# avik-pal/RegNeuralDE.jl

Measured on AMD Instinct MI355X. Metric: training-step samples/sec + mean NFE, MNIST Neural ODE bs=512, higher is better.
Workload: dtype f32; 1 GPU; MNIST NODE regularized (error_est), Tsit5 reltol=abstol=1.4e-8, batch 512 per GPU, 1xMI355X per rank; step = loss fwd + reverse pass through the solver + InvDecay/Momentum update; the weights train during the timed steps (mean_nfe drifts with --steps: value_fixed_weights of --full is the stationary companion); global_batch=512, parallelism=single

## Files before the change

### include/rnde.h

```cpp
#ifndef RNDE_H
#define RNDE_H
#include <stddef.h>
#include <stdint.h>

#ifdef __cplusplus
extern "C" {
#endif

#define RNDE_MAX_LAYERS 8

typedef enum {
    RNDE_OK = 0,
    RNDE_ERR_BAD_ARG = 1,
    RNDE_ERR_MAX_ATTEMPTS = 2,
    RNDE_ERR_DT_UNDERFLOW = 3,
    RNDE_ERR_NONFINITE = 4,
    RNDE_ERR_HIP = 5,
    RNDE_ERR_NO_TAPE = 6,
    RNDE_ERR_NO_DEVICE = 7
} rnde_status;

typedef enum { RNDE_ACT_IDENTITY = 0, RNDE_ACT_TANH = 1, RNDE_ACT_RELU = 2, RNDE_ACT_SIGMOID = 3, RNDE_ACT_SOFTPLUS = 4, RNDE_ACT_ELU = 5 } rnde_act;
typedef enum { RNDE_PRE_NONE = 0, RNDE_PRE_TANH = 1, RNDE_PRE_CUBE = 2 } rnde_pre_act;
typedef enum { RNDE_SOLVER_TSIT5 = 0, RNDE_SOLVER_DP5 = 1, RNDE_SOLVER_DOP853 = 2 } rnde_solver;
typedef enum { RNDE_REG_NONE = 0, RNDE_REG_ERR = 1, RNDE_REG_STIFF = 2, RNDE_REG_ERR_STIFF = 3,
               RNDE_REG_STIFF_DT = 4
} rnde_reg;

typedef struct {
    int32_t n_layers;
    int32_t dims[RNDE_MAX_LAYERS + 1];
    int32_t act[RNDE_MAX_LAYERS];
    int32_t time_dep;
    int32_t pre_act;
    int32_t max_batch;
    int32_t solver;
    float   reltol, abstol;
    int32_t regularize;
    int32_t cb_save_start;
    int32_t track_ctrl;
    int32_t track_initdt;
    int32_t max_attempts;
    int32_t device;
    int32_t col_tile;
    int32_t persist;
    int32_t wgrad_side_pct;
    int32_t stage_generic;
} rnde_node_config;

typedef struct rnde_node rnde_node;
typedef struct rnde_comm rnde_comm;

const char* rnde_version(void);
const char* rnde_last_error(const rnde_node* h);
int32_t     rnde_param_count(const rnde_node_config* cfg);

rnde_status rnde_node_create(const rnde_node_config* cfg, rnde_node** out);
void        rnde_node_destroy(rnde_node* h);

rnde_status rnde_node_create_tiled(const rnde_node_config* cfg, rnde_node** out);
int64_t     rnde_node_tiled_lds_bytes(const rnde_node_config* cfg);

rnde_status rnde_node_forward(rnde_node* h, const float* x_dev, const float* p_dev, int32_t B,
                              float t0, float t1, float* u_out_dev, int64_t* nfe_out,
                              float* saveval_host, int32_t* n_saveval_out, int32_t keep_tape,
                              void* stream);

rnde_status rnde_node_forward_saveat(rnde_node* h, const float* x_dev, const float* p_dev, int32_t B,
                                     float t0, float t1, const float* saveat_host, int32_t n_saveat,
                                     float* u_saved_dev, int64_t* nfe_out, float* saveval_host,
                                     int32_t* n_saveval_out, int32_t keep_tape, void* stream);

rnde_status rnde_node_forward_everystep(rnde_node* h, const float* x_dev, const float* p_dev, int32_t B, float t0, float t1,
                                        int32_t save_start, float* sol_out_dev, int32_t capacity, float* t_host_out, int32_t* n_out,
                                        int64_t* nfe_out, float* saveval_host, int32_t* n_saveval_out, int32_t keep_tape, void* stream);

rnde_status rnde_node_forward_replay(rnde_node* h, const float* x_dev, const float* p_dev, int32_t B,
                                     float t0, float t1, const float* steps_host, int32_t n_steps,
                                     float* u_out_dev, int64_t* nfe_out, float* saveval_host,
                                     int32_t* n_saveval_out, int32_t keep_tape, void* stream);

rnde_status rnde_node_backward(rnde_node* h, const float* u_bar_dev, const float* saveval_bar_host,
                               float* x_bar_dev, float* p_bar_dev, float* tspan_bar_host,
                               void* stream);

rnde_status rnde_node_backward_async(rnde_node* h, const float* u_bar_dev, const float* saveval_bar_host,
                                     float* x_bar_dev, float* p_bar_dev, float* tspan_bar_dev, void* stream);

rnde_status rnde_node_release_tape(rnde_node* h);

rnde_status rnde_node_forward_host(rnde_node* h, const float* x, const float* p, int32_t B, float t0,
                                   float t1, float* u_out, int64_t* nfe_out, float* saveval,
                                   int32_t* n_saveval_out, int32_t keep_tape);
rnde_status rnde_node_backward_host(rnde_node* h, const float* u_bar, const float* saveval_bar,
                                    float* x_bar, float* p_bar, float* tspan_bar);

rnde_status rnde_node_steps(rnde_node* h, float* steps_host, int32_t capacity, int32_t* n_attempts_out);

rnde_status rnde_debug_feval(rnde_node* h, const float* u_dev, const float* p_dev, int32_t B, float t,
                             float* out_dev, void* stream);
rnde_status rnde_debug_attempt(rnde_node* h, const float* uprev_dev, const float* k1_dev,
                               const float* p_dev, int32_t B, float t, float dt, float* k_out_dev,
                               float* unew_out_dev, float* eest_out, void* stream);
rnde_status rnde_bench_attempt(rnde_node* h, const float* x_dev, const float* p_dev, int32_t B,
                               int32_t iters, float* mean_us_out, void* stream);
rnde_status rnde_bench_attempt_taped(rnde_node* h, const float* x_dev, const float* p_dev, int32_t B,
                                     int32_t iters, float* mean_us_out, void* stream);
rnde_status rnde_bench_attempt_cold_tape(rnde_node* h, const float* x_dev, const float* p_dev, int32_t B, int32_t iters,
                                         int32_t records, float* mean_us_out, void* stream);
rnde_status rnde_node_set_timing(rnde_node* h, int32_t on);
rnde_status rnde_node_timing(rnde_node* h, float* fwd_attempts_ms, float* rev_sweep_ms, float* rev_rest_ms);
int32_t     rnde_node_last_attempts(const rnde_node* h);
int32_t     rnde_node_fallback_count(const rnde_node* h);
int32_t     rnde_node_launches_per_attempt(const rnde_node* h);
int32_t     rnde_node_one_launch_solves(const rnde_node* h);
#define RNDE_MATRIX_F32 0
#define RNDE_MATRIX_BF16X3 1
rnde_status rnde_node_set_matrix_mode(rnde_node* h, int32_t mode);
int32_t     rnde_node_matrix_mode(const rnde_node* h);

typedef struct rnde_tapes rnde_tapes;
rnde_status rnde_tapes_create(const rnde_node_config* cfg, int32_t max_tapes, rnde_tapes** out);
void        rnde_tapes_destroy(rnde_tapes* t);
const char* rnde_tapes_last_error(const rnde_tapes* t);
int32_t     rnde_tapes_in_use(const rnde_tapes* t);
rnde_node*  rnde_tapes_node(rnde_tapes* t, int32_t tape_id);
rnde_status rnde_tapes_forward(rnde_tapes* t, const float* x_dev, const float* p_dev, int32_t B, float t0, float t1, float* u_out_dev,
                               int64_t* nfe_out, float* saveval_host, int32_t* n_saveval_out, int32_t keep_tape, void* stream,
                               int32_t* tape_id_out);
rnde_status rnde_tapes_backward(rnde_tapes* t, int32_t tape_id, const float* u_bar_dev, const float* saveval_bar_host, float* x_bar_dev,
                                float* p_bar_dev, float* tspan_bar_host, void* stream);
rnde_status rnde_tapes_release(rnde_tapes* t, int32_t tape_id);

rnde_status rnde_classifier_head(rnde_node* h, const float* u_dev, const float* p3_dev, const float* y_dev,
                                 int32_t B, int32_t n_classes, float* logits_out_dev, float* u_bar_dev,
                                 float* p3_bar_dev, float* ce_out_dev, void* stream);

rnde_status rnde_node_classifier_grad(rnde_node* h, const float* x_dev, const float* p2_dev, const float* p3_dev,
                                      const float* y_dev, int32_t B, int32_t n_classes, float t0, float t1, float lambda,
                                      float* p2_bar_dev, float* p3_bar_dev, float* x_bar_dev, float* ce_out_dev,
                                      float* reg_out_host, int64_t* nfe_out, rnde_comm* comm, void* stream);

rnde_status rnde_momentum_step(float* p_dev, const float* g_dev, float* v_dev, int64_t len, int64_t n, float gamma,
                               float eta, float rho, void* stream);

rnde_status rnde_momentum_step_scaled(float* p_dev, const float* g_dev, float* v_dev, int64_t len, int64_t n, float gamma,
                                      float eta, float rho, float gscale, void* stream);
rnde_status rnde_adam_step(float* p_dev, const float* g_dev, float* m_dev, float* v_dev, int64_t len, int64_t t, float eta, float beta1,
                           float beta2, float eps, float gscale, void* stream);
rnde_status rnde_adabelief_step(float* p_dev, const float* g_dev, float* m_dev, float* s_dev, int64_t len, float eta, float beta1, float beta2,
                                float eps, float gscale, void* stream);

#define RNDE_COMM_ID_BYTES 128
rnde_status rnde_comm_unique_id(uint8_t id_out[RNDE_COMM_ID_BYTES]);
rnde_status rnde_comm_create(const uint8_t id[RNDE_COMM_ID_BYTES], int32_t rank, int32_t world, int32_t device, rnde_comm** out);
void        rnde_comm_destroy(rnde_comm* c);
int32_t     rnde_comm_world(const rnde_comm* c);
const char* rnde_comm_last_error(const rnde_comm* c);
const char* rnde_comm_library(void);
rnde_status rnde_comm_allreduce(rnde_comm* c, float* buf_dev, int64_t n, int32_t mean, void* stream);
rnde_status rnde_comm_create_local_group(int32_t world, int32_t device, rnde_comm** out);
rnde_status rnde_comm_health(rnde_comm* c);
#define RNDE_COMM_WINDOW_BYTES 64
typedef struct rnde_comm_window rnde_comm_window;
rnde_status rnde_comm_window_create(int32_t device, rnde_comm_window** win_out, uint8_t handle_out[RNDE_COMM_WINDOW_BYTES]);
void        rnde_comm_window_destroy(rnde_comm_window* w);
rnde_status rnde_comm_create_peers(rnde_comm_window* win, const uint8_t* handles, int32_t rank, int32_t world, rnde_comm** out);
const char* rnde_comm_path(const rnde_comm* c);

rnde_status rnde_node_set_coupling(rnde_node* h, rnde_comm* c, int32_t global_batch);

typedef enum { RNDE_SDE_SOSRI = 0, RNDE_SDE_SRIW1 = 1, RNDE_SDE_SOSRI2 = 2 } rnde_sde_solver;

typedef struct {
    int32_t drift_layers;
    int32_t drift_dims[RNDE_MAX_LAYERS + 1];
    int32_t drift_act[RNDE_MAX_LAYERS];
    int32_t diff_layers;
    int32_t diff_dims[RNDE_MAX_LAYERS + 1];
    int32_t diff_act[RNDE_MAX_LAYERS];
    int32_t max_batch;
    int32_t solver;
    float   reltol, abstol;
    int32_t regularize;
    int32_t cb_save_start;
    int32_t max_attempts;
    int32_t device;
    float   beta1, beta2, gamma, qmin, qmax, qoldinit, delta;
    int32_t generic;
    float   stability_size;
} rnde_nsde_config;

typedef struct rnde_nsde rnde_nsde;

int32_t     rnde_nsde_param_count(const rnde_nsde_config* cfg, int32_t* len_drift_out);
rnde_status rnde_nsde_create(const rnde_nsde_config* cfg, rnde_nsde** out);
void        rnde_nsde_destroy(rnde_nsde* h);
const char* rnde_nsde_last_error(const rnde_nsde* h);

rnde_status rnde_nsde_forward(rnde_nsde* h, const float* x_dev, const float* p_dev, int32_t B, float t0, float t1,
                              const float* noise_dev, int32_t n_pool, uint64_t seed, float* u_out_dev,
                              int64_t* nfe1_out, int64_t* nfe2_out, float* saveval_host, int32_t* n_saveval_out,
                              int32_t keep_tape, void* stream);
rnde_status rnde_nsde_forward_saveat(rnde_nsde* h, const float* x_dev, const float* p_dev, int32_t B, float t0, float t1,
                                     const float* noise_dev, int32_t n_pool, uint64_t seed, const float* saveat_host,
                                     int32_t n_saveat, float* u_saved_dev, int64_t* nfe1_out, int64_t* nfe2_out,
                                     float* saveval_host, int32_t* n_saveval_out, int32_t keep_tape, void* stream);

rnde_status rnde_nsde_forward_everystep(rnde_nsde* h, const float* x_dev, const float* p_dev, int32_t B, float t0, float t1,
                                        const float* noise_dev, int32_t n_pool, uint64_t seed, int32_t save_start, float* sol_out_dev,
                                        int32_t capacity, float* t_host_out, int32_t* n_out, int64_t* nfe1_out, int64_t* nfe2_out,
                                        float* saveval_host, int32_t* n_saveval_out, int32_t keep_tape, void* stream);
rnde_status rnde_nsde_forward_replay(rnde_nsde* h, const float* x_dev, const float* p_dev, int32_t B, float t0, float t1,
                                     const float* noise_dev, int32_t n_pool, const float* steps_host, int32_t n_steps,
                                     float* u_out_dev, int64_t* nfe1_out, int64_t* nfe2_out, float* saveval_host,
                                     int32_t* n_saveval_out, int32_t keep_tape, void* stream);
rnde_status rnde_nsde_backward(rnde_nsde* h, const float* u_bar_dev, const float* saveval_bar_host, float* x_bar_dev,
                               float* p_bar_dev, void* stream);
rnde_status rnde_nsde_backward_async(rnde_nsde* h, const float* u_bar_dev, const float* saveval_bar_host, float* x_bar_dev,
                               float* p_bar_dev, void* stream);
rnde_status rnde_nsde_classifier_head(rnde_nsde* h, const float* u_dev, const float* p3_dev, const float* y_dev, int32_t B, int32_t n_classes,
                                      float* logits_out_dev, float* u_bar_dev, float* p3_bar_dev, float* ce_out_dev, void* stream);

rnde_status rnde_nsde_classifier_grad(rnde_nsde* h, const float* x_dev, const float* p2_dev, const float* p3_dev, const float* y_dev,
                                      int32_t B, int32_t n_classes, float t0, float t1, const float* noise_dev, int32_t n_pool,
                                      uint64_t seed, float lambda, float* p2_bar_dev, float* p3_bar_dev, float* x_bar_dev,
                                      float* ce_out_dev, float* reg_out_host, int64_t* nfe1_out, int64_t* nfe2_out, void* stream);
rnde_status rnde_moment_loss(const float* u_saved_dev, const float* data_mean_dev, const float* data_var_dev, int32_t D, int32_t T, int32_t B,
                             float* loss_out_dev, float* u_bar_dev, void* stream);
rnde_status rnde_nsde_moment_grad(rnde_nsde* h, const float* x_dev, const float* p_dev, int32_t B, float t0, float t1, const float* noise_dev,
                                  int32_t n_pool, uint64_t seed, const float* saveat_host, int32_t n_saveat, const float* data_mean_dev,
                                  const float* data_var_dev, float c, float* p_bar_dev, float* x_bar_dev, float* loss_out_dev, float* reg_out_host,
                                  int64_t* nfe1_out, int64_t* nfe2_out, void* stream);
rnde_status rnde_nsde_set_pre_act(rnde_nsde* h, int32_t drift_pre, int32_t diff_pre);
rnde_status rnde_nsde_steps(rnde_nsde* h, float* steps_host, int32_t capacity, int32_t* n_attempts_out, int32_t* draws_out);
rnde_status rnde_nsde_debug_attempt(rnde_nsde* h, const float* uprev_dev, const float* p_dev, int32_t B, float dt,
                                    const float* dW_dev, const float* dZ_dev, float* kg_out_dev, float* unew_out_dev,
                                    float* eest_out, void* stream);
rnde_status rnde_nsde_timing(rnde_nsde* h, float* solve_ms, float* rev_sweep_ms, int32_t* attempts, int32_t* accepted);
rnde_status rnde_normal_fill(float* out_dev, int64_t n, uint64_t seed, uint64_t stream_id, void* stream);

typedef struct { int32_t max_batch, max_T, device; } rnde_latent_config;
typedef struct rnde_latent rnde_latent;
rnde_status rnde_latent_create(const rnde_latent_config* cfg, rnde_latent** out);
void        rnde_latent_destroy(rnde_latent* h);
const char* rnde_latent_last_error(const rnde_latent* h);
void        rnde_latent_param_counts(int32_t* n_p1, int32_t* n_p2, int32_t* n_p4);
rnde_status rnde_latent_encode(rnde_latent* h, const float* x_dev, const float* p1_dev, const float* p2_dev, const float* eps_dev, int32_t B,
                               int32_t T, float* z0_out_dev, float* mu0_out_dev, float* logvar_out_dev, void* stream);
rnde_status rnde_latent_decode_loss(rnde_latent* h, const float* res_dev, const float* p4_dev, const float* x_dev, int32_t B, int32_t T,
                                    float* loss2_out_dev, float* res_bar_out_dev, float* p4_bar_out_dev, void* stream);
rnde_status rnde_adamax_step(float* p_dev, const float* g_dev, float* m_dev, float* u_dev, int64_t len, int64_t n, float gamma, float eta, float beta1,
                             float beta2, float eps, float beta1_pow, void* stream);
rnde_status rnde_latent_encode_backward(rnde_latent* h, const float* z0_bar_dev, float lambda_k, const float* p1_dev, const float* p2_dev,
                                        const float* x_dev, float* p1_bar_out_dev, float* p2_bar_out_dev, void* stream);

typedef enum { RNDE_FFJORD_CONCAT_SQUASH = 0, RNDE_FFJORD_TRACKER_FORWARD = 1 } rnde_ffjord_dynamics;
typedef struct {
    int32_t in_dims, hidden;
    int32_t dynamics;
    int32_t time_dep;
    int32_t regularize;
    int32_t kinetic_reg;
    int32_t max_batch, solver;
    float reltol, abstol;
    int32_t cb_save_start;
    int32_t max_attempts, device;
} rnde_ffjord_config;
// ... 59 lines not shown
```

### regneuralde.jl_amd/_lib.py

```python
import ctypes as C
import os

from . import build as _build

MAX_LAYERS = 8
OK, BAD_ARG, MAX_ATTEMPTS, DT_UNDERFLOW, NONFINITE, HIP_ERR, NO_TAPE, NO_DEVICE = range(8)
REG = {"none": 0, False: 0, None: 0, "error_est": 1, True: 1, "stiff_est": 2, "error_stiff_est": 3}


class NodeConfig(C.Structure):
    _fields_ = [("n_layers", C.c_int32), ("dims", C.c_int32 * (MAX_LAYERS + 1)), ("act", C.c_int32 * MAX_LAYERS),
                ("time_dep", C.c_int32), ("pre_act", C.c_int32), ("max_batch", C.c_int32), ("solver", C.c_int32),
                ("reltol", C.c_float), ("abstol", C.c_float), ("regularize", C.c_int32),
                ("cb_save_start", C.c_int32), ("track_ctrl", C.c_int32), ("track_initdt", C.c_int32),
                ("max_attempts", C.c_int32), ("device", C.c_int32), ("col_tile", C.c_int32),
                ("persist", C.c_int32), ("wgrad_side_pct", C.c_int32), ("stage_generic", C.c_int32)]


class NsdeConfig(C.Structure):
    _fields_ = [("drift_layers", C.c_int32), ("drift_dims", C.c_int32 * (MAX_LAYERS + 1)), ("drift_act", C.c_int32 * MAX_LAYERS),
                ("diff_layers", C.c_int32), ("diff_dims", C.c_int32 * (MAX_LAYERS + 1)), ("diff_act", C.c_int32 * MAX_LAYERS),
                ("max_batch", C.c_int32), ("solver", C.c_int32), ("reltol", C.c_float), ("abstol", C.c_float),
                ("regularize", C.c_int32), ("cb_save_start", C.c_int32), ("max_attempts", C.c_int32), ("device", C.c_int32),
                ("beta1", C.c_float), ("beta2", C.c_float), ("gamma", C.c_float), ("qmin", C.c_float), ("qmax", C.c_float),
                ("qoldinit", C.c_float), ("delta", C.c_float), ("generic", C.c_int32), ("stability_size", C.c_float)]


class FfjordConfig(C.Structure):
    _fields_ = [("in_dims", C.c_int32), ("hidden", C.c_int32), ("dynamics", C.c_int32), ("time_dep", C.c_int32), ("regularize", C.c_int32),
                ("kinetic_reg", C.c_int32), ("max_batch", C.c_int32), ("solver", C.c_int32), ("reltol", C.c_float), ("abstol", C.c_float),
                ("cb_save_start", C.c_int32), ("max_attempts", C.c_int32), ("device", C.c_int32)]


class FfjordChainConfig(C.Structure):
    _fields_ = [("n_layers", C.c_int32), ("dims", C.c_int32 * (MAX_LAYERS + 1)), ("act", C.c_int32 * MAX_LAYERS), ("time_dep", C.c_int32),
                ("regularize", C.c_int32), ("max_batch", C.c_int32), ("solver", C.c_int32), ("reltol", C.c_float), ("abstol", C.c_float),
                ("cb_save_start", C.c_int32), ("max_attempts", C.c_int32), ("device", C.c_int32)]


class LatentConfig(C.Structure):
    _fields_ = [("max_batch", C.c_int32), ("max_T", C.c_int32), ("device", C.c_int32)]


ODE_SOLVER = {"Tsit5": 0, "AutoTsit5": 0, "DP5": 1, "DOP853": 2}
SDE_SOLVER = {"SOSRI": 0, "SRIW1": 1, "SOSRI2": 2, "AutoSOSRI2": 2}


class RndeError(RuntimeError):
    def __init__(self, status, msg):
        super().__init__(f"rnde status {status}: {msg}")
        self.status = status


_lib = None


def lib():
    global _lib
    if _lib is not None:
        return _lib
    path = _build.LIB
    if not os.path.exists(path):
        raise ImportError(f"{path} is missing: build it with `python -c 'import __graft_entry__ as g; g.build()'` "
                          "(hipcc --offload-arch=gfx950). There is no CPU fallback for the integration path.")
    L = C.CDLL(path)
    vp, f, i32, i64p, fp, i32p = C.c_void_p, C.c_float, C.c_int32, C.POINTER(C.c_int64), C.POINTER(C.c_float), C.POINTER(C.c_int32)
    L.rnde_version.restype = C.c_char_p
    L.rnde_last_error.restype = C.c_char_p
    L.rnde_last_error.argtypes = [vp]
    L.rnde_param_count.restype = i32
    L.rnde_param_count.argtypes = [C.POINTER(NodeConfig)]
    L.rnde_node_create.argtypes = [C.POINTER(NodeConfig), C.POINTER(vp)]
    L.rnde_node_destroy.argtypes = [vp]
    L.rnde_node_destroy.restype = None
    L.rnde_node_create_tiled.argtypes = [C.POINTER(NodeConfig), C.POINTER(vp)]
    L.rnde_node_tiled_lds_bytes.argtypes = [C.POINTER(NodeConfig)]
    L.rnde_node_tiled_lds_bytes.restype = C.c_int64
    L.rnde_node_forward.argtypes = [vp, vp, vp, i32, f, f, vp, i64p, fp, i32p, i32, vp]
    L.rnde_node_forward_saveat.argtypes = [vp, vp, vp, i32, f, f, fp, i32, vp, i64p, fp, i32p, i32, vp]
    L.rnde_node_forward_everystep.argtypes = [vp, vp, vp, i32, f, f, i32, vp, i32, fp, i32p, i64p, fp, i32p, i32, vp]
    L.rnde_node_forward_replay.argtypes = [vp, vp, vp, i32, f, f, fp, i32, vp, i64p, fp, i32p, i32, vp]
    L.rnde_node_backward.argtypes = [vp, vp, fp, vp, vp, fp, vp]
    L.rnde_node_backward_async.restype = C.c_int32
    L.rnde_node_backward_async.argtypes = [vp, vp, fp, vp, vp, vp, vp]
    L.rnde_node_release_tape.argtypes = [vp]
    L.rnde_node_forward_host.argtypes = [vp, fp, fp, i32, f, f, fp, i64p, fp, i32p, i32]
    L.rnde_node_backward_host.argtypes = [vp, fp, fp, fp, fp, fp]
    L.rnde_node_steps.argtypes = [vp, fp, i32, i32p]
    L.rnde_debug_feval.argtypes = [vp, vp, vp, i32, f, vp, vp]
    L.rnde_debug_attempt.argtypes = [vp, vp, vp, vp, i32, f, f, vp, vp, fp, vp]
    L.rnde_bench_attempt.argtypes = [vp, vp, vp, i32, i32, fp, vp]
    L.rnde_bench_attempt_taped.argtypes = [vp, vp, vp, i32, i32, fp, vp]
    L.rnde_bench_attempt_cold_tape.argtypes = [vp, vp, vp, i32, i32, i32, fp, vp]
    L.rnde_node_set_timing.argtypes = [vp, i32]
    L.rnde_node_timing.argtypes = [vp, fp, fp, fp]
    L.rnde_node_fallback_count.restype = C.c_int32
    L.rnde_node_fallback_count.argtypes = [vp]
    L.rnde_node_last_attempts.restype = C.c_int32
    L.rnde_node_last_attempts.argtypes = [vp]
    L.rnde_node_launches_per_attempt.restype = C.c_int32
    L.rnde_node_launches_per_attempt.argtypes = [vp]
    L.rnde_node_one_launch_solves.restype = C.c_int32
    L.rnde_node_one_launch_solves.argtypes = [vp]
    L.rnde_node_set_matrix_mode.restype = C.c_int32
    L.rnde_node_set_matrix_mode.argtypes = [vp, i32]
    L.rnde_node_matrix_mode.restype = C.c_int32
    L.rnde_node_matrix_mode.argtypes = [vp]
    L.rnde_classifier_head.argtypes = [vp, vp, vp, vp, i32, i32, vp, vp, vp, vp, vp]
    L.rnde_node_classifier_grad.argtypes = [vp, vp, vp, vp, vp, i32, i32, f, f, f, vp, vp, vp, vp, fp, C.POINTER(C.c_int64), vp, vp]
    L.rnde_momentum_step.argtypes = [vp, vp, vp, C.c_int64, C.c_int64, f, f, f, vp]
    u64 = C.c_uint64
    L.rnde_momentum_step_scaled.argtypes = [vp, vp, vp, C.c_int64, C.c_int64, f, f, f, f, vp]
    L.rnde_adam_step.argtypes = [vp, vp, vp, vp, C.c_int64, C.c_int64, C.c_float, C.c_float, C.c_float, C.c_float, C.c_float, vp]
    L.rnde_adabelief_step.argtypes = [vp, vp, vp, vp, C.c_int64, f, f, f, f, f, vp]
    L.rnde_moment_loss.argtypes = [vp, vp, vp, i32, i32, i32, vp, vp, vp]
    L.rnde_comm_unique_id.argtypes = [C.c_char_p]
    L.rnde_comm_create.argtypes = [C.c_char_p, i32, i32, i32, C.POINTER(vp)]
    L.rnde_comm_destroy.argtypes = [vp]
    L.rnde_comm_destroy.restype = None
    L.rnde_comm_world.argtypes = [vp]
    L.rnde_comm_world.restype = i32
    L.rnde_comm_last_error.argtypes = [vp]
    L.rnde_comm_last_error.restype = C.c_char_p
    L.rnde_comm_library.argtypes = []
    L.rnde_comm_library.restype = C.c_char_p
    L.rnde_comm_allreduce.argtypes = [vp, vp, C.c_int64, i32, vp]
    L.rnde_comm_create_local_group.argtypes = [i32, i32, C.POINTER(vp)]
    L.rnde_node_set_coupling.argtypes = [vp, vp, i32]
    L.rnde_comm_health.argtypes = [vp]
    L.rnde_comm_window_create.argtypes = [i32, C.POINTER(vp), C.c_char_p]
    L.rnde_comm_window_destroy.argtypes = [vp]
    L.rnde_comm_window_destroy.restype = None
    L.rnde_comm_create_peers.argtypes = [vp, C.c_char_p, i32, i32, C.POINTER(vp)]
    L.rnde_comm_path.argtypes = [vp]
    L.rnde_comm_path.restype = C.c_char_p
    L.rnde_tapes_create.argtypes = [C.POINTER(NodeConfig), i32, C.POINTER(vp)]
    L.rnde_tapes_destroy.argtypes = [vp]
    L.rnde_tapes_destroy.restype = None
    L.rnde_tapes_last_error.argtypes = [vp]
    L.rnde_tapes_last_error.restype = C.c_char_p
    L.rnde_tapes_in_use.argtypes = [vp]
    L.rnde_tapes_node.argtypes = [vp, i32]
    L.rnde_tapes_node.restype = vp
    L.rnde_tapes_forward.argtypes = [vp, vp, vp, i32, C.c_float, C.c_float, vp, C.POINTER(C.c_int64), fp, C.POINTER(i32), i32, vp, C.POINTER(i32)]
    L.rnde_tapes_backward.argtypes = [vp, i32, vp, fp, vp, vp, fp, vp]
    L.rnde_tapes_release.argtypes = [vp, i32]
    L.rnde_nsde_param_count.restype = i32
    L.rnde_nsde_param_count.argtypes = [C.POINTER(NsdeConfig), i32p]
    L.rnde_nsde_create.argtypes = [C.POINTER(NsdeConfig), C.POINTER(vp)]
    L.rnde_nsde_destroy.argtypes = [vp]
    L.rnde_nsde_destroy.restype = None
    L.rnde_nsde_last_error.restype = C.c_char_p
    L.rnde_nsde_last_error.argtypes = [vp]
    L.rnde_nsde_forward.argtypes = [vp, vp, vp, i32, f, f, vp, i32, u64, vp, i64p, i64p, fp, i32p, i32, vp]
    L.rnde_nsde_forward_saveat.argtypes = [vp, vp, vp, i32, f, f, vp, i32, u64, fp, i32, vp, i64p, i64p, fp, i32p, i32, vp]
    L.rnde_nsde_forward_everystep.argtypes = [vp, vp, vp, i32, f, f, vp, i32, u64, i32, vp, i32, fp, i32p, i64p, i64p, fp, i32p, i32, vp]
    L.rnde_nsde_forward_replay.argtypes = [vp, vp, vp, i32, f, f, vp, i32, fp, i32, vp, i64p, i64p, fp, i32p, i32, vp]
    L.rnde_nsde_backward.argtypes = [vp, vp, fp, vp, vp, vp]
    L.rnde_nsde_backward_async.argtypes = [vp, vp, fp, vp, vp, vp]
    L.rnde_nsde_classifier_head.argtypes = [vp, vp, vp, vp, i32, i32, vp, vp, vp, vp, vp]
    L.rnde_nsde_classifier_grad.argtypes = [vp, vp, vp, vp, vp, i32, i32, f, f, vp, i32, C.c_uint64, f, vp, vp, vp, vp, fp, C.POINTER(C.c_int64), C.POINTER(C.c_int64), vp]
    L.rnde_nsde_steps.argtypes = [vp, fp, i32, i32p, i32p]
    L.rnde_nsde_debug_attempt.argtypes = [vp, vp, vp, i32, f, vp, vp, vp, vp, fp, vp]
    L.rnde_nsde_set_pre_act.argtypes = [vp, i32, i32]
    L.rnde_nsde_moment_grad.argtypes = [vp, vp, vp, i32, f, f, vp, i32, u64, fp, i32, vp, vp, f, vp, vp, vp, fp, i64p, i64p, vp]
    L.rnde_nsde_timing.argtypes = [vp, fp, fp, i32p, i32p]
    L.rnde_normal_fill.argtypes = [vp, C.c_int64, u64, u64, vp]
    L.rnde_latent_create.argtypes = [C.POINTER(LatentConfig), C.POINTER(vp)]
    L.rnde_latent_destroy.argtypes = [vp]
    L.rnde_latent_destroy.restype = None
    L.rnde_latent_last_error.argtypes = [vp]
    L.rnde_latent_last_error.restype = C.c_char_p
    L.rnde_latent_param_counts.argtypes = [i32p, i32p, i32p]
    L.rnde_latent_param_counts.restype = None
    L.rnde_latent_encode.argtypes = [vp, vp, vp, vp, vp, i32, i32, vp, vp, vp, vp]
    L.rnde_latent_decode_loss.argtypes = [vp, vp, vp, vp, i32, i32, vp, vp, vp, vp]
    L.rnde_latent_encode_backward.argtypes = [vp, vp, f, vp, vp, vp, vp, vp, vp]
    L.rnde_adamax_step.argtypes = [vp, vp, vp, vp, C.c_int64, C.c_int64, f, f, f, f, f, f, vp]
    L.rnde_ffjord_param_count.restype = i32
    L.rnde_ffjord_param_count.argtypes = [C.POINTER(FfjordConfig)]
    L.rnde_ffjord_create.argtypes = [C.POINTER(FfjordConfig), C.POINTER(vp)]
    L.rnde_ffjord_destroy.argtypes = [vp]
    L.rnde_ffjord_destroy.restype = None
    L.rnde_ffjord_last_error.argtypes = [vp]
    L.rnde_ffjord_last_error.restype = C.c_char_p
    L.rnde_ffjord_forward.argtypes = [vp, vp, vp, vp, i32, f, f, u64, vp, vp, i64p, fp, i32p, i32, vp]
    L.rnde_ffjord_forward_replay.argtypes = [vp, vp, vp, vp, i32, f, f, u64, fp, i32, vp, vp, i64p, fp, i32p, i32, vp]
    L.rnde_ffjord_steps.argtypes = [vp, fp, i32, i32p]
    L.rnde_ffjord_backward.argtypes = [vp, vp, fp, vp, vp, vp]
    L.rnde_ffjord_sample.argtypes = [vp, vp, vp, i32, f, f, u64, vp, vp]
    L.rnde_ffjord_debug_feval.argtypes = [vp, vp, vp, vp, i32, f, i32, vp, vp]
    L.rnde_ffjord_timing.argtypes = [vp, fp, fp, i32p, i32p]
    L.rnde_ffjord_create_tiled.argtypes = [C.POINTER(FfjordConfig), C.POINTER(vp)]
    L.rnde_ffjord_engine.restype = i32
    L.rnde_ffjord_engine.argtypes = [vp]
    L.rnde_ffjord_forward_kinetic.argtypes = [vp, vp, vp, vp, i32, f, f, u64, vp, vp, vp, i64p, i32, vp]
    L.rnde_ffjord_forward_kinetic_replay.argtypes = [vp, vp, vp, vp, i32, f, f, u64, fp, i32, vp, vp, vp, i64p, i32, vp]
    L.rnde_ffjord_backward_kinetic.argtypes = [vp, vp, vp, vp, vp, vp]
    L.rnde_ffjord_debug_feval_kinetic.argtypes = [vp, vp, vp, vp, i32, f, vp, vp]
    L.rnde_ffjord_step_log.argtypes = [vp, fp, i32, i32p]
    L.rnde_ffjord_chain_param_count.restype = i32
    L.rnde_ffjord_chain_param_count.argtypes = [C.POINTER(FfjordChainConfig)]
    L.rnde_ffjord_create_chain.argtypes = [C.POINTER(FfjordChainConfig), C.POINTER(vp)]
    L.rnde_ffjord_forward_exact.argtypes = [vp, vp, vp, i32, f, f, vp, vp, i64p, fp, i32p, i32, vp]
    L.rnde_ffjord_forward_exact_replay.argtypes = [vp, vp, vp, i32, f, f, fp, i32, vp, vp, i64p, fp, i32p, i32, vp]
    L.rnde_ffjord_set_track_ctrl.argtypes = [vp, i32]
    L.rnde_ffjord_track_ctrl.restype = i32
    L.rnde_ffjord_track_ctrl.argtypes = [vp]
    _lib = L
    return L


EXPORTS = ["rnde_version", "rnde_last_error", "rnde_param_count", "rnde_node_create", "rnde_node_destroy",
           "rnde_node_forward", "rnde_node_forward_saveat", "rnde_node_forward_everystep", "rnde_node_forward_replay", "rnde_node_backward", "rnde_node_backward_async", "rnde_node_release_tape", "rnde_node_forward_host",
           "rnde_node_backward_host", "rnde_node_steps", "rnde_debug_feval", "rnde_debug_attempt",
           "rnde_bench_attempt", "rnde_bench_attempt_taped", "rnde_bench_attempt_cold_tape", "rnde_node_set_timing", "rnde_node_timing", "rnde_node_last_attempts", "rnde_node_fallback_count",
           "rnde_node_launches_per_attempt", "rnde_node_one_launch_solves", "rnde_node_set_matrix_mode", "rnde_node_matrix_mode", "rnde_classifier_head", "rnde_node_classifier_grad", "rnde_momentum_step", "rnde_momentum_step_scaled", "rnde_adam_step",
           "rnde_comm_unique_id", "rnde_comm_create", "rnde_comm_destroy", "rnde_comm_world", "rnde_comm_last_error", "rnde_comm_library", "rnde_comm_allreduce", "rnde_comm_create_local_group", "rnde_comm_health", "rnde_comm_window_create", "rnde_comm_window_destroy", "rnde_comm_create_peers", "rnde_comm_path", "rnde_node_set_coupling", "rnde_tapes_create", "rnde_tapes_destroy", "rnde_tapes_last_error", "rnde_tapes_in_use", "rnde_tapes_node", "rnde_tapes_forward", "rnde_tapes_backward", "rnde_tapes_release",
           "rnde_nsde_param_count", "rnde_nsde_create", "rnde_nsde_destroy", "rnde_nsde_last_error", "rnde_nsde_forward",
           "rnde_nsde_forward_saveat", "rnde_nsde_forward_everystep", "rnde_nsde_forward_replay", "rnde_nsde_backward", "rnde_nsde_backward_async", "rnde_nsde_classifier_head", "rnde_nsde_classifier_grad", "rnde_nsde_steps", "rnde_nsde_debug_attempt", "rnde_nsde_set_pre_act", "rnde_nsde_moment_grad", "rnde_moment_loss", "rnde_adabelief_step", "rnde_nsde_timing", "rnde_normal_fill", "rnde_latent_create", "rnde_latent_destroy", "rnde_latent_last_error", "rnde_latent_param_counts", "rnde_latent_encode",
           "rnde_latent_decode_loss", "rnde_latent_encode_backward", "rnde_adamax_step",
           "rnde_ffjord_param_count", "rnde_ffjord_create", "rnde_ffjord_destroy", "rnde_ffjord_last_error", "rnde_ffjord_forward",
           "rnde_ffjord_forward_replay", "rnde_ffjord_steps", "rnde_ffjord_backward", "rnde_ffjord_sample", "rnde_ffjord_debug_feval",
           "rnde_ffjord_timing", "rnde_ffjord_create_tiled", "rnde_ffjord_engine", "rnde_ffjord_forward_kinetic",
           "rnde_ffjord_forward_kinetic_replay", "rnde_ffjord_backward_kinetic", "rnde_ffjord_debug_feval_kinetic", "rnde_ffjord_step_log",
           "rnde_ffjord_chain_param_count", "rnde_ffjord_create_chain", "rnde_ffjord_forward_exact", "rnde_ffjord_forward_exact_replay",
           "rnde_ffjord_set_track_ctrl", "rnde_ffjord_track_ctrl",
           "rnde_node_create_tiled", "rnde_node_tiled_lds_bytes"]


def check(h, status):
    if status != OK:
        msg = lib().rnde_last_error(h).decode() if h else lib().rnde_last_error(None).decode()
        raise RndeError(status, msg)


def check_latent(h, status):
    if status != OK:
        raise RndeError(status, lib().rnde_latent_last_error(h if h else None).decode())


def check_ffjord(h, status):
    if status != OK:
        raise RndeError(status, lib().rnde_ffjord_last_error(h if h else None).decode())


def check_nsde(h, status):
    if status != OK:
        raise RndeError(status, lib().rnde_nsde_last_error(h if h else None).decode())
```

### regneuralde.jl_amd/csrc/rnde.hip

```cpp
#include "rnde_node.h"

static thread_local std::string g_create_err;
void rnde_set_create_error(const std::string& msg) { g_create_err = msg; }
extern "C" const char* rnde_version(void) { return "rnde 0.1.0 (gfx950)"; }
extern "C" const char* rnde_last_error(const rnde_node* h) { return h ? h->err.c_str() : g_create_err.c_str(); }

extern "C" int32_t rnde_param_count(const rnde_node_config* c) {
    int n = 0;
    for (int l = 0; l < c->n_layers; ++l) n += (c->dims[l] + (c->time_dep ? 1 : 0)) * c->dims[l + 1] + c->dims[l + 1];
    return n;
}

StepParams make_params(rnde_node* h, const float* x, int B, float t0, float t1, int tape) {
    StepParams P{};
    P.x = x;
    P.f0 = h->f0; P.h0 = h->h0; P.u1 = h->u1; P.f1 = h->f1; P.h1 = h->h1;
    P.arena = h->arena; P.rec_stride = h->rec_stride;
    P.ctl = h->ctl; P.ctl_final = h->ctl_final; P.meta = h->meta; P.initrec = h->initrec;
    P.errpart = h->errpart; P.initpart = h->initpart; P.dbg_out = nullptr;
    P.D = h->D; P.H = h->H; P.B = B; P.Bn = h->couple ? h->couple_batch : B;
    P.Bpad = ((B + 15) / 16) * 16;
    P.nwg = h->engine == 2 ? h->sR * (P.Bpad / 16) : (h->engine == 3 ? (h->mw ? P.Bpad / 16 : (P.Bpad / 16 + kCW - 1) / kCW) : P.Bpad / h->BT);
    P.reltol = h->cfg.reltol; P.abstol = h->cfg.abstol; P.t0 = t0; P.t1 = t1;
    P.tape = tape; P.max_attempts = h->cfg.max_attempts;
// ... 233 lines not shown
    if (h->mw_lat) return h->rk_tab ? launch_mw_t<2, MODE, 1, 1>(h, Q, n, s) : launch_mw_t<2, MODE, 0, 1>(h, Q, n, s);
    if (h->rk_tab) {
        switch (h->NKD) {
            case 4: return launch_mw_t<1, MODE, 1>(h, Q, n, s);
            case 8: return launch_mw_t<2, MODE, 1>(h, Q, n, s);
            default: return launch_mw_t<4, MODE, 1>(h, Q, n, s);
        }
    }
    switch (h->NKD) {
        case 4: return launch_mw_t<1, MODE, 0>(h, Q, n, s);
        case 8: return launch_mw_t<2, MODE, 0>(h, Q, n, s);
        default: return launch_mw_t<4, MODE, 0>(h, Q, n, s);
    }
}
static rnde_status ensure_mw_slab(rnde_node* h, long long evals, int Bpad, hipStream_t s) {
    const long long per_eval = (long long)(h->Bpad_max / 16) * h->mg.RS * 64;
    (void)Bpad;
    if (h->mw_slab_evals >= evals) return RNDE_OK;
    long long want = std::max(evals, 2 * h->mw_slab_evals);
    {
        const long long full = 2 + (long long)(h->rk_S - 1) * h->cfg.max_attempts;
        long long cap_mb = 8192;
        if (const char* e = getenv("RNDE_EAGER_SLAB_MB")) cap_mb = atoll(e);
        size_t fr = 0, tot = 0;
        const size_t full_bytes = (size_t)full * per_eval * 4;
        if (full > want && cap_mb > 0 && full_bytes <= (size_t)cap_mb << 20 && hipMemGetInfo(&fr, &tot) == hipSuccess && full_bytes <= fr / 8) want = full;
    }
    float* nb = nullptr;
    HIPCHK(h, hipStreamSynchronize(s));
    if (hipMalloc((void**)&nb, (size_t)want * per_eval * 4) != hipSuccess) {
        (void)hipGetLastError();
        nb = nullptr;
        want = evals;
        HIPCHK(h, hipMalloc((void**)&nb, (size_t)want * per_eval * 4));
    }
    if (h->mw_slab) {
        HIPCHK(h, hipMemcpy(nb, h->mw_slab, (size_t)h->mw_slab_evals * per_eval * 4, hipMemcpyDeviceToDevice));
        hipFree(h->mw_slab);
    }
    h->mw_slab = nb; h->mw_slab_evals = want;
    return RNDE_OK;
}

static rnde_status chain_pack(rnde_node* h, const float* p_dev, hipStream_t s) {
    if (h->mw) {
        const long long tm = (long long)mw_tab_floats(h->mg);
        hipLaunchKernelGGL(rnde_chainmw_pack_kernel, dim3((int)std::min<long long>((tm + 255) / 256, 512)), dim3(256), 0, s, p_dev, h->mw_tab, h->mg);
        HIPCHK(h, hipGetLastError());
        return RNDE_OK;
    }
    const long long total = (long long)(h->cg.nfrag_f + h->cg.nfrag_b + h->cg.nfrag_t) * 64;
    hipLaunchKernelGGL(rnde_chain_pack_kernel, dim3((int)std::min<long long>((total + 255) / 256, 512)), dim3(256), 0, s, p_dev, h->cfrags, h->cg);
    HIPCHK(h, hipGetLastError());
    return RNDE_OK;
}
static hipError_t chain_convert(const float* src, float* dst, int D, int B, int ntiles, int nksD, int to_caller, hipStream_t s) {
    const long long total = (long long)ntiles * nksD * 64;
    hipLaunchKernelGGL(rnde_chain_convert_kernel, dim3((int)std::min<long long>((total + 255) / 256, 512)), dim3(256), 0, s, src, dst, D, B, ntiles, nksD, to_caller);
    return hipGetLastError();
}

extern "C" rnde_status rnde_node_create(const rnde_node_config* c, rnde_node** out) {
    *out = nullptr;
    int ndev = 0;
    if (hipGetDeviceCount(&ndev) != hipSuccess || ndev <= c->device) { g_create_err = "no HIP device"; return RNDE_ERR_NO_DEVICE; }
    if ((c->solver != RNDE_SOLVER_TSIT5 && c->solver != RNDE_SOLVER_DP5 && c->solver != RNDE_SOLVER_DOP853) || c->n_layers < 1 || c->n_layers > RNDE_MAX_LAYERS || c->dims[0] != c->dims[c->n_layers]) {
        g_create_err = "unsupported configuration: Tsit5 (or DP5) over a Dense chain with dims[0] == dims[n_layers]"; return RNDE_ERR_BAD_ARG;
    }
    if (c->pre_act != RNDE_PRE_NONE && c->pre_act != RNDE_PRE_TANH && c->pre_act != RNDE_PRE_CUBE) {
        g_create_err = "pre_act: RNDE_PRE_NONE, RNDE_PRE_TANH or RNDE_PRE_CUBE"; return RNDE_ERR_BAD_ARG;
    }
    if (!rnde_check_acts(c->n_layers, c->act, "act", g_create_err)) return RNDE_ERR_BAD_ARG;
    const bool mnist_form = c->n_layers == 2 && c->time_dep && !c->pre_act && c->act[0] == RNDE_ACT_TANH;
    if (mnist_form && c->col_tile != 64 && c->col_tile != 65 && c->act[1] != RNDE_ACT_IDENTITY && c->act[1] != RNDE_ACT_TANH) {
        g_create_err = std::string("act[1] = ") + rnde_act_name(c->act[1]) + ": the stage engine (two time-dependent layers, act[0] = tanh, no pre_act, col_tile 0 / 16) "
                       "serves identity or tanh in its second layer; a chain of width <= 64 runs any served activation on the chain engine (col_tile 64 / 65)";
        return RNDE_ERR_BAD_ARG;
    }
    if ((c->solver == RNDE_SOLVER_DP5 || c->solver == RNDE_SOLVER_DOP853) && ((mnist_form && c->col_tile != 65) || c->col_tile == 64 || c->regularize >= RNDE_REG_STIFF)) {
        g_create_err = "DP5 / DOP853 run on the tableau-as-data kernels of the chain engine (col_tile 0 for Dense chains of width <= 64, or 65), callbacks none / EEst*dt";
        return RNDE_ERR_BAD_ARG;
    }
    if (c->col_tile == 64 || c->col_tile == 65 || !mnist_form) return chain_create(c, out);
    if (c->regularize < RNDE_REG_NONE || c->regularize > RNDE_REG_STIFF_DT) { g_create_err = "regularize: unknown value"; return RNDE_ERR_BAD_ARG; }
    rnde_node* h = new rnde_node();
    h->cfg = *c;
    h->D = c->dims[0]; h->H = c->dims[1]; h->P = rnde_param_count(c); h->act2 = c->act[1];
    h->BT = 8;
    if (c->col_tile != 0 && c->col_tile != 16) {
        g_create_err = "col_tile must be 0 (auto) or 16 (stage engine) for the two-layer TDChain form; 64 / 65 select the chain engine.  (The round-1 column-owner "
                       "engine, col_tile 4 / 8, was retired in round 4: 126 us per attempted step against 24; its sources are kept under tools/experiments/column_owner/.)";
        delete h; return RNDE_ERR_BAD_ARG;
    }
    if (h->H + 2 > 128 || h->D < 1 || h->H < 1 || (h->D + 15) / 16 > 64 || c->max_batch < 1 || c->max_attempts < 1) {
        g_create_err = "shape outside the kernel limits (H <= 126, D <= 1024)"; delete h; return RNDE_ERR_BAD_ARG;
    }
    h->Bpad_max = ((c->max_batch + 15) / 16) * 16;
    h->sMT = (h->D + 15) / 16; h->sHT = (h->H + 1 + 15) / 16; h->sK2b = (h->H + 2 + 15) / 16; h->sKHb = (h->H + 15) / 16;
    { int best = 1, bw = 1 << 30;
      for (int wt = std::min(8, h->sMT); wt >= std::max(1, std::min(4, h->sMT)); --wt) { int R = (h->sMT + wt - 1) / wt; int waste = R * wt - h->sMT; if (waste < bw) { bw = waste; best = wt; } }
      if (const char* e = getenv("RNDE_STAGE_WT")) { const int v = atoi(e); if (v >= 1 && v <= 8) best = std::min(v, h->sMT); }
      h->sWT = best; h->sR = (h->sMT + best - 1) / best; }
    h->engine = 2;
    h->nwg_max = std::max(h->Bpad_max / h->BT, h->sR * (h->Bpad_max / 16));
    h->stage_lds = sizeof(float) * ((size_t)16 * (16 * std::max(h->sK2b, h->sHT) + 4) + (size_t)16 * (16 * std::max(h->sWT, h->sKHb) + 4) + 64);
    if (hipSetDevice(c->device) != hipSuccess) { g_create_err = "hipSetDevice failed"; delete h; return RNDE_ERR_HIP; }
    const size_t A = (size_t)h->D * h->Bpad_max, HB = (size_t)h->H * h->Bpad_max;
    RecLayout L{(long long)A, (long long)HB};
    h->rec_stride = L.total();
    auto dm = [&](void** p, size_t bytes) { return hipMalloc(p, bytes) == hipSuccess; };
    bool ok = true;
    ok &= dm((void**)&h->f0, A * 4) && dm((void**)&h->u1, A * 4) && dm((void**)&h->f1, A * 4) && dm((void**)&h->xcopy, A * 4);
    ok &= dm((void**)&h->h0, HB * 4) && dm((void**)&h->h1, HB * 4);
    ok &= dm((void**)&h->pcopy, (size_t)h->P * 4);
    ok &= dm((void**)&h->spwB, (size_t)h->sMT * h->sK2b * 64 * 16) && dm((void**)&h->spwD, (size_t)h->sHT * h->sMT * 64 * 16);
    ok &= dm((void**)&h->spwBt, (size_t)h->sMT * h->sKHb * 64 * 16) && dm((void**)&h->spwDt, (size_t)h->sHT * h->sMT * 64 * 16);
    ok &= dm((void**)&h->slab2, (size_t)2 * (h->Bpad_max / 16) * h->sR * h->sHT * 64 * 16);
    const size_t tslab_bytes = (size_t)kSlabBufs * (h->Bpad_max / 16) * h->sR * h->sHT * 64 * 16;
    h->tslab_bytes = tslab_bytes;
    ok &= dm((void**)&h->tslab, tslab_bytes);
    static_assert(sizeof(StepState) <= 512 && sizeof(InitRec) <= 504, "mailbox layout");
    h->mbox_meta_off = (1024 + (size_t)h->nwg_max * 4 + 255) / 256 * 256;
    const size_t mbox_bytes = h->mbox_meta_off + (size_t)(c->max_attempts + 1) * sizeof(StepMeta);
    ok &= dm((void**)&h->mbox, mbox_bytes) && hipHostMalloc((void**)&h->h_mbox, mbox_bytes) == hipSuccess;
    if (ok) {
        hipMemset(h->mbox, 0, mbox_bytes);
        h->ctl_final = (StepState*)h->mbox; h->initrec = (InitRec*)(h->mbox + 512);
        h->pabort = (unsigned*)(h->mbox + 1016); h->pxcc = (unsigned*)(h->mbox + 1024); h->meta = (StepMeta*)(h->mbox + h->mbox_meta_off);
        h->h_ctl = (StepState*)h->h_mbox; h->h_init = (InitRec*)(h->h_mbox + 512);
        h->h_pchk = (unsigned*)(h->h_mbox + 1016); h->h_meta = (StepMeta*)(h->h_mbox + h->mbox_meta_off);
    }
    ok &= dm((void**)&h->ctl, 2 * sizeof(StepState));
    ok &= dm((void**)&h->errpart, (size_t)(6 * h->nwg_max + 256 + 16) * 4) && dm((void**)&h->initpart, (size_t)(3 * h->nwg_max + 256) * 4);
    h->arena_recs = 2;
    ok &= dm((void**)&h->arena, (size_t)h->arena_recs * h->rec_stride * 4);
    ok &= hipHostMalloc((void**)&h->h_scal, 64 * sizeof(float)) == hipSuccess;
    if (!ok) { g_create_err = "device allocation failed"; rnde_node_destroy(h); return RNDE_ERR_HIP; }
    hipMemset(h->tslab, 0xFF, tslab_bytes); hipMemset(h->pabort, 0, 8); hipMemset(h->pxcc, 0, (size_t)h->nwg_max * 4);
    {
        const char* e = getenv("RNDE_PERSIST");
        const bool off = c->persist < 0 || (e && e[0] == '0');
        h->persist = (h->engine == 2 && h->sR <= 8 && !off) ? 1 : 0;
        if (const char* e2 = getenv("RNDE_PERSIST_SPINS")) h->persist_spins = atoi(e2);
        if (const char* e3 = getenv("RNDE_PERSIST2")) h->persist2 = atoi(e3);
        h->wgrad_side_pct = c->wgrad_side_pct < 0 ? 0 : (c->wgrad_side_pct == 0 ? 30 : std::min(100, c->wgrad_side_pct));
        if (const char* e3 = getenv("RNDE_WGRAD_SIDE")) h->wgrad_side_pct = atoi(e3);
        h->stage_generic = (c->stage_generic != 0 || getenv("RNDE_STAGE_GENERIC") != nullptr) ? 1 : 0;
        if (const char* e6 = getenv("RNDE_STAGE_SOLVE")) h->stage_solve = atoi(e6);
    }
    if (h->persist == 1 && h->stage_solve && c->max_attempts + kSolveInitRows < (int)kMeetRows) {
        if (h->s_meet.create_granules((size_t)c->max_attempts + kSolveInitRows, 3, 256) != hipSuccess) { g_create_err = "device allocation failed"; rnde_node_destroy(h); return RNDE_ERR_HIP; }
    }
    if (h->persist == 1) {
        h->x3 = 1;
        if (const char* e7 = getenv("RNDE_X3")) h->x3 = atoi(e7) != 0;
        if (h->sMT == 49 && h->sHT == 7 && h->sR == 7 && h->sWT == 7 && h->D == 784 && h->H == 100 && !h->stage_generic) {
            const size_t img = (size_t)49 * 4 * 3 * 64 * 16;
            if (hipMalloc(&h->x3B, img) != hipSuccess || hipMalloc(&h->x3D, img) != hipSuccess || hipMalloc(&h->x3Bt, img) != hipSuccess || hipMalloc(&h->x3Dt, img) != hipSuccess) { g_create_err = "device allocation failed"; rnde_node_destroy(h); return RNDE_ERR_HIP; }
        } else h->x3 = 0;
    }
    h->predicted = 12;
    *out = h;
    return RNDE_OK;
}

extern "C" void rnde_node_destroy(rnde_node* h) {
    if (!h) return;
    node_tiled_destroy(h);
    void* d[] = {h->f0, h->h0, h->u1, h->f1, h->h1, h->arena, h->xcopy, h->pcopy, h->spwB, h->spwD, h->spwBt, h->spwDt, h->slab2,
                 h->ctl, h->ctl_final, h->meta, h->initrec, h->errpart, h->initpart};
    if (h->mbox || h->h_mbox) {
        for (void*& p : d) if (p == h->ctl_final || p == h->meta || p == h->initrec) p = nullptr;
        h->pabort = h->pxcc = nullptr; h->h_pchk = nullptr; h->h_ctl = nullptr; h->h_meta = nullptr; h->h_init = nullptr;
        if (h->mbox) hipFree(h->mbox);
        if (h->h_mbox) hipHostFree(h->h_mbox);
    }
    for (void* p : d) if (p) hipFree(p);
    bwd_free(h->bw);
    if (h->head_ws) hipFree(h->head_ws);
    if (h->cg_ws) hipFree(h->cg_ws);
    if (h->ev_host) hipEventDestroy(h->ev_host);
    if (h->sv_t_dev) hipFree(h->sv_t_dev);
    if (h->replay_dev) hipFree(h->replay_dev);
    if (h->cfrags) hipFree(h->cfrags);
    if (h->mw_tab) hipFree(h->mw_tab);
    h->mw_meet.destroy();
    if (h->h_mw_bchk) hipHostFree(h->h_mw_bchk);
    if (h->h_mw_bargs) hipHostFree(h->h_mw_bargs);
    if (h->mw_bargs) hipFree(h->mw_bargs);
    if (h->mw_slab) hipFree(h->mw_slab);
    if (h->tslab) hipFree(h->tslab);
    h->s_meet.destroy();
    if (h->x3B) hipFree(h->x3B);
    if (h->x3D) hipFree(h->x3D);
    if (h->x3Bt) hipFree(h->x3Bt);
    if (h->x3Dt) hipFree(h->x3Dt);
    if (h->pabort) hipFree(h->pabort);
    if (h->pxcc) hipFree(h->pxcc);
    if (h->h_pchk) hipHostFree(h->h_pchk);
    if (h->cslab) hipFree(h->cslab);
    if (h->ev_t) hipFree(h->ev_t);
    if (h->h_ev_t) hipHostFree(h->h_ev_t);
    for (hipEvent_t e : h->wevents) hipEventDestroy(e);
    for (hipEvent_t e : h->tev) if (e) hipEventDestroy(e);
    if (h->wstream) hipStreamDestroy(h->wstream);
    if (h->h_ctl) hipHostFree(h->h_ctl);
    if (h->h_meta) hipHostFree(h->h_meta);
    if (h->h_init) hipHostFree(h->h_init);
    if (h->h_scal) hipHostFree(h->h_scal);
    delete h;
}

rnde_status couple_sum(rnde_node* h, float* partials, long long count, hipStream_t s) {
    if (!h->couple) return RNDE_OK;
    const rnde_status st = rnde_comm_allreduce(h->couple, partials, count, 0, (void*)s);
    if (st != RNDE_OK) h->err = std::string("coupled controller: ") + rnde_comm_last_error(h->couple);
    return st;
}
extern "C" rnde_status rnde_node_set_coupling(rnde_node* h, rnde_comm* c, int32_t global_batch) {
    if (!h) return RNDE_ERR_BAD_ARG;
    RNDE_TILED_REFUSE(h, "rnde_node_set_coupling is not served (one controller over several shards: the stage engine and the chain engine's multi-wave kernels, rnde_node_create)");
    if (!c) { h->couple = nullptr; h->couple_batch = 0; h->couple_world = 1; return RNDE_OK; }
    const int world = rnde_comm_world(c);
    if (h->engine != 2 && !(h->engine == 3 && h->mw)) { h->err = "coupled controller: the stage engine (MNIST form, col_tile 0 or 16) and the chain engine's multi-wave kernels only"; return RNDE_ERR_BAD_ARG; }
    if (global_batch < world || world < 1) { h->err = "coupled controller: global_batch must cover every rank"; return RNDE_ERR_BAD_ARG; }
    h->couple = c; h->couple_batch = global_batch; h->couple_world = world;
    return RNDE_OK;
}

static rnde_status ensure_arena(rnde_node* h, long long recs) {
    if (h->arena_recs >= recs) return RNDE_OK;
    if (h->arena) hipFree(h->arena);
    h->arena = nullptr; h->arena_recs = 0;
    HIPCHK(h, hipMalloc((void**)&h->arena, (size_t)recs * h->rec_stride * 4));
    h->arena_recs = recs;
    return RNDE_OK;
}

static StageParams make_stage_params(rnde_node* h, const StepParams& P, const float* p_dev) {
    StageParams Q{};
    Q.F = P; Q.p = p_dev; Q.pwB = h->spwB; Q.pwD = h->spwD; Q.slab = h->slab2;
    Q.MT = h->sMT; Q.WT = h->sWT; Q.R = h->sR; Q.C = P.Bpad / 16; Q.HT = h->sHT; Q.K2b = h->sK2b; Q.Bpad16 = P.Bpad;
    return Q;
}
template <int ACT2, int MODE>
static hipError_t launch_stage_t(rnde_node* h, const StageParams& Q, int n, int s, hipStream_t st) {
    hipLaunchKernelGGL((rnde_stage_kernel<ACT2, MODE>), dim3(Q.R * Q.C), dim3(64 * Q.WT), h->stage_lds, st, Q, n, s);
    return hipGetLastError();
}
template <int MODE>
static hipError_t launch_stage(rnde_node* h, const StageParams& Q, int n, int s, hipStream_t st) {
    return h->act2 ? launch_stage_t<1, MODE>(h, Q, n, s, st) : launch_stage_t<0, MODE>(h, Q, n, s, st);
}
hipError_t stage_pack(rnde_node* h, const float* p, f32x4* dst, int which, int MTrows, int Kb, hipStream_t st) {
    const long long total = (long long)MTrows * Kb * 64;
    const int grid = (int)std::min<long long>((total + 255) / 256, 1024);
    hipLaunchKernelGGL(rnde_stage_pack_kernel, dim3(grid), dim3(256), 0, st, p, dst, which, h->D, h->H, MTrows, Kb);
    return hipGetLastError();
}
static rnde_status x3_pack(rnde_node* h, const float* p_dev, bool with_rev, hipStream_t s) {
    h->x3_fwd = false;
    if (!(h->x3 && h->x3B && h->x3D && h->persist == 1 && !h->stage_generic)) return RNDE_OK;
    HIPCHK(h, rnde_launch_x3_pack(p_dev, h->x3B, h->x3D, with_rev ? h->x3Bt : nullptr, with_rev ? h->x3Dt : nullptr, h->D, h->H, h->sMT, h->sWT, h->sR, h->sHT, s));
    h->x3_fwd = true;
    h->x3_packed = with_rev;
    return RNDE_OK;
}
static rnde_status stage_pack_weights(rnde_node* h, const float* p_dev, hipStream_t s) {
    HIPCHK(h, stage_pack(h, p_dev, h->spwB, 0, h->sMT, h->sK2b, s));
    HIPCHK(h, stage_pack(h, p_dev, h->spwD, 1, h->sHT, h->sMT, s));
    return x3_pack(h, p_dev, false, s);
}
rnde_status stage_pack_all(rnde_node* h, const float* p_dev, hipStream_t s, const float* x_src, long long x_floats) {
    PackJobs J{};
    int n = 0;
    auto add = [&](void* dst, long long total, int kind, int which, int kdim, const float* src = nullptr) { J.j[n++] = PackJob{dst, src, total, kind, which, kdim, 0}; };
    add(h->spwB, (long long)h->sMT * h->sK2b * 64, 0, 0, h->sK2b);
    add(h->spwD, (long long)h->sHT * h->sMT * 64, 0, 1, h->sMT);
    add(h->spwBt, (long long)h->sMT * h->sKHb * 64, 0, 2, h->sKHb);
    add(h->spwDt, (long long)h->sHT * h->sMT * 64, 0, 3, h->sMT);
    auto add_copy = [&](float* dst, const float* src, long long floats) {
        const bool v4 = floats % 4 == 0 && ((uintptr_t)dst % 16 == 0) && ((uintptr_t)(src ? src : p_dev) % 16 == 0);
        add(dst, v4 ? floats / 4 : floats, v4 ? 3 : 2, 0, 0, src);
    };
    add_copy(h->pcopy, nullptr, (long long)h->P);
    if (x_src) add_copy(h->xcopy, x_src, x_floats);
    long long most = 0;
    for (int i = 0; i < n; ++i) most = std::max(most, J.j[i].total);
    const int grid = (int)std::min<long long>((most + 255) / 256, 256);
    hipLaunchKernelGGL(rnde_pack_all_kernel, dim3(grid, n), dim3(256), 0, s, p_dev, J, h->D, h->H);
    HIPCHK(h, hipGetLastError());
    h->rev_packed = true;
    return x3_pack(h, p_dev, true, s);
}
hipError_t slab_prepare(rnde_node* h, int Bpad, hipStream_t s) {
    if (h->tslab_Bpad == Bpad) return hipSuccess;
    h->tslab_Bpad = Bpad;
    return hipMemsetAsync(h->tslab, 0xFF, h->tslab_bytes, s);
}
static bool stage_two_tile(const rnde_node* h, const StageParams& Q) {
    const bool fix = Q.WT == 7 && Q.HT == 7 && Q.K2b == 7 && Q.MT == 49 && Q.R == 7 && h->D == 784 && h->H == 100 && !h->stage_generic;
    return h->persist == 1 && fix && Q.C % 2 == 0 && h->persist2 != 0 && (Q.C >= kPersist2MinTiles || h->persist2 >= 1);
}
static bool stage_epart_reduce(const rnde_node* h, const StageParams& Q) {
    return stage_two_tile(h, Q) && Q.F.nwg >= 896 && !getenv("RNDE_NO_EPART_REDUCE");
}
static hipError_t stage_attempt(rnde_node* h, const StageParams& Q, int n, hipStream_t s) {
    if (h->persist == 1) {
        PersistSync Y{h->tslab, h->pabort, h->pxcc, h->persist_spins};
        if (hipError_t e = slab_prepare(h, Q.Bpad16, s); e != hipSuccess) return e;
        const dim3 grid(8 * Q.R * ((Q.C + 7) / 8));
        const bool fix = Q.WT == 7 && Q.HT == 7 && Q.K2b == 7 && Q.MT == 49 && Q.R == 7 && h->D == 784 && h->H == 100 && !h->stage_generic;
        static const bool x3_over_mt = !(getenv("RNDE_X3_MT") && atoi(getenv("RNDE_X3_MT")) == 0);
        if (stage_two_tile(h, Q)) {
            const dim3 grid2(8 * Q.R * ((Q.C / 2 + 7) / 8));
            if (h->x3_fwd && x3_over_mt) {
                const size_t xlds2 = sizeof(float) * ((size_t)2 * 2 * kX3ImageFloats + 32 * 3);
                if (h->act2) hipLaunchKernelGGL((rnde_stage_attempt_mt_kernel<1, 2, 1>), grid2, dim3(64 * 7), xlds2, s, Q, n, Y, (const void*)h->x3B, (const void*)h->x3D);
                else hipLaunchKernelGGL((rnde_stage_attempt_mt_kernel<0, 2, 1>), grid2, dim3(64 * 7), xlds2, s, Q, n, Y, (const void*)h->x3B, (const void*)h->x3D);
                return hipGetLastError();
            }
            const size_t lds2 = sizeof(float) * (2 * 2 * 16 * (16 * 7 + 4) + 32 * 3);
            if (h->act2) hipLaunchKernelGGL((rnde_stage_attempt_mt_kernel<1, 2>), grid2, dim3(64 * 7), lds2, s, Q, n, Y, (const void*)nullptr, (const void*)nullptr);
            else hipLaunchKernelGGL((rnde_stage_attempt_mt_kernel<0, 2>), grid2, dim3(64 * 7), lds2, s, Q, n, Y, (const void*)nullptr, (const void*)nullptr);
            return hipGetLastError();
        }
        if (fix && h->x3_fwd) {
            const size_t xlds = sizeof(float) * ((size_t)2 * kX3ImageFloats + 64);
            if (h->act2) hipLaunchKernelGGL((rnde_stage_attempt_kernel<1, 1, 1>), grid, dim3(64 * 7), xlds, s, Q, n, Y, (const void*)h->x3B, (const void*)h->x3D);
            else hipLaunchKernelGGL((rnde_stage_attempt_kernel<0, 1, 1>), grid, dim3(64 * 7), xlds, s, Q, n, Y, (const void*)h->x3B, (const void*)h->x3D);
        } else if (fix) {
            if (h->act2) hipLaunchKernelGGL((rnde_stage_attempt_kernel<1, 1>), grid, dim3(64 * Q.WT), h->stage_lds, s, Q, n, Y, (const void*)nullptr, (const void*)nullptr);
            else hipLaunchKernelGGL((rnde_stage_attempt_kernel<0, 1>), grid, dim3(64 * Q.WT), h->stage_lds, s, Q, n, Y, (const void*)nullptr, (const void*)nullptr);
        } else if (h->act2) hipLaunchKernelGGL((rnde_stage_attempt_kernel<1, 0>), grid, dim3(64 * Q.WT), h->stage_lds, s, Q, n, Y, (const void*)nullptr, (const void*)nullptr);
        else hipLaunchKernelGGL((rnde_stage_attempt_kernel<0, 0>), grid, dim3(64 * Q.WT), h->stage_lds, s, Q, n, Y, (const void*)nullptr, (const void*)nullptr);
        return hipGetLastError();
    }
    hipError_t e = launch_stage<SM_START>(h, Q, n, 0, s);
    for (int st = 1; st <= 5 && e == hipSuccess; ++st) e = launch_stage<SM_STAGE>(h, Q, n, st, s);
    if (e == hipSuccess) e = launch_stage<SM_LAST>(h, Q, n, 6, s);
    return e;
}

bool bsweep_failed(rnde_node* h, hipStream_t s) {
    if (!h->pending_bsweep) return false;
    h->pending_bsweep = false;
    const MeetVerdict v = meet_verdict(h->h_mw_bchk, h->bsweep_nt, h->bsweep_global);
    if (v == MEET_OK) return false;
    fprintf(stderr, "[rnde] chain engine: one-launch reverse sweep abandoned (%s); one launch per reversed attempt for the next %d solves\n",
            v == MEET_TIMED_OUT ? "a meeting timed out" : "workgroups pinned by block index landed on different XCDs", h->mw_retry_after);
    h->mw_bsweep = -1; h->mw_clean = 0; ++h->persist_fallbacks;
    h->mw_meet.clear_abort(s);
    h->h_mw_bchk[0] = 0;
    return true;
}

static rnde_status forward_core(rnde_node* h, const float* x_dev, const float* p_dev, int32_t B, float t0, float t1,
                                float* u_out_dev, const float* saveat_host, int32_t n_saveat, float* sv_out_dev,
                                int64_t* nfe_out, float* saveval_host, int32_t* n_saveval_out, int32_t keep_tape, void* stream);

void persist_check_enqueue(rnde_node* h, int grid, hipStream_t s) {
    if (h->persist != 1) return;
    h->h_pchk[0] = 1;
    if (hipMemcpyAsync(h->h_pchk, h->pabort, 8, hipMemcpyDeviceToHost, s) != hipSuccess) return;
    (void)hipMemcpyAsync(h->h_pchk + 2, h->pxcc, (size_t)grid * 4, hipMemcpyDeviceToHost, s);
}
bool persist_check_result(rnde_node* h, int C, int R, hipStream_t s) {
    if (h->persist != 1) return false;
    bool bad = h->h_pchk[0] != 0;
    for (int ct = 0; ct < C && !bad; ++ct)
        for (int rb = 1; rb < R; ++rb) if (h->h_pchk[2 + rb * C + ct] != h->h_pchk[2 + ct]) { bad = true; break; }
    if (bad) {
        fprintf(stderr, "[rnde] persistent attempt kernel suspended (%s); using the multi-launch kernels for the next %d solves\n",
                h->h_pchk[0] ? "hand-off timed out" : "column tile spans XCDs", h->persist_retry_after);
        h->persist = -1; h->persist_clean = 0; ++h->persist_fallbacks;
        hipMemsetAsync(h->pabort, 0, 8, s);
    }
    return bad;
}
static bool persist_failed(rnde_node* h, int grid, int C, int R, hipStream_t s) {
    if (h->persist != 1) return false;
    persist_check_enqueue(h, grid, s);
    if (hipStreamSynchronize(s) != hipSuccess) return true;
    return persist_check_result(h, C, R, s);
}

rnde_status forward_impl(rnde_node* h, const float* x_dev, const float* p_dev, int32_t B, float t0, float t1,
                                float* u_out_dev, const float* saveat_host, int32_t n_saveat, float* sv_out_dev,
                                int64_t* nfe_out, float* saveval_host, int32_t* n_saveval_out, int32_t keep_tape, void* stream) {
    if (h && h->engine == 4) return node_tiled_forward(h, x_dev, p_dev, B, t0, t1, u_out_dev, saveat_host, n_saveat, sv_out_dev, nfe_out, saveval_host, n_saveval_out, keep_tape, stream);
    rnde_status st = RNDE_INTERNAL_RETRY;
    for (int tries = 0; tries < 4 && st == RNDE_INTERNAL_RETRY; ++tries)
        st = forward_core(h, x_dev, p_dev, B, t0, t1, u_out_dev, saveat_host, n_saveat, sv_out_dev, nfe_out, saveval_host, n_saveval_out, keep_tape, stream);
    if (st == RNDE_INTERNAL_RETRY) { h->err = "the forward solve asked to be redone four times in a row (one-launch fallbacks and slab growth): giving up"; st = RNDE_ERR_HIP; }
    return st;
}

extern "C" rnde_status rnde_node_forward(rnde_node* h, const float* x_dev, const float* p_dev, int32_t B, float t0,
                                         float t1, float* u_out_dev, int64_t* nfe_out, float* saveval_host,
                                         int32_t* n_saveval_out, int32_t keep_tape, void* stream) {
    return forward_impl(h, x_dev, p_dev, B, t0, t1, u_out_dev, nullptr, 0, nullptr, nfe_out, saveval_host, n_saveval_out, keep_tape, stream);
}

extern "C" rnde_status rnde_node_forward_replay(rnde_node* h, const float* x_dev, const float* p_dev, int32_t B, float t0,
                                                float t1, const float* steps_host, int32_t n_steps, float* u_out_dev,
                                                int64_t* nfe_out, float* saveval_host, int32_t* n_saveval_out,
                                                int32_t keep_tape, void* stream) {
    if (!h || !steps_host || n_steps < 1) return RNDE_ERR_BAD_ARG;
    if (n_steps > h->cfg.max_attempts) { h->err = "replay: more steps than max_attempts"; return RNDE_ERR_BAD_ARG; }
    h->replay_host = steps_host; h->n_replay = n_steps;
    const rnde_status st = forward_impl(h, x_dev, p_dev, B, t0, t1, u_out_dev, nullptr, 0, nullptr, nfe_out, saveval_host, n_saveval_out, keep_tape, stream);
    h->replay_host = nullptr; h->n_replay = 0;
    return st;
}

extern "C" rnde_status rnde_node_forward_saveat(rnde_node* h, const float* x_dev, const float* p_dev, int32_t B, float t0,
                                                float t1, const float* saveat_host, int32_t n_saveat, float* u_saved_dev,
                                                int64_t* nfe_out, float* saveval_host, int32_t* n_saveval_out,
                                                int32_t keep_tape, void* stream) {
    if (!h || !saveat_host || n_saveat < 1 || !u_saved_dev) return RNDE_ERR_BAD_ARG;
    return forward_impl(h, x_dev, p_dev, B, t0, t1, nullptr, saveat_host, n_saveat, u_saved_dev, nfe_out, saveval_host, n_saveval_out, keep_tape, stream);
}

static rnde_status forward_core(rnde_node* h, const float* x_dev, const float* p_dev, int32_t B, float t0, float t1,
                                float* u_out_dev, const float* saveat_host, int32_t n_saveat, float* sv_out_dev,
                                int64_t* nfe_out, float* saveval_host, int32_t* n_saveval_out, int32_t keep_tape, void* stream) {
    if (!h) return RNDE_ERR_BAD_ARG;
    hipStream_t s = (hipStream_t)stream;
    if (n_saveat > 0) {
        if (h->rk_tab == 2) { h->err = "saveat: this Runge-Kutta table carries no dense output (DOP853)"; return RNDE_ERR_BAD_ARG; }
        for (int i = 0; i < n_saveat; ++i)
            if (!(saveat_host[i] >= t0 && saveat_host[i] <= t1) || (i > 0 && !(saveat_host[i] > saveat_host[i - 1]))) {
                h->err = "saveat must be increasing and inside [t0, t1]"; return RNDE_ERR_BAD_ARG;
            }
        if ((size_t)n_saveat > h->sv_cap) {
            if (h->sv_t_dev) hipFree(h->sv_t_dev);
            h->sv_t_dev = nullptr; h->sv_cap = 0;
            HIPCHK(h, hipMalloc((void**)&h->sv_t_dev, (size_t)n_saveat * 4));
            h->sv_cap = n_saveat;
        }
        h->saveat.assign(saveat_host, saveat_host + n_saveat);
        HIPCHK(h, hipMemcpyAsync(h->sv_t_dev, h->saveat.data(), (size_t)n_saveat * 4, hipMemcpyHostToDevice, s));
    } else h->saveat.clear();
    if (B < 1 || B > h->cfg.max_batch || !(t1 > t0)) { h->err = "bad B or tspan"; return RNDE_ERR_BAD_ARG; }
    if (h->couple && (long long)B * h->couple_world != h->couple_batch) {
// ... 211 lines not shown
            HIPCHK(h, hipMemcpyAsync(h->h_mbox, h->mbox, h->mbox_meta_off + (size_t)launched * sizeof(StepMeta), hipMemcpyDeviceToHost, s));
        } else {
            HIPCHK(h, hipMemcpyAsync(h->h_ctl, h->ctl_final, sizeof(StepState), hipMemcpyDeviceToHost, s));
            HIPCHK(h, hipMemcpyAsync(h->h_meta, h->meta, (size_t)launched * sizeof(StepMeta), hipMemcpyDeviceToHost, s));
            HIPCHK(h, hipMemcpyAsync(h->h_init, h->initrec, sizeof(InitRec), hipMemcpyDeviceToHost, s));
        }
        if (h->after_solve) {
            HIPCHK(h, hipEventRecord(h->ev_host, s));
            const rnde_status hs = h->after_solve(s);
            if (hs != RNDE_OK) return hs;
            HIPCHK(h, hipEventSynchronize(h->ev_host));
        } else HIPCHK(h, hipStreamSynchronize(s));
#ifdef RNDE_DIAG
        if (h->engine == 2 && getenv("RNDE_DIAG_FWD") && h->diag_buf) {
            unsigned long long hst[64] = {0};
            hipMemcpy(hst, h->diag_buf, sizeof(hst), hipMemcpyDeviceToHost);
            if (hst[34]) {
                fprintf(stderr, "attempt %s of a real solve (workgroup 0 thread 0, cycles): controller %lld startC %lld startD %lld |", getenv("RNDE_DIAG_FWD"), (long long)(hst[1]-hst[0]), (long long)(hst[2]-hst[1]), (long long)(hst[3]-hst[2]));
                for (int st_ = 0; st_ < 6; ++st_) fprintf(stderr, " poll %lld", (long long)(hst[4 + 5 * st_] - hst[3 + 5 * st_]));
                fprintf(stderr, " | total %lld  (entry -> all loads issued %lld, -> controller state here %lld)\n", (long long)(hst[34]-hst[0]), (long long)(hst[35]-hst[0]), (long long)(hst[36]-hst[35]));
            }
        }
#endif
        if (h->couple && rnde_comm_health(h->couple) != RNDE_OK) { h->err = std::string("coupled controller: ") + rnde_comm_last_error(h->couple); return RNDE_ERR_HIP; }
        if (bsweep_failed(h, s)) { h->err = "the one-launch reverse sweep of the previous asynchronous backward call was abandoned: the gradients of that step are invalid (one launch per reversed attempt now in use)"; return RNDE_ERR_HIP; }
        if (h->engine == 2 && persist_check_result(h, SQ.C, SQ.R, s)) {
            if (h->pending_bwd) {
                h->pending_bwd = false;
                h->err = "a persistent kernel abandoned its hand-off during or after the previous asynchronous reverse pass: the gradients of that step are invalid (multi-launch kernels now in use)";
                return RNDE_ERR_HIP;
            }
            if (h->couple) {
                h->err = "coupled controller: a persistent kernel abandoned its hand-off; the ranks are out of step -- use cfg.persist = -1 (7-launch kernels) with rnde_node_set_coupling where other work shares the GPU";
                return RNDE_ERR_HIP;
            }
            return RNDE_INTERNAL_RETRY;
        }
        h->pending_bwd = false;
        if (h->h_ctl->done) break;
        if (launched >= cap) { h->err = "max_attempts reached"; h->n_att = h->h_ctl->n_att; return RNDE_ERR_MAX_ATTEMPTS; }
        chunk = h->couple ? 16 : 4;
    }
    h->n_att = h->h_ctl->n_att;
    h->predicted = h->n_att + 1;
    if (h->engine == 3 && (h->mw_solve == -1 || h->mw_bsweep == -1) && ++h->mw_clean >= h->mw_retry_after) {
        if (h->mw_solve == -1) h->mw_solve = 1;
        if (h->mw_bsweep == -1) h->mw_bsweep = 1;
        h->mw_retry_after = std::min(1024, 2 * h->mw_retry_after);
        h->mw_meet.slot = (h->mw_meet.slot + 1) & 7;
    }
    if (h->persist == -1 && h->engine == 2 && h->cfg.persist >= 0 && ++h->persist_clean >= h->persist_retry_after) {
        h->persist = 1; h->persist_retry_after = std::min(1024, 2 * h->persist_retry_after);
        h->tslab_Bpad = -1;
    }
    if (nfe_out) *nfe_out = 3 + (int64_t)(h->rk_S - 1) * h->n_att;
    int nsv = 0;
    h->sv_index.assign(h->n_att, -1);
    const float stab = 1.0f / 3.5068f;
    auto cbval = [&](float eest, float dt, float eig) -> float {
        const bool eg_ok = !(eig == 0.f || eig != eig);
        switch (h->cfg.regularize) {
            case RNDE_REG_ERR: return eest * dt;
            case RNDE_REG_STIFF: return eg_ok ? stab * fabsf(eig) : 0.f;
            case RNDE_REG_ERR_STIFF: { const float e = eest * dt; return ((e == 0.f || e != e) ? 0.f : e) + 0.1f * (eg_ok ? stab * eig : 0.f); }
            case RNDE_REG_STIFF_DT: return fabsf(eig * dt);
            default: return 0.f;
        }
    };
    if (h->cfg.regularize != RNDE_REG_NONE) {
        if (h->cfg.cb_save_start) { if (saveval_host) saveval_host[nsv] = cbval(1.f, 0.f, 1.f); ++nsv; }
        for (int i = 0; i < h->n_att; ++i)
            if (h->h_meta[i].flags & F_ACCEPT) {
                if (saveval_host) saveval_host[nsv] = cbval(h->h_meta[i].eest, h->h_meta[i].dt, h->h_meta[i].eigen);
                h->sv_index[i] = nsv++;
            }
    }
    h->n_saveval = nsv;
    if (n_saveval_out) *n_saveval_out = nsv;
    switch (h->h_ctl->status) {
        case 0: break;
        case 2: h->err = "max_attempts reached"; return RNDE_ERR_MAX_ATTEMPTS;
        case 3: h->err = "dt underflow"; return RNDE_ERR_DT_UNDERFLOW;
        default: h->err = "non-finite error estimate or dt"; return RNDE_ERR_NONFINITE;
    }
    h->have_tape = keep_tape != 0;
    return RNDE_OK;
}

extern "C" rnde_status rnde_node_forward_everystep(rnde_node* h, const float* x_dev, const float* p_dev, int32_t B, float t0, float t1, int32_t save_start,
                                                   float* sol_out_dev, int32_t capacity, float* t_host_out, int32_t* n_out, int64_t* nfe_out,
                                                   float* saveval_host, int32_t* n_saveval_out, int32_t keep_tape, void* stream) {
    if (!h || !n_out || !sol_out_dev || capacity < 1) return RNDE_ERR_BAD_ARG;
    RNDE_TILED_REFUSE(h, "rnde_node_forward_everystep is not served (the end state only; save_everystep runs on the engines of rnde_node_create)");
    rnde_status st = forward_impl(h, x_dev, p_dev, B, t0, t1, nullptr, nullptr, 0, nullptr, nullptr, nullptr, nullptr, 0, stream);
    if (st != RNDE_OK) return st;
    std::vector<float> times;
    if (save_start) times.push_back(t0);
    for (int i = 0; i < h->n_att; ++i) {
        const StepMeta& m = h->h_meta[i];
        if (m.flags & F_ACCEPT) { float tn = m.t + m.dt; if (tn > t1) tn = t1; times.push_back(tn); }
    }
    *n_out = (int32_t)times.size();
    if ((int)times.size() > capacity) { h->err = "rnde_node_forward_everystep: more accepted steps than the output has room for"; return RNDE_ERR_BAD_ARG; }
    if (t_host_out) memcpy(t_host_out, times.data(), times.size() * sizeof(float));
    st = forward_impl(h, x_dev, p_dev, B, t0, t1, nullptr, times.data(), (int32_t)times.size(), sol_out_dev, nfe_out, saveval_host, n_saveval_out, keep_tape, stream);
    if (st != RNDE_OK) return st;
    size_t k = save_start ? 1 : 0;
    for (int i = 0; i < h->n_att; ++i) {
        const StepMeta& m = h->h_meta[i];
        if (!(m.flags & F_ACCEPT)) continue;
        float tn = m.t + m.dt; if (tn > t1) tn = t1;
        if (k >= times.size() || times[k] != tn) { h->err = "rnde_node_forward_everystep: the saving solve did not retrace the steps of the first one"; return RNDE_ERR_HIP; }
        ++k;
    }
    if (k != times.size()) { h->err = "rnde_node_forward_everystep: the saving solve took fewer accepted steps than the first one"; return RNDE_ERR_HIP; }
    return RNDE_OK;
}

extern "C" rnde_status rnde_node_steps(rnde_node* h, float* steps_host, int32_t capacity, int32_t* n_out) {
    if (!h) return RNDE_ERR_BAD_ARG;
    const int n = std::min(capacity, h->n_att);
    for (int i = 0; i < n; ++i) {
        steps_host[4 * i + 0] = h->h_meta[i].t; steps_host[4 * i + 1] = h->h_meta[i].dt;
        steps_host[4 * i + 2] = h->h_meta[i].eest; steps_host[4 * i + 3] = (h->h_meta[i].flags & F_ACCEPT) ? 1.f : 0.f;
    }
    if (n_out) *n_out = h->n_att;
    return RNDE_OK;
}

extern "C" rnde_status rnde_node_set_timing(rnde_node* h, int32_t on) {
    if (!h) return RNDE_ERR_BAD_ARG;
    if (on && !h->tev[0]) for (auto& e : h->tev) HIPCHK(h, hipEventCreate(&e));
    h->timing = on ? 1 : 0; h->tev_fwd = h->tev_bwd = false;
    return RNDE_OK;
}
extern "C" rnde_status rnde_node_timing(rnde_node* h, float* fwd_attempts_ms, float* rev_sweep_ms, float* rev_rest_ms) {
    if (h && h->engine == 4) return node_tiled_timing(h, fwd_attempts_ms, rev_sweep_ms, rev_rest_ms);
    if (!h || !h->timing) return RNDE_ERR_BAD_ARG;
    float a = -1.f, b = -1.f, c = -1.f;
    if (h->tev_fwd) { HIPCHK(h, hipEventSynchronize(h->tev[1])); HIPCHK(h, hipEventElapsedTime(&a, h->tev[0], h->tev[1])); }
    if (h->tev_bwd) {
        HIPCHK(h, hipEventSynchronize(h->tev[4]));
        HIPCHK(h, hipEventElapsedTime(&b, h->tev[2], h->tev[3])); HIPCHK(h, hipEventElapsedTime(&c, h->tev[3], h->tev[4]));
    }
    if (fwd_attempts_ms) *fwd_attempts_ms = a;
    if (rev_sweep_ms) *rev_sweep_ms = b;
    if (rev_rest_ms) *rev_rest_ms = c;
    return RNDE_OK;
}
extern "C" int32_t rnde_node_last_attempts(const rnde_node* h) { return h ? h->n_att : 0; }
extern "C" int32_t rnde_node_fallback_count(const rnde_node* h) { return h ? h->persist_fallbacks : 0; }

extern "C" int32_t rnde_node_one_launch_solves(const rnde_node* h) { return h ? h->one_launch_solves : 0; }
extern "C" rnde_status rnde_node_set_matrix_mode(rnde_node* h, int32_t mode) {
    if (!h) return RNDE_ERR_BAD_ARG;
    if (mode != RNDE_MATRIX_F32 && mode != RNDE_MATRIX_BF16X3) { h->err = "matrix mode: 0 (fp32-input MFMA) or 1 (bf16x3 on the matrix cores)"; return RNDE_ERR_BAD_ARG; }
    if (mode == RNDE_MATRIX_BF16X3) RNDE_TILED_REFUSE(h, "rnde_node_set_matrix_mode(h, 1) is not served (its layer products are the fp32-input MFMA, mode 0; bf16x3 serves the MNIST form on the stage engine)");
    h->x3 = (mode == RNDE_MATRIX_BF16X3 && h->x3B && h->x3D) ? 1 : 0;
    return RNDE_OK;
}
extern "C" int32_t rnde_node_matrix_mode(const rnde_node* h) { return (h && h->x3 && h->x3B && h->x3D) ? RNDE_MATRIX_BF16X3 : RNDE_MATRIX_F32; }
extern "C" int32_t rnde_node_launches_per_attempt(const rnde_node* h) {
    if (!h) return 0;
    return (h->engine == 2 && h->persist != 1) ? 7 : 1;
}

extern "C" rnde_status rnde_node_release_tape(rnde_node* h) {
    if (!h) return RNDE_ERR_BAD_ARG;
    h->have_tape = false;
    return RNDE_OK;
}

extern "C" rnde_status rnde_node_forward_host(rnde_node* h, const float* x, const float* p, int32_t B, float t0, float t1,
                                              float* u_out, int64_t* nfe_out, float* saveval, int32_t* n_saveval_out,
                                              int32_t keep_tape) {
    if (!h) return RNDE_ERR_BAD_ARG;
    float *xd = nullptr, *pd = nullptr, *ud = nullptr;
    const size_t nb = (size_t)h->D * B * 4;
    HIPCHK(h, hipMalloc((void**)&xd, nb)); HIPCHK(h, hipMalloc((void**)&ud, nb)); HIPCHK(h, hipMalloc((void**)&pd, (size_t)h->P * 4));
    HIPCHK(h, hipMemcpy(xd, x, nb, hipMemcpyHostToDevice)); HIPCHK(h, hipMemcpy(pd, p, (size_t)h->P * 4, hipMemcpyHostToDevice));
    rnde_status st = rnde_node_forward(h, xd, pd, B, t0, t1, ud, nfe_out, saveval, n_saveval_out, keep_tape, nullptr);
    if (st == RNDE_OK || st == RNDE_ERR_MAX_ATTEMPTS) hipMemcpy(u_out, ud, nb, hipMemcpyDeviceToHost);
    hipFree(xd); hipFree(pd); hipFree(ud);
    return st;
}

extern "C" rnde_status rnde_debug_feval(rnde_node* h, const float* u_dev, const float* p_dev, int32_t B, float t,
                                        float* out_dev, void* stream) {
    if (!h || B < 1 || B > h->cfg.max_batch) return RNDE_ERR_BAD_ARG;
    if (h->engine == 4) return node_tiled_feval(h, u_dev, p_dev, B, t, out_dev, stream);
    hipStream_t s = (hipStream_t)stream;
    StepParams P = make_params(h, u_dev, B, 0.f, 1.f, 0);
    P.forced = 1; P.forced_t = t; P.dbg_out = out_dev;
    if (h->engine == 3) {
        rnde_status st3 = chain_pack(h, p_dev, s);
        if (st3 != RNDE_OK) return st3;
        if (h->mw) HIPCHK(h, launch_mw<MW_FEVAL>(h, make_mw_params(h, P), 0, s));
        else HIPCHK(h, launch_chain<CM_FEVAL>(h, make_chain_params(h, P), 0, nullptr, s));
        HIPCHK(h, hipStreamSynchronize(s));
        return RNDE_OK;
    }
    if (h->engine == 2) {
        rnde_status st2 = stage_pack_weights(h, p_dev, s);
        if (st2 != RNDE_OK) return st2;
        StageParams SQ = make_stage_params(h, P, p_dev);
        HIPCHK(h, launch_stage<SM_FEVAL1>(h, SQ, 0, 0, s));
        HIPCHK(h, launch_stage<SM_FEVAL2>(h, SQ, 0, 0, s));
        HIPCHK(h, hipStreamSynchronize(s));
        return RNDE_OK;
    }
    h->err = "rnde_debug_feval: unknown engine";
    return RNDE_ERR_BAD_ARG;
}

extern "C" rnde_status rnde_debug_attempt(rnde_node* h, const float* uprev_dev, const float* k1_dev, const float* p_dev,
                                          int32_t B, float t, float dt, float* k_out_dev, float* unew_out_dev,
                                          float* eest_out, void* stream) {
    if (!h || B < 1 || B > h->cfg.max_batch) return RNDE_ERR_BAD_ARG;
    RNDE_TILED_REFUSE(h, "rnde_debug_attempt is not served (its solve is one launch with no single-attempt entry; rnde_node_forward_replay runs a given attempt sequence)");
    hipStream_t s = (hipStream_t)stream;
    h->have_tape = false;
    StepParams P = make_params(h, uprev_dev, B, 0.f, 1.f, 0);
    P.forced = 1; P.forced_t = t; P.forced_dt = dt;
    if (h->engine == 3) {
        rnde_status st3 = chain_pack(h, p_dev, s);
        if (st3 != RNDE_OK) return st3;
        const ChainParams CQ = make_chain_params(h, P);
        const int nks = h->NKD;
        HIPCHK(h, chain_convert(k1_dev, h->f0, h->D, B, CQ.ntiles, nks, 0, s));
        if (h->mw) { HIPCHK(h, launch_mw<MW_STEP>(h, make_mw_params(h, P), 0, s)); HIPCHK(h, launch_mw<MW_FINISH>(h, make_mw_params(h, P), 1, s)); }
        else { HIPCHK(h, launch_chain<CM_STEP>(h, CQ, 0, nullptr, s)); HIPCHK(h, launch_chain<CM_FINISH>(h, CQ, 1, nullptr, s)); }
        HIPCHK(h, hipMemcpyAsync(h->h_ctl, h->ctl_final, sizeof(StepState), hipMemcpyDeviceToHost, s));
        const ChainRec CL{(long long)CQ.ntiles * nks * 64, h->rk_S};
        for (int sidx = 2; sidx <= h->rk_S; ++sidx)
            HIPCHK(h, chain_convert(h->arena + CL.k(sidx), k_out_dev + (size_t)(sidx - 2) * h->D * B, h->D, B, CQ.ntiles, nks, 1, s));
        HIPCHK(h, chain_convert(h->arena + CL.unew(), unew_out_dev, h->D, B, CQ.ntiles, nks, 1, s));
        HIPCHK(h, hipStreamSynchronize(s));
        if (eest_out) *eest_out = h->h_ctl->last_eest;
        return RNDE_OK;
    }
    HIPCHK(h, hipMemsetAsync(h->f0, 0, (size_t)h->D * P.Bpad * 4, s));
    HIPCHK(h, hipMemcpyAsync(h->f0, k1_dev, (size_t)h->D * B * 4, hipMemcpyDeviceToDevice, s));
    {
        rnde_status st2 = stage_pack_weights(h, p_dev, s);
        if (st2 != RNDE_OK) return st2;
        StageParams SQ = make_stage_params(h, P, p_dev);
        HIPCHK(h, stage_attempt(h, SQ, 0, s));
        hipLaunchKernelGGL(rnde_stage_finish_kernel, dim3(256), dim3(256), 0, s, SQ, 1, (float*)nullptr);
        HIPCHK(h, hipGetLastError());
    }
    HIPCHK(h, hipMemcpyAsync(h->h_ctl, h->ctl_final, sizeof(StepState), hipMemcpyDeviceToHost, s));
    RecLayout L{(long long)h->D * P.Bpad, (long long)h->H * P.Bpad};
    const float* R = h->arena;
    for (int sidx = 2; sidx <= 7; ++sidx)
        HIPCHK(h, hipMemcpyAsync(k_out_dev + (size_t)(sidx - 2) * h->D * B, R + L.k(sidx), (size_t)h->D * B * 4, hipMemcpyDeviceToDevice, s));
    HIPCHK(h, hipMemcpyAsync(unew_out_dev, R + L.unew(), (size_t)h->D * B * 4, hipMemcpyDeviceToDevice, s));
    HIPCHK(h, hipStreamSynchronize(s));
    if (h->engine == 2 && persist_failed(h, h->sR * (P.Bpad / 16), P.Bpad / 16, h->sR, s)) { h->err = "persistent attempt kernel abandoned its hand-off; call again (multi-launch kernels now in use)"; return RNDE_ERR_HIP; }
    if (eest_out) *eest_out = h->h_ctl->last_eest;
    return RNDE_OK;
}

static rnde_status bench_attempt_impl(rnde_node* h, const float* x_dev, const float* p_dev, int32_t B, int32_t iters, int32_t taped,
                                      float* mean_us_out, void* stream);
extern "C" rnde_status rnde_bench_attempt(rnde_node* h, const float* x_dev, const float* p_dev, int32_t B, int32_t iters,
                                          float* mean_us_out, void* stream) {
    return bench_attempt_impl(h, x_dev, p_dev, B, iters, 0, mean_us_out, stream);
}
extern "C" rnde_status rnde_bench_attempt_taped(rnde_node* h, const float* x_dev, const float* p_dev, int32_t B, int32_t iters,
                                                float* mean_us_out, void* stream) {
    return bench_attempt_impl(h, x_dev, p_dev, B, iters, 1, mean_us_out, stream);
}
extern "C" rnde_status rnde_bench_attempt_cold_tape(rnde_node* h, const float* x_dev, const float* p_dev, int32_t B, int32_t iters,
                                                    int32_t records, float* mean_us_out, void* stream) {
    if (records < 2) return RNDE_ERR_BAD_ARG;
    return bench_attempt_impl(h, x_dev, p_dev, B, iters, records, mean_us_out, stream);
}
static rnde_status bench_attempt_impl(rnde_node* h, const float* x_dev, const float* p_dev, int32_t B, int32_t iters, int32_t taped,
                                      float* mean_us_out, void* stream) {
    if (!h || B < 1 || B > h->cfg.max_batch || iters < 1) return RNDE_ERR_BAD_ARG;
    RNDE_TILED_REFUSE(h, "rnde_bench_attempt* are not served (there is no per-attempt launch to time; rnde_node_timing reports the one-launch solve and the reverse sweep)");
    hipStream_t s = (hipStream_t)stream;
    h->have_tape = false;
    if (taped > 1) { const rnde_status sa = ensure_arena(h, std::min<long long>(taped, h->cfg.max_attempts)); if (sa != RNDE_OK) return sa; }
    StepParams P = make_params(h, x_dev, B, 0.f, 1.f, taped ? 1 : 0);
    P.forced = 1; P.forced_t = 0.f; P.forced_dt = 0.05f;
    rnde_status st = h->engine == 3 ? chain_pack(h, p_dev, s) : RNDE_OK;
    if (st != RNDE_OK) return st;
    StageParams SQ{};
    ChainParams CQ{};
    MwParams MQ{};
    if (h->engine == 3 && h->mw) {
        if (taped) { st = ensure_mw_slab(h, 8, P.Bpad, s); if (st != RNDE_OK) return st; }
        MQ = make_mw_params(h, P);
        HIPCHK(h, launch_mw<MW_INIT_A>(h, MQ, 0, s));
        for (int i = 0; i < 3; ++i) HIPCHK(h, launch_mw<MW_STEP>(h, MQ, 0, s));
    } else if (h->engine == 3) {
        CQ = make_chain_params(h, P);
        HIPCHK(h, launch_chain<CM_INIT_A>(h, CQ, 0, nullptr, s));
        for (int i = 0; i < 3; ++i) HIPCHK(h, launch_chain<CM_STEP>(h, CQ, 0, nullptr, s));
    } else {
        st = stage_pack_weights(h, p_dev, s);
        if (st != RNDE_OK) return st;
        SQ = make_stage_params(h, P, p_dev);
        HIPCHK(h, launch_stage<SM_I1>(h, SQ, 0, 0, s));
        HIPCHK(h, launch_stage<SM_I2>(h, SQ, 0, 0, s));
// ... 61 lines not shown
```

### regneuralde.jl_amd/csrc/rnde_binit_stage.h

```cpp
#pragma once
#include "rnde_bstage.h"

namespace rnde {

template <int ACT2, int STEP>
__global__ __launch_bounds__(64 * kSMaxW) void rnde_binit_stage_kernel(const BStageParams Q) {
#pragma clang fp contract(off)
    const BwdParams& Bq = Q.B;
    const StepParams& P = Bq.F;
    extern __shared__ __attribute__((aligned(16))) float smem[];
    const int KZ = 16 * Q.KHb + 4, KG = 16 * Q.WT + 4;
    float* ZL = smem;
    float* GL = ZL + kSCB * KZ;
    float* RED = GL + kSCB * KG;
    const int tid = threadIdx.x, lane = tid & 63;
    const int w = __builtin_amdgcn_readfirstlane(tid >> 6);
    const int rb = blockIdx.x / Q.C, ct = blockIdx.x - rb * Q.C;
    const int wg = blockIdx.x;
    const int col = lane & 15, gcol = ct * kSCB + col;
    const bool colok = gcol < P.B;
    const bool vec = (P.D & 3) == 0;
    const bool writer = (blockIdx.x == 0 && tid == 0);
    const int T = rb * Q.WT + w;
    const int r0 = 16 * T + 4 * (lane >> 4);
    const bool tile_ok = T < Q.MT;
    const long long A = (long long)P.D * P.Bpad, HB = (long long)P.H * P.Bpad;
    const size_t co = (size_t)gcol * P.D;
    const double N = (double)P.D * (double)P.Bn;
    const InitRec ir = *P.initrec;
    const float dt0 = ir.dt0;
    constexpr bool kD = (STEP == 0 || STEP == 2);
    constexpr int kPhase = STEP < 2 ? 1 : 2;
    constexpr int par = STEP < 2 ? 0 : 1;

    float dot = 0.f, tau = 0.f;
    if constexpr (kD) {
        f32x4 wD[kSMaxW];
#pragma unroll
        for (int kb = 0; kb < kSMaxW; ++kb)
            if (kb < Q.WT && w < Q.HT && rb * Q.WT + kb < Q.MT) wD[kb] = Q.pwDt[((size_t)w * Q.MT + rb * Q.WT + kb) * 64 + lane];
        f32x4 xv = {0.f, 0.f, 0.f, 0.f}, f0v = xv, f1v = xv, ub1 = xv, Uv = xv, K1v = xv;
        if (tile_ok) {
            xv = ld4(P.x + co, r0, P.D, colok, P.xvec != 0);
            f0v = ld4(P.f0 + co, r0, P.D, true, vec);
            f1v = ld4(P.f1 + co, r0, P.D, true, vec);
            if constexpr (kPhase == 2) {
                ub1 = ld4(Bq.UB1 + co, r0, P.D, true, vec);
                Uv = ld4(Bq.U + co, r0, P.D, true, vec);
                K1v = ld4(Bq.K1 + co, r0, P.D, true, vec);
            }
        }
        f32x4 v = {0.f, 0.f, 0.f, 0.f};
        if constexpr (kPhase == 1) {
            double tb, dtpb, qoldb, t1b, t0b;
            finish_attempt_scalars(Bq, 0, lane, tb, dtpb, qoldb, t1b, t0b);
            const double dtb = Bq.track_initdt ? dtpb : 0.0;
            double dt0b = 0, d1b = 0, d2b = 0;
            if (ir.sel == 2) { t1b += dtb; t0b -= dtb; }
            else if (ir.sel == 0) dt0b += 100.0 * dtb;
            else if (!ir.dt1_const) {
                const double mm = ir.max_is_d2 ? (double)ir.d2 : (double)ir.d1;
                const double mb = dtb * (-0.2) * (double)ir.dt1 / mm;
                if (ir.max_is_d2) d2b += mb; else d1b += mb;
            } else if (dt0 * 1e-3f > 1e-6f) dt0b += 1e-3 * dtb;
            const double n2 = (double)ir.d2 * (double)dt0, n2b = d2b / (double)dt0;
            dt0b += -d2b * (double)ir.d2 / (double)dt0;
            const double coef_w = n2 > 0 ? n2b / (N * n2) : 0.0;
            if (writer) { IBState b; b.tb = tb; b.t1b = t1b; b.t0b = t0b; b.dt0b = dt0b; b.d1b = d1b; b.d2b = d2b; b.coef_w = coef_w; b.pad = 0; Bq.ibstate[0] = b; }
            const float cw = (float)coef_w;
            if (tile_ok) {
#pragma unroll
                for (int i = 0; i < 4; ++i) {
                    const float sk = P.abstol + fabsf(xv[i]) * P.reltol;
                    const float wv = (f1v[i] - f0v[i]) / sk;
                    const float f1b = (colok && r0 + i < P.D ? cw * wv : 0.f) / sk;
                    v[i] = ACT2 ? f1b * (1.f - f1v[i] * f1v[i]) : f1b;
                }
                st4(Bq.zi2 + A + co, r0, P.D, true, vec, v);
            }
        } else {
            const IBState ib = Bq.ibstate[0];
            double dot1 = 0, tau1 = 0;
            for (int i = lane; i < P.nwg; i += 64) { dot1 += (double)Bq.ipart[4 * i]; tau1 += (double)Bq.ipart[4 * i + 1]; }
            dot1 = wave_sum_d(dot1); tau1 = wave_sum_d(tau1);
            double dt0b = ib.dt0b + tau1 + dot1, t0b = ib.t0b + tau1, t1b = ib.t1b, d1b = ib.d1b, d0b = 0;
            if (ir.dt0_clamped) { t1b += dt0b; t0b -= dt0b; }
            else if (!ir.dt0_const) { d0b = dt0b / (100.0 * (double)ir.d1); d1b += -dt0b * (double)dt0 / (double)ir.d1; }
            const float cv = ir.d1 > 0.f ? (float)(d1b / (N * (double)ir.d1)) : 0.f;
            const float cz = ir.d0 > 0.f ? (float)(d0b / (N * (double)ir.d0)) : 0.f;
            const float cw = (float)ib.coef_w;
            if (writer) { IBState b = ib; b.t1b = t1b; b.t0b = t0b; Bq.ibstate[1] = b; }
            if (tile_ok) {
                f32x4 u0b = {0.f, 0.f, 0.f, 0.f};
#pragma unroll
                for (int i = 0; i < 4; ++i) {
                    const bool ok = colok && r0 + i < P.D;
                    const float sk = P.abstol + fabsf(xv[i]) * P.reltol;
                    const float wv = (f1v[i] - f0v[i]) / sk, vv = f0v[i] / sk, z = xv[i] / sk;
                    const float wb = ok ? cw * wv : 0.f, vb = ok ? cv * vv : 0.f, zb = ok ? cz * z : 0.f;
                    const float skb = -(wb * wv + vb * vv + zb * z) / sk;
                    const float f0b = K1v[i] + dt0 * ub1[i] + (vb - wb) / sk;
                    u0b[i] = Uv[i] + ub1[i] + zb / sk + skb * P.reltol * sgnf(xv[i]);
                    if (Bq.sv_ubar0 && ok) u0b[i] += Bq.sv_ubar0[((size_t)gcol * Bq.sv_T) * P.D + r0 + i];
                    v[i] = ACT2 ? f0b * (1.f - f0v[i] * f0v[i]) : f0b;
                }
                st4(Bq.zi2 + co, r0, P.D, true, vec, v);
                st_tile(Bq.xbar + co, r0, P.D, colok, false, u0b);
            }
        }
#pragma unroll
        for (int i = 0; i < 4; ++i) GL[col * KG + kperm(16 * w + 4 * (lane >> 4) + i)] = tile_ok ? v[i] : 0.f;
        __syncthreads();
        f32x4* sl = (f32x4*)Q.slab + ((((size_t)par * Q.C + ct) * Q.R + rb) * Q.HT) * 64;
        const float* gbp = GL + col * KG + 4 * (lane >> 4);
        f32x4 bg[kSMaxW];
#pragma unroll
        for (int kb = 0; kb < kSMaxW; ++kb) if (kb < Q.WT) bg[kb] = *(const f32x4*)(gbp + 16 * kb);
        if (w < Q.HT) {
            f32x4 acc0 = {0.f, 0.f, 0.f, 0.f}, acc1 = {0.f, 0.f, 0.f, 0.f};
#pragma unroll
            for (int kb = 0; kb < kSMaxW; ++kb) {
                if (kb < Q.WT && rb * Q.WT + kb < Q.MT) {
                    acc0 = mfma16(wD[kb][0], bg[kb][0], acc0);
                    acc1 = mfma16(wD[kb][1], bg[kb][1], acc1);
                    acc0 = mfma16(wD[kb][2], bg[kb][2], acc0);
                    acc1 = mfma16(wD[kb][3], bg[kb][3], acc1);
                }
            }
            sl[(size_t)w * 64 + lane] = acc0 + acc1;
        }
        for (int ht = w + Q.WT; ht < Q.HT; ht += Q.WT) {
            f32x4 acc0 = {0.f, 0.f, 0.f, 0.f}, acc1 = {0.f, 0.f, 0.f, 0.f};
#pragma unroll
            for (int kb = 0; kb < kSMaxW; ++kb) {
                if (kb < Q.WT && rb * Q.WT + kb < Q.MT) {
                    const f32x4 a = Q.pwDt[((size_t)ht * Q.MT + rb * Q.WT + kb) * 64 + lane];
                    acc0 = mfma16(a[0], bg[kb][0], acc0);
                    acc1 = mfma16(a[1], bg[kb][1], acc1);
                    acc0 = mfma16(a[2], bg[kb][2], acc0);
                    acc1 = mfma16(a[3], bg[kb][3], acc1);
                }
            }
            sl[(size_t)ht * 64 + lane] = acc0 + acc1;
        }
        return;
    } else {
        f32x4 wB[kSMaxHT];
#pragma unroll
        for (int kb = 0; kb < kSMaxHT; ++kb)
            if (kb < Q.KHb && tile_ok) wB[kb] = Q.pwBt[((size_t)T * Q.KHb + kb) * 64 + lane];
        const float* hsrc = kPhase == 1 ? P.h1 : P.h0;
        float* z1dst = kPhase == 1 ? Bq.zi1 + HB : Bq.zi1;
        const float* W1t = Q.p + (size_t)P.H * P.D;
        const f32x4* sl = (const f32x4*)Q.slab + (((size_t)par * Q.C + ct) * Q.R) * Q.HT * 64;
        f32x4 f0v = {0.f, 0.f, 0.f, 0.f};
        if (kPhase == 1 && tile_ok) f0v = ld4(P.f0 + co, r0, P.D, true, vec);
        for (int ht = w; ht < Q.HT; ht += Q.WT) {
            f32x4 z = {0.f, 0.f, 0.f, 0.f};
            for (int r = 0; r < Q.R; ++r) z += sl[((size_t)r * Q.HT + ht) * 64 + lane];
            const int h0 = 16 * ht + 4 * (lane >> 4);
#pragma unroll
            for (int i = 0; i < 4; ++i) {
                const int hr = h0 + i;
                float zv = 0.f;
                if (hr < P.H) {
                    const float hv = hsrc[(size_t)gcol * P.H + hr];
                    zv = z[i] * (1.f - hv * hv);
                    if (rb == 0) { z1dst[(size_t)gcol * P.H + hr] = zv; tau += W1t[hr] * zv; }
                } else if (hr == P.H) {
                    if (rb == 0) tau += z[i];
                }
                if (hr < 16 * Q.KHb) ZL[col * KZ + kperm(hr)] = zv;
            }
        }
        if (Q.KHb > Q.HT) {
            for (int i = tid; i < kSCB * 16 * Q.KHb; i += blockDim.x) {
                const int c = i / (16 * Q.KHb), k = i - c * 16 * Q.KHb;
                if (k >= 16 * Q.HT) ZL[c * KZ + kperm(k)] = 0.f;
            }
        }
        __syncthreads();
        f32x4 gb = {0.f, 0.f, 0.f, 0.f};
        if (tile_ok) {
            f32x4 acc0 = {0.f, 0.f, 0.f, 0.f}, acc1 = {0.f, 0.f, 0.f, 0.f};
            const float* zb = ZL + col * KZ + 4 * (lane >> 4);
            f32x4 bf[kSMaxHT];
#pragma unroll
            for (int kb = 0; kb < kSMaxHT; ++kb) if (kb < Q.KHb) bf[kb] = *(const f32x4*)(zb + 16 * kb);
#pragma unroll
            for (int kb = 0; kb < kSMaxHT; ++kb) {
                if (kb < Q.KHb) {
                    acc0 = mfma16(wB[kb][0], bf[kb][0], acc0);
                    acc1 = mfma16(wB[kb][1], bf[kb][1], acc1);
                    acc0 = mfma16(wB[kb][2], bf[kb][2], acc0);
                    acc1 = mfma16(wB[kb][3], bf[kb][3], acc1);
                }
            }
            gb = acc0 + acc1;
#pragma unroll
            for (int i = 0; i < 4; ++i) if (r0 + i >= P.D) gb[i] = 0.f;
            if constexpr (kPhase == 1) {
                st4(Bq.UB1 + co, r0, P.D, true, vec, gb);
#pragma unroll
                for (int i = 0; i < 4; ++i) dot += gb[i] * f0v[i];
            } else {
                const f32x4 u0b = ld_tile(Bq.xbar + co, r0, P.D, colok, false);
                st_tile(Bq.xbar + co, r0, P.D, colok, false, u0b + gb);
            }
        }
        if (!colok) tau = 0.f;
        dot = wave_sum_f(dot); tau = wave_sum_f(tau);
        __syncthreads();
        if (lane == 0) { RED[w] = dot; RED[8 + w] = tau; }
        __syncthreads();
        if (tid == 0) {
            float sa = 0.f, ta = 0.f;
            for (int i = 0; i < Q.WT; ++i) { sa += RED[i]; ta += RED[8 + i]; }
            if constexpr (kPhase == 1) { float* o = Bq.ipart + (size_t)wg * 4; o[0] = sa; o[1] = ta; o[2] = 0.f; o[3] = 0.f; }
            else { float* o = Bq.ipart + ((size_t)P.nwg + wg) * 4; o[0] = ta; o[1] = 0.f; o[2] = 0.f; o[3] = 0.f; }
        }
    }
}

}
```

### regneuralde.jl_amd/csrc/rnde_node.h

```cpp
#pragma once
#include "../../include/rnde.h"
#include "rnde_fwd.h"
#include "rnde_bwd.h"
#include "rnde_stage.h"
#include "rnde_bstage.h"
#include "rnde_stage_persist2.h"
#include "rnde_bstage_persist.h"
#include "rnde_solve_sync.h"
#include "rnde_meet.h"
#include "rnde_binit_stage.h"
#include "rnde_head.h"
#include "rnde_chain.h"
#include "rk_tables.h"
#include "rnde_bchain.h"
#include "rnde_chainmw.h"
#include "rnde_bchainmw.h"

#include <chrono>
#include <algorithm>
#include <atomic>
#include <cmath>
#include <cstdlib>
#include <cstdio>
#include <cstring>
#include <functional>
#include <string>
#include <vector>

static hipError_t rnde_malloc(void** p, size_t bytes) {
    const hipError_t e = (hipMalloc)(p, bytes);
    const bool poison = getenv("RNDE_POISON") != nullptr;
    if (e == hipSuccess && poison && bytes) (void)hipMemset(*p, 0xFF, bytes);
    return e;
}
#define hipMalloc(p, n) rnde_malloc((void**)(p), (n))

extern "C" hipError_t rnde_launch_stage_solve(const void* stage_params, const void* persist_sync, const void* solve_sync, int act2, int x3, hipStream_t s);
extern "C" hipError_t rnde_launch_x3_pack(const float* p, void* x3B, void* x3D, void* x3Bt, void* x3Dt, int D, int H, int MT, int WT, int R, int HT, hipStream_t s);
using namespace rnde;

struct rnde_node {
    rnde_node_config cfg{};
    int D = 0, H = 0, P = 0, BT = 8, act2 = 1;
    int Bpad_max = 0, nwg_max = 0;
    int engine = 1;
    struct rnde_node_tiled* tiled = nullptr;
    ChainGeo cg{}; float* cfrags = nullptr; int NKD = 0, chain_alt = 0;
    int chain_ga = 0;
    size_t chain_lds_f = 0, chain_lds_b = 0;
    rnde_comm* couple = nullptr; int couple_batch = 0, couple_world = 1;
    int rk_tab = 0; RkTab rk{};
    int mw_clean = 0, mw_retry_after = 8;
    int mw_solve = 1; MeetRes mw_meet;
    int mw_bsweep = 1; int* mw_bargs = nullptr; int* h_mw_bargs = nullptr; unsigned* h_mw_bchk = nullptr; bool pending_bsweep = false; int bsweep_nt = 0; bool bsweep_global = false;
    int rk_S = 7, rk_order = 5;
    int mw_lat = 0;
    int mw = 0; MwGeo mg{}; float* mw_tab = nullptr; float* mw_slab = nullptr; long long mw_slab_evals = 0; size_t mw_lds_f = 0, mw_lds_b = 0;
    float* cslab = nullptr; size_t cslab_floats = 0; float* ev_t = nullptr; float* h_ev_t = nullptr;
    int sMT = 0, sWT = 0, sR = 0, sHT = 0, sK2b = 0, sKHb = 0;
    f32x4 *spwB = nullptr, *spwD = nullptr, *spwBt = nullptr, *spwDt = nullptr;
    float* slab2 = nullptr;
    size_t stage_lds = 0;
    float* head_ws = nullptr; size_t head_ws_floats = 0;
    std::function<rnde_status(hipStream_t)> after_solve; hipEvent_t ev_host = nullptr; bool rev_packed = false;
    float* cg_ws = nullptr; size_t cg_ws_floats = 0; std::vector<float> cg_sv;
    float* sv_t_dev = nullptr; size_t sv_cap = 0; std::vector<float> saveat;
    float* replay_dev = nullptr; size_t replay_cap = 0; const float* replay_host = nullptr; int n_replay = 0;
    int wgrad_side_pct = 30, stage_generic = 0;
    int persist_clean = 0, persist_retry_after = 8, persist_fallbacks = 0;
    int persist2 = -1;
    int persist = 0, persist_spins = kPersistMaxSpins; int tslab_Bpad = -1; size_t tslab_bytes = 0; float* tslab = nullptr; unsigned *pabort = nullptr, *pxcc = nullptr; unsigned* h_pchk = nullptr;
    int stage_solve = 1; MeetRes s_meet; int one_launch_solves = 0;
    int x3 = 0; void *x3B = nullptr, *x3D = nullptr, *x3Bt = nullptr, *x3Dt = nullptr; bool x3_packed = false, x3_fwd = false;
    hipStream_t wstream = nullptr;
    std::vector<hipEvent_t> wevents;
    float *f0 = nullptr, *h0 = nullptr, *u1 = nullptr, *f1 = nullptr, *h1 = nullptr, *arena = nullptr;
    float* xcopy = nullptr;
    long long arena_recs = 0, rec_stride = 0;
    float* pcopy = nullptr;
    StepState *ctl = nullptr, *ctl_final = nullptr;
    unsigned char *mbox = nullptr, *h_mbox = nullptr; size_t mbox_meta_off = 0;
    StepMeta* meta = nullptr;
    InitRec* initrec = nullptr;
    float *errpart = nullptr, *initpart = nullptr;
    BwdBuffers bw{};
    StepState* h_ctl = nullptr;
    StepMeta* h_meta = nullptr;
    InitRec* h_init = nullptr;
    float* h_scal = nullptr;
    int B = 0, Bpad = 0, nwg = 0, n_att = 0, predicted = 0;
    float t0 = 0, t1 = 0;
    bool have_tape = false;
    bool pending_bwd = false;
    float* diag_buf = nullptr;
    std::vector<int> sv_index;
    int n_saveval = 0;
    int timing = 0; hipEvent_t tev[5] = {nullptr, nullptr, nullptr, nullptr, nullptr}; bool tev_fwd = false, tev_bwd = false;
    std::string err;
};

#define HIPCHK(h, call)                                                                              \
    do {                                                                                             \
        hipError_t e__ = (call);                                                                     \
        if (e__ != hipSuccess) {                                                                     \
            (h)->err = std::string(#call) + ": " + hipGetErrorString(e__);                           \
            return RNDE_ERR_HIP;                                                                     \
        }                                                                                            \
    } while (0)

void rnde_set_create_error(const std::string& msg);
void node_tiled_destroy(rnde_node* h);
rnde_status node_tiled_forward(rnde_node* h, const float* x_dev, const float* p_dev, int32_t B, float t0, float t1, float* u_out_dev,
                               const float* saveat_host, int32_t n_saveat, float* sv_out_dev, int64_t* nfe_out, float* saveval_host,
                               int32_t* n_saveval_out, int32_t keep_tape, void* stream);
rnde_status node_tiled_backward(rnde_node* h, const float* u_bar_dev, const float* saveval_bar_host, float* x_bar_dev, float* p_bar_dev,
                                float* tspan_bar_host, void* stream);
rnde_status node_tiled_feval(rnde_node* h, const float* u_dev, const float* p_dev, int32_t B, float t, float* out_dev, void* stream);
rnde_status node_tiled_timing(rnde_node* h, float* fwd_ms, float* rev_sweep_ms, float* rev_rest_ms);
#define RNDE_TILED_REFUSE(h, what)                                                                                                       \
    do {                                                                                                                                 \
        if ((h) && (h)->engine == 4) {                                                                                                   \
            (h)->err = std::string("TrackedNeuralODE tiled engine: ") + what;                                                            \
            return RNDE_ERR_BAD_ARG;                                                                                                     \
        }                                                                                                                                \
    } while (0)

static const rnde_status RNDE_INTERNAL_RETRY = static_cast<rnde_status>(100);
StepParams make_params(rnde_node* h, const float* x, int B, float t0, float t1, int tape);
MwParams make_mw_params(rnde_node* h, const StepParams& P);
ChainParams make_chain_params(rnde_node* h, const StepParams& P);
rnde_status couple_sum(rnde_node* h, float* partials, long long count, hipStream_t s);
hipError_t stage_pack(rnde_node* h, const float* p, f32x4* dst, int which, int MTrows, int Kb, hipStream_t st);
rnde_status stage_pack_all(rnde_node* h, const float* p_dev, hipStream_t s, const float* x_src = nullptr, long long x_floats = 0);
hipError_t slab_prepare(rnde_node* h, int Bpad, hipStream_t s);
void persist_check_enqueue(rnde_node* h, int grid, hipStream_t s);
bool persist_check_result(rnde_node* h, int C, int R, hipStream_t s);
bool bsweep_failed(rnde_node* h, hipStream_t s);
rnde_status forward_impl(rnde_node* h, const float* x_dev, const float* p_dev, int32_t B, float t0, float t1,
                         float* u_out_dev, const float* saveat_host, int32_t n_saveat, float* sv_out_dev,
                         int64_t* nfe_out, float* saveval_host, int32_t* n_saveval_out, int32_t keep_tape, void* stream);
```

### regneuralde.jl_amd/csrc/rnde_reverse.hip

```cpp
#include "rnde_node.h"
#include "rnde_wgradx.h"

static rnde_status chain_bwd_run(rnde_node* h, const float* u_bar_dev, const float* saveval_bar_host, float* x_bar_dev,
                                 float* p_bar_dev, float* tspan_bar_host, hipStream_t s, bool sync = true, float* tspan_bar_dev = nullptr);
static rnde_status bwd_run(rnde_node* h, const float* u_bar_dev, const float* saveval_bar_host, float* x_bar_dev,
                           float* p_bar_dev, float* tspan_bar_host, hipStream_t s, bool sync = true, float* tspan_bar_dev = nullptr);


extern "C" rnde_status rnde_node_backward_async(rnde_node* h, const float* u_bar_dev, const float* saveval_bar_host, float* x_bar_dev,
                                                float* p_bar_dev, float* tspan_bar_dev, void* stream) {
    if (!h) return RNDE_ERR_BAD_ARG;
    RNDE_TILED_REFUSE(h, "rnde_node_backward_async is not served (rnde_node_backward runs its reverse sweep and waits for it)");
    if (!h->have_tape) { h->err = "no recorded forward"; return RNDE_ERR_NO_TAPE; }
    if (h->engine == 3) return chain_bwd_run(h, u_bar_dev, saveval_bar_host, x_bar_dev, p_bar_dev, nullptr, (hipStream_t)stream, false, tspan_bar_dev);
    return bwd_run(h, u_bar_dev, saveval_bar_host, x_bar_dev, p_bar_dev, nullptr, (hipStream_t)stream, false, tspan_bar_dev);
}

extern "C" rnde_status rnde_node_backward(rnde_node* h, const float* u_bar_dev, const float* saveval_bar_host,
                                          float* x_bar_dev, float* p_bar_dev, float* tspan_bar_host, void* stream) {
    if (!h) return RNDE_ERR_BAD_ARG;
    if (!h->have_tape) { h->err = "no recorded forward"; return RNDE_ERR_NO_TAPE; }
    if (h->engine == 4) return node_tiled_backward(h, u_bar_dev, saveval_bar_host, x_bar_dev, p_bar_dev, tspan_bar_host, stream);
    if (h->engine == 3) return chain_bwd_run(h, u_bar_dev, saveval_bar_host, x_bar_dev, p_bar_dev, tspan_bar_host, (hipStream_t)stream);
    return bwd_run(h, u_bar_dev, saveval_bar_host, x_bar_dev, p_bar_dev, tspan_bar_host, (hipStream_t)stream);
// ... 183 lines not shown
    BwdParams Q{};
    Q.F = make_params(h, h->xcopy, h->B, h->t0, h->t1, 1);
    Q.U = b.U; Q.K1 = b.K1; Q.UB1 = b.UB1; Q.zi2 = b.zi2; Q.zi1 = b.zi1; Q.svb_att = d_svb;
    Q.bstate = b.bstate; Q.ibstate = b.ibstate; Q.bpart = b.bpart; Q.ipart = b.ipart;
    Q.ubar = u_bar_dev; Q.xbar = x_bar_dev; Q.tspan_out = b.tspan_out;
    Q.n_att = n_att; Q.track_ctrl = h->cfg.track_ctrl; Q.track_initdt = h->cfg.track_initdt; Q.reg_kind = h->cfg.regularize;
    Q.bpart_n = Q.F.nwg;
    Q.tspan_scale = h->couple ? 1.f / (float)h->couple_world : 1.f;
#ifdef RNDE_DIAG
    if (getenv("RNDE_DIAG_BWD")) { if (!h->diag_buf) hipMalloc((void**)&h->diag_buf, 8192); hipMemset(h->diag_buf, 0, 512); Q.F.dbg_out = h->diag_buf; }
#endif
    Q.sv_T = (int)h->saveat.size();
    Q.sv_ubar0 = (!h->saveat.empty() && h->saveat[0] == h->t0) ? u_bar_dev : nullptr;
    if (!h->saveat.empty() && h->engine != 2) { h->err = "saveat reverse pass runs on the stage engine only"; return RNDE_ERR_BAD_ARG; }
    const long long A = (long long)h->D * Q.F.Bpad, HB = (long long)h->H * Q.F.Bpad;
    RecLayout L{A, HB};
    int ne = 2;
    h_ev2[0] = EvalDesc{b.zi2, h->h0, h->t0, 0};           h_ev1[0] = EvalDesc{b.zi1, h->xcopy, h->t0, 0};
    h_ev2[1] = EvalDesc{b.zi2 + A, h->h1, h->t0 + h->h_init->dt0, 0}; h_ev1[1] = EvalDesc{b.zi1 + HB, h->u1, h->t0 + h->h_init->dt0, 0};
    for (int n = 0; n < n_att; ++n) {
        const StepMeta& m = h->h_meta[n];
        const float* R = h->arena + (long long)m.rec * h->rec_stride;
        for (int sidx = 2; sidx <= 7; ++sidx) {
            const float ts = m.t + tsC(sidx - 1) * m.dt;
            h_ev2[ne] = EvalDesc{R + L.k(sidx), R + L.h(sidx), ts, 0};
            h_ev1[ne] = EvalDesc{R + L.z1(sidx), sidx < 7 ? R + L.g(sidx) : R + L.unew(), ts, 0};
            ++ne;
        }
    }
    HIPCHK(h, hipMemcpyAsync(b.ev1, b.h_ev1, 2 * (size_t)ne * sizeof(EvalDesc) + (size_t)n_att * 4, hipMemcpyHostToDevice, s));
    float* slab1 = b.slab;
    float* slab2w = b.slab + b.slab_floats;
    int cur1 = 0, cur2 = 0, evi = 0;
    const int per_chunk = std::max(1, (ne + 239) / 240);
    const int side_pct = h->wgrad_side_pct;
    const int sweep_cus = 8 * h->sR * ((Q.F.Bpad / 16 + 7) / 8);
    const bool side = h->engine == 2 && h->persist == 1 && side_pct > 0 && n_att >= 8 && sweep_cus <= 224 &&
                      wgrad3_ok(h->H, h->D) && wgrad3_ok(h->D, h->H);
    const int side_att = side ? std::min(n_att, n_att * side_pct / 100) : 0;
    const int group = std::max(4, (side_att + 5) / 6);
    bool used_side = false;
    auto wgrad_group = [&](int lo, int hi, bool on_side) -> rnde_status {
        if (hi <= lo) return RNDE_OK;
        hipStream_t ws = s;
        if (on_side) {
            hipEvent_t ev = h->wevents[evi++ % 64];
            HIPCHK(h, hipEventRecord(ev, s));
            HIPCHK(h, hipStreamWaitEvent(h->wstream, ev, 0));
            ws = h->wstream; used_side = true;
        }
        rnde_status r = launch_wgrad_part(h, d_ev1 + lo, hi - lo, per_chunk, h->H, h->D, h->B, slab1, &cur1, ws, on_side ? 16 : 0);
        if (r != RNDE_OK) return r;
        return launch_wgrad_part(h, d_ev2 + lo, hi - lo, per_chunk, h->D, h->H, h->B, slab2w, &cur2, ws, on_side ? 16 : 0);
    };
    int hi_att = n_att;
    hipError_t e;
    h->tev_bwd = false;
    if (h->timing) HIPCHK(h, hipEventRecord(h->tev[2], s));
    if (h->engine == 2) {
        if (!h->rev_packed) {
            HIPCHK(h, stage_pack(h, h->pcopy, h->spwBt, 2, h->sMT, h->sKHb, s));
            HIPCHK(h, stage_pack(h, h->pcopy, h->spwDt, 3, h->sHT, h->sMT, s));
        }
        h->rev_packed = false;
        BStageParams BQ{};
        BQ.B = Q; BQ.p = h->pcopy; BQ.pwBt = h->spwBt; BQ.pwDt = h->spwDt; BQ.slab = h->slab2; BQ.x3Bt = h->x3Bt; BQ.x3Dt = h->x3Dt;
        BQ.UTB = b.UTB; BQ.UNB = b.UNB; BQ.UPB0 = b.UPB0; BQ.GB = b.GB;
        BQ.EXK = b.GB + 6 * A; BQ.EXG = b.GB + 7 * A; BQ.SVW = b.GB + 8 * A;
        BQ.sv_t = h->saveat.empty() ? nullptr : h->sv_t_dev; BQ.sv_ubar = u_bar_dev; BQ.nsave = (int)h->saveat.size();
        BQ.MT = h->sMT; BQ.WT = h->sWT; BQ.R = h->sR; BQ.C = Q.F.Bpad / 16; BQ.HT = h->sHT; BQ.KHb = h->sKHb;
        double* const bsum = (double*)(b.bstate + 2);
        const bool pre_reduce = h->persist == 1 && Q.bpart_n >= 896 && !getenv("RNDE_NO_BPART_REDUCE");
        if (pre_reduce) BQ.B.bsum = bsum;
        const dim3 grid(BQ.R * BQ.C), blk(64 * BQ.WT);
        std::vector<int> sv_lo(n_att, 0), sv_hi(n_att, 0);
        if (!h->saveat.empty()) {
            int ns = (h->saveat[0] == h->t0) ? 1 : 0;
            for (int n = 0; n < n_att; ++n) {
                sv_lo[n] = ns;
                if (h->h_meta[n].flags & F_ACCEPT) {
                    const float tnew = h->h_meta[n].t + h->h_meta[n].dt;
                    while (ns < (int)h->saveat.size() && h->saveat[ns] <= tnew) ++ns;
                }
                sv_hi[n] = ns;
            }
        }
        auto eig_coefs = [&](int n, float& c1, float& c2) {
            c1 = 0.f; c2 = 0.f;
            const StepMeta& mm = h->h_meta[n];
            const bool eg_ok = !(mm.eigen == 0.f || mm.eigen != mm.eigen);
            double eigb = 0.0;
            if (h->cfg.regularize == RNDE_REG_STIFF && eg_ok) eigb = (double)b.h_svb[n] * (mm.eigen > 0 ? 1.0 : -1.0) / 3.5068;
            if (h->cfg.regularize == RNDE_REG_ERR_STIFF && eg_ok) eigb = 0.1 * (double)b.h_svb[n] / 3.5068;
            if (h->cfg.regularize == RNDE_REG_STIFF_DT && eg_ok) eigb = (double)b.h_svb[n] * ((double)mm.eigen * (double)mm.dt > 0 ? 1.0 : -1.0) * (double)mm.dt;
            if (eigb != 0.0 && mm.n1 > 0.f && mm.n2 > 0.f) {
                c1 = (float)(eigb / ((double)mm.n2 * (double)mm.n1));
                c2 = (float)(-eigb * ((double)mm.n1 / (double)mm.n2) / ((double)mm.n2 * (double)mm.n2));
            }
        };
        for (int n = n_att - 1; n >= 0; --n) {
            float c1 = 0.f, c2 = 0.f;
            eig_coefs(n, c1, c2);
            const double qo = pow((double)h->h_meta[n].qold_in, (double)kBeta2);
            if (h->persist == 1) {
                PersistSync Y{h->tslab, h->pabort, h->pxcc, h->persist_spins};
                HIPCHK(h, slab_prepare(h, Q.F.Bpad, s));
                const dim3 pgrid(8 * BQ.R * ((BQ.C + 7) / 8));
                const bool fix = BQ.WT == 7 && BQ.HT == 7 && BQ.KHb == 7 && BQ.MT == 49 && BQ.R == 7 && h->D == 784 && h->H == 100 && !h->stage_generic;
                if (fix) {
                    const size_t flds = h->stage_lds + (size_t)(RNDE_BSTAGE_HDMA ? 1 : 0) * 6 * 7 * 2 * 1024;
                    static DeviceOnce attr;
                    if (attr.need()) {
                        HIPCHK(h, hipFuncSetAttribute((const void*)rnde_bstage_attempt_kernel<1, 1>, hipFuncAttributeMaxDynamicSharedMemorySize, 160 * 1024));
                        HIPCHK(h, hipFuncSetAttribute((const void*)rnde_bstage_attempt_kernel<0, 1>, hipFuncAttributeMaxDynamicSharedMemorySize, 160 * 1024));
                        attr.done();
                    }
                    const bool x3 = h->x3_packed && h->x3Bt && h->x3Dt && !getenv("RNDE_X3_REV_OFF");
                    if (x3) {
                        const size_t xlds = sizeof(float) * ((size_t)2 * kX3ImageFloats + 64) + (size_t)(RNDE_BSTAGE_HDMA ? 1 : 0) * 6 * 7 * 2 * 1024;
                        static DeviceOnce attr3;
                        if (attr3.need()) {
#define RNDE_X3_ATTR(A, E) HIPCHK(h, hipFuncSetAttribute((const void*)rnde_bstage_attempt_kernel<A, 1, 1, E>, hipFuncAttributeMaxDynamicSharedMemorySize, 160 * 1024));
                            RNDE_X3_ATTR(1, 0) RNDE_X3_ATTR(1, 1) RNDE_X3_ATTR(1, 2) RNDE_X3_ATTR(1, 3) RNDE_X3_ATTR(0, 0) RNDE_X3_ATTR(0, 1) RNDE_X3_ATTR(0, 2) RNDE_X3_ATTR(0, 3)
#undef RNDE_X3_ATTR
                            attr3.done();
                        }
                        const int ex = (h->saveat.empty() ? 0 : 1) | (h->cfg.regularize >= RNDE_REG_STIFF ? 2 : 0);
#define RNDE_X3_LAUNCH(A, E) hipLaunchKernelGGL((rnde_bstage_attempt_kernel<A, 1, 1, E>), pgrid, blk, xlds, s, BQ, n, h->h_meta[n], c1, c2, sv_lo[n], sv_hi[n], Y, qo, b.h_svb[n])
                        if (h->act2) { if (ex == 0) RNDE_X3_LAUNCH(1, 0); else if (ex == 1) RNDE_X3_LAUNCH(1, 1); else if (ex == 2) RNDE_X3_LAUNCH(1, 2); else RNDE_X3_LAUNCH(1, 3); }
                        else { if (ex == 0) RNDE_X3_LAUNCH(0, 0); else if (ex == 1) RNDE_X3_LAUNCH(0, 1); else if (ex == 2) RNDE_X3_LAUNCH(0, 2); else RNDE_X3_LAUNCH(0, 3); }
#undef RNDE_X3_LAUNCH
                    } else if (h->act2) hipLaunchKernelGGL((rnde_bstage_attempt_kernel<1, 1>), pgrid, blk, flds, s, BQ, n, h->h_meta[n], c1, c2, sv_lo[n], sv_hi[n], Y, qo, b.h_svb[n]);
                    else hipLaunchKernelGGL((rnde_bstage_attempt_kernel<0, 1>), pgrid, blk, flds, s, BQ, n, h->h_meta[n], c1, c2, sv_lo[n], sv_hi[n], Y, qo, b.h_svb[n]);
                } else if (h->act2) hipLaunchKernelGGL((rnde_bstage_attempt_kernel<1, 0>), pgrid, blk, h->stage_lds, s, BQ, n, h->h_meta[n], c1, c2, sv_lo[n], sv_hi[n], Y, qo, b.h_svb[n]);
                else hipLaunchKernelGGL((rnde_bstage_attempt_kernel<0, 0>), pgrid, blk, h->stage_lds, s, BQ, n, h->h_meta[n], c1, c2, sv_lo[n], sv_hi[n], Y, qo, b.h_svb[n]);
                if ((st = couple_sum(h, b.bpart + (size_t)(n & 1) * Q.bpart_n * 4, 4LL * Q.bpart_n, s)) != RNDE_OK) return st;
                if (pre_reduce && n > 0) hipLaunchKernelGGL(rnde_bpart_reduce_kernel, dim3(1), dim3(64), 0, s, Q, n, bsum);
                if (n >= n_att - side_att && (hi_att - n >= group || n == n_att - side_att)) {
                    st = wgrad_group(2 + 6 * n, 2 + 6 * hi_att, true);
                    if (st != RNDE_OK) return st;
                    hi_att = n;
                }
                continue;
            }
            if (h->act2) hipLaunchKernelGGL((rnde_bstage_kernel<1, BM_START>), grid, blk, h->stage_lds, s, BQ, n, 0, h->h_meta[n], c1, c2, sv_lo[n], sv_hi[n], qo);
            else hipLaunchKernelGGL((rnde_bstage_kernel<0, BM_START>), grid, blk, h->stage_lds, s, BQ, n, 0, h->h_meta[n], c1, c2, sv_lo[n], sv_hi[n], qo);
            for (int j = 6; j >= 1; --j) {
                if (h->act2) hipLaunchKernelGGL((rnde_bstage_kernel<1, BM_STAGE>), grid, blk, h->stage_lds, s, BQ, n, j, h->h_meta[n], c1, c2, sv_lo[n], sv_hi[n], qo);
                else hipLaunchKernelGGL((rnde_bstage_kernel<0, BM_STAGE>), grid, blk, h->stage_lds, s, BQ, n, j, h->h_meta[n], c1, c2, sv_lo[n], sv_hi[n], qo);
            }
            if ((st = couple_sum(h, b.bpart + (size_t)(n & 1) * Q.bpart_n * 4, 4LL * Q.bpart_n, s)) != RNDE_OK) return st;
        }
        HIPCHK(h, hipGetLastError());
        {
            if (h->act2) {
                hipLaunchKernelGGL((rnde_binit_stage_kernel<1, 0>), grid, blk, h->stage_lds, s, BQ);
                hipLaunchKernelGGL((rnde_binit_stage_kernel<1, 1>), grid, blk, h->stage_lds, s, BQ);
            } else {
                hipLaunchKernelGGL((rnde_binit_stage_kernel<0, 0>), grid, blk, h->stage_lds, s, BQ);
                hipLaunchKernelGGL((rnde_binit_stage_kernel<0, 1>), grid, blk, h->stage_lds, s, BQ);
            }
            if ((st = couple_sum(h, Q.ipart, 4LL * Q.F.nwg, s)) != RNDE_OK) return st;
            if (h->act2) {
                hipLaunchKernelGGL((rnde_binit_stage_kernel<1, 2>), grid, blk, h->stage_lds, s, BQ);
                hipLaunchKernelGGL((rnde_binit_stage_kernel<1, 3>), grid, blk, h->stage_lds, s, BQ);
            } else {
                hipLaunchKernelGGL((rnde_binit_stage_kernel<0, 2>), grid, blk, h->stage_lds, s, BQ);
                hipLaunchKernelGGL((rnde_binit_stage_kernel<0, 3>), grid, blk, h->stage_lds, s, BQ);
            }
            if ((st = couple_sum(h, Q.ipart + 4LL * Q.F.nwg, 4LL * Q.F.nwg, s)) != RNDE_OK) return st;
            hipLaunchKernelGGL(rnde_bfin_kernel, dim3(1), dim3(64), 0, s, Q);
            HIPCHK(h, hipGetLastError());
        }
    }
    if (h->timing) HIPCHK(h, hipEventRecord(h->tev[3], s));
    st = wgrad_group(0, 2 + 6 * hi_att, false);
    if (st != RNDE_OK) return st;
    if (used_side) {
        hipEvent_t ev = h->wevents[64];
        HIPCHK(h, hipEventRecord(ev, h->wstream));
        HIPCHK(h, hipStreamWaitEvent(s, ev, 0));
    }
    if (cur1 > 16 && cur2 > 16) {
        const long long len1 = (long long)h->H * (h->D + 2), len2 = (long long)h->D * (h->H + 2);
        const size_t seg_r = std::max((size_t)len1, (size_t)len2);
        float* r1 = b.slab_r; float* r2 = b.slab_r + 16 * seg_r;
        const int pg1 = (cur1 + 15) / 16, g1 = (cur1 + pg1 - 1) / pg1, pg2 = (cur2 + 15) / 16, g2 = (cur2 + pg2 - 1) / pg2;
        const int grid = (int)std::min<long long>((std::max(len1, len2) + 255) / 256, 2048);
        ReducePair A{{{slab1, r1, len1, cur1, pg1}, {slab2w, r2, len2, cur2, pg2}}};
        hipLaunchKernelGGL(rnde_wgrad_reduce_pair, dim3(grid, std::max(g1, g2), 2), dim3(256), 0, s, A);
        ReducePair Bp{{{r1, p_bar_dev, len1, g1, g1}, {r2, p_bar_dev + (size_t)h->H * (h->D + 2), len2, g2, g2}}};
        hipLaunchKernelGGL(rnde_wgrad_reduce_pair, dim3(grid, 1, 2), dim3(256), 0, s, Bp);
        HIPCHK(h, hipGetLastError());
    } else {
        st = launch_wgrad_reduce(h, slab1, cur1, h->H, h->D, p_bar_dev, s);
        if (st != RNDE_OK) return st;
        st = launch_wgrad_reduce(h, slab2w, cur2, h->D, h->H, p_bar_dev + (size_t)h->H * (h->D + 2), s);
        if (st != RNDE_OK) return st;
    }
    if (h->timing) { HIPCHK(h, hipEventRecord(h->tev[4], s)); h->tev_bwd = true; }
#ifdef RNDE_DIAG
    if (h->engine == 2 && h->persist == 1 && getenv("RNDE_DIAG_BWD")) {
        unsigned long long hst[64] = {0};
        hipStreamSynchronize(s);
        hipMemcpy(hst, h->diag_buf, sizeof(hst), hipMemcpyDeviceToHost);
        fprintf(stderr, "persistent reverse attempt (workgroup 0 thread 0, cycles): START %lld (entry->weights issued %lld, ->w1t %lld, ->array loads issued %lld, finish_attempt_scalars %lld, scalar chain %lld, vector part %lld), its phase D + put %lld\n", (long long)(hst[1]-hst[0]), (long long)(hst[43]-hst[0]), (long long)(hst[44]-hst[43]), (long long)(hst[40]-hst[44]), (long long)(hst[41]-hst[40]), (long long)(hst[42]-hst[41]), (long long)(hst[1]-hst[42]), (long long)(hst[2]-hst[1]));
        for (int st = 0; st < 6; ++st) { const unsigned long long* q = hst + 3 + 5 * st; const unsigned long long prev = st == 0 ? hst[2] : hst[7 + 5 * (st - 1)];
            fprintf(stderr, "  stage j=%d: poll %lld A %lld B %lld C %lld D+put %lld\n", 6 - st, (long long)(q[0]-prev), (long long)(q[1]-q[0]), (long long)(q[2]-q[1]), (long long)(q[3]-q[2]), st < 5 ? (long long)(q[4]-q[3]) : 0LL); }
        fprintf(stderr, "  total %lld cycles to the end of stage 1, END (reduction of the 21 partial sums) %lld; in START's vector part the wait for the record's k arrays %lld\n",
                (long long)(hst[34]-hst[0]), (long long)(hst[35]-hst[34]), (long long)(hst[45]-hst[42]));
    }
#endif
    if (!sync) {
        if (tspan_bar_dev) HIPCHK(h, hipMemcpyAsync(tspan_bar_dev, b.tspan_out, 8, hipMemcpyDeviceToDevice, s));
        h->have_tape = false;
        h->pending_bwd = (h->engine == 2 && h->persist == 1);
        return RNDE_OK;
    }
    HIPCHK(h, hipMemcpyAsync(h->h_scal, b.tspan_out, 8, hipMemcpyDeviceToHost, s));
    if (h->engine == 2) persist_check_enqueue(h, h->sR * (Q.F.Bpad / 16), s);
    HIPCHK(h, hipStreamSynchronize(s));
    if (h->couple && rnde_comm_health(h->couple) != RNDE_OK) { h->err = std::string("coupled controller: ") + rnde_comm_last_error(h->couple); return RNDE_ERR_HIP; }
    if (tspan_bar_host) { tspan_bar_host[0] = h->h_scal[0]; tspan_bar_host[1] = h->h_scal[1]; }
    h->have_tape = false;
    if (h->engine == 2 && persist_check_result(h, Q.F.Bpad / 16, h->sR, s)) {
        h->err = "persistent reverse kernel abandoned its hand-off (tape consumed): rerun forward + backward, the multi-launch kernels are now in use";
        return RNDE_ERR_HIP;
    }
    return RNDE_OK;
}

static rnde_status head_reserve(rnde_node* h, int32_t B, int32_t n_classes) {
    const size_t need = (size_t)B * n_classes + B + (size_t)kHeadChunks * n_classes * h->D;
    if (h->head_ws_floats < need) {
        if (h->head_ws) hipFree(h->head_ws);
        h->head_ws = nullptr; h->head_ws_floats = 0;
        HIPCHK(h, hipMalloc((void**)&h->head_ws, need * 4));
        h->head_ws_floats = need;
    }
    return RNDE_OK;
}
extern "C" rnde_status rnde_classifier_head(rnde_node* h, const float* u_dev, const float* p3_dev, const float* y_dev,
                                            int32_t B, int32_t n_classes, float* logits_out_dev, float* u_bar_dev,
                                            float* p3_bar_dev, float* ce_out_dev, void* stream) {
    if (!h || B < 1 || n_classes < 1 || n_classes > kHeadMaxC) return RNDE_ERR_BAD_ARG;
    hipStream_t s = (hipStream_t)stream;
    const rnde_status rs = head_reserve(h, B, n_classes);
    if (rs != RNDE_OK) return rs;
    float* delta = h->head_ws;
    float* ce_col = h->head_ws + (size_t)B * n_classes;
    if (h->D > 256 * kHeadRowsPerThread) { h->err = "classifier head: D <= 1024"; return RNDE_ERR_BAD_ARG; }
    if (n_classes == 10) hipLaunchKernelGGL((rnde_head_col_kernel<10>), dim3(B), dim3(256), 0, s, u_dev, p3_dev, y_dev, h->D, n_classes, B,
                       logits_out_dev, u_bar_dev, delta, ce_col);
    else hipLaunchKernelGGL((rnde_head_col_kernel<0>), dim3(B), dim3(256), 0, s, u_dev, p3_dev, y_dev, h->D, n_classes, B,
                       logits_out_dev, u_bar_dev, delta, ce_col);
    float* partial = ce_col + B;
    hipLaunchKernelGGL(rnde_head_wgrad_kernel, dim3((h->D + 255) / 256, kHeadChunks), dim3(256), 0, s, u_dev, (const float*)delta,
                       h->D, n_classes, B, partial);
    hipLaunchKernelGGL(rnde_head_reduce_kernel, dim3((n_classes * h->D + 255) / 256), dim3(256), 0, s, (const float*)partial,
                       (const float*)delta, (const float*)ce_col, h->D, n_classes, B, p3_bar_dev, ce_out_dev);
    HIPCHK(h, hipGetLastError());
    return RNDE_OK;
}

extern "C" rnde_status rnde_node_classifier_grad(rnde_node* h, const float* x_dev, const float* p2_dev, const float* p3_dev,
                                                 const float* y_dev, int32_t B, int32_t n_classes, float t0, float t1,
                                                 float lambda, float* p2_bar_dev, float* p3_bar_dev, float* x_bar_dev,
                                                 float* ce_out_dev, float* reg_out_host, int64_t* nfe_out, rnde_comm* comm,
                                                 void* stream) {
    if (!h || !x_dev || !p2_dev || !p3_dev || !y_dev || !p2_bar_dev || !p3_bar_dev || !ce_out_dev) return RNDE_ERR_BAD_ARG;
    RNDE_TILED_REFUSE(h, "rnde_node_classifier_grad is not served (the fused training step runs on the stage engine: two-layer dynamics, rnde_node_create with col_tile 0)");
    if (h->engine != 2) { h->err = "rnde_node_classifier_grad: two-layer dynamics on the stage engine (col_tile 0)"; return RNDE_ERR_BAD_ARG; }
    if (B < 1 || B > h->cfg.max_batch) { h->err = "bad B or tspan"; return RNDE_ERR_BAD_ARG; }
    HIPCHK(h, hipSetDevice(h->cfg.device));
    const size_t A = (size_t)h->D * B;
    if (h->cg_ws_floats < 3 * A) {
        if (h->cg_ws) hipFree(h->cg_ws);
        h->cg_ws = nullptr; h->cg_ws_floats = 0;
        HIPCHK(h, hipMalloc((void**)&h->cg_ws, 3 * A * 4));
        h->cg_ws_floats = 3 * A;
    }
    if (!h->ev_host) HIPCHK(h, hipEventCreateWithFlags(&h->ev_host, hipEventDisableTiming));
    if (n_classes < 1 || n_classes > kHeadMaxC) return RNDE_ERR_BAD_ARG;
    rnde_status st = head_reserve(h, B, n_classes);
    if (st != RNDE_OK) return st;
    float* u = h->cg_ws; float* ubar = h->cg_ws + A; float* xbar = x_bar_dev ? x_bar_dev : h->cg_ws + 2 * A;
    h->cg_sv.resize((size_t)h->cfg.max_attempts + 1);
    int32_t nsv = 0;
    int64_t nfe = 0;
    h->after_solve = [&](hipStream_t s) -> rnde_status {
        const rnde_status r = rnde_classifier_head(h, u, p3_dev, y_dev, B, n_classes, nullptr, ubar, p3_bar_dev, ce_out_dev, s);
        return r;
    };
    st = forward_impl(h, x_dev, p2_dev, B, t0, t1, u, nullptr, 0, nullptr, &nfe, h->cg_sv.data(), &nsv, 1, stream);
    h->after_solve = nullptr;
    if (st != RNDE_OK) { h->rev_packed = false; return st; }
    double reg = 0.0;
    const bool regularize = lambda != 0.f && nsv > 0 && h->cfg.regularize != RNDE_REG_NONE;
    if (regularize) {
        for (int i = 0; i < nsv; ++i) reg += h->cg_sv[i];
        reg = (double)lambda * reg / nsv;
        for (int i = 0; i < nsv; ++i) h->cg_sv[i] = lambda / (float)nsv;
    }
    if (reg_out_host) *reg_out_host = (float)reg;
    if (nfe_out) *nfe_out = nfe;
    const int64_t n3 = (int64_t)n_classes * h->D + n_classes;
    st = bwd_run(h, ubar, regularize ? h->cg_sv.data() : nullptr, xbar, p2_bar_dev, nullptr, (hipStream_t)stream, false, nullptr);
// ... 323 lines not shown
```

### regneuralde.jl_amd/csrc/rnde_stage.h

```cpp
#pragma once
#include "rnde_fwd.h"

namespace rnde {

constexpr int kSCB = 16;
constexpr int kSMaxW = 8;
constexpr int kSMaxHT = 8;

struct StageParams {
    StepParams F;
    const float* p;
    const f32x4* pwB;
    const f32x4* pwD;
    float* slab;
    int MT, WT, R, C, HT, K2b;
    int Bpad16;
};

__device__ __forceinline__ int kperm(int k) { return (k & ~15) | ((k & 3) << 2) | ((k >> 2) & 3); }

__device__ __forceinline__ f32x4 mfma16(float a, float b, f32x4 c) {
    return __builtin_amdgcn_mfma_f32_16x16x4f32(a, b, c, 0, 0, 0);
}
__device__ __forceinline__ float add_square_unfused(float acc, float d) {
#pragma clang fp contract(off)
    const float m = d * d;
    return acc + m;
}
__device__ __forceinline__ f32x4 fma4(float s, f32x4 a, f32x4 c) { return __builtin_elementwise_fma((f32x4){s, s, s, s}, a, c); }

__device__ __forceinline__ f32x4 stage_pack_elem(const float* __restrict__ p, int which, int D, int H, int Kb, long long i) {
    const float* W1 = p;
    const float* b1 = W1 + (size_t)H * (D + 1);
    const float* W2 = b1 + H;
    const float* b2 = W2 + (size_t)D * (H + 1);
    const int l = (int)(i & 63);
    const int kb = (int)((i >> 6) % Kb);
    const int T = (int)((i >> 6) / Kb);
    const int m = 16 * T + (l & 15);
    f32x4 v;
#pragma unroll
    for (int q = 0; q < 4; ++q) {
        const int k = 16 * kb + 4 * q + (l >> 4);
        float w = 0.f;
        if (which == 0) { if (m < D) w = k <= H ? W2[(size_t)k * D + m] : (k == H + 1 ? b2[m] : 0.f); }
        else if (which == 1) { if (m < H && k < D) w = W1[(size_t)k * H + m]; }
        else if (which == 2) { if (m < D && k < H) w = W1[(size_t)m * H + k]; }
        else { if (m <= H && k < D) w = W2[(size_t)m * D + k]; }
        v[q] = w;
    }
    return v;
}
static __global__ void rnde_stage_pack_kernel(const float* __restrict__ p, f32x4* __restrict__ dst, int which, int D, int H,
                                       int MTrows, int Kb) {
    const long long total = (long long)MTrows * Kb * 64;
    for (long long i = blockIdx.x * (long long)blockDim.x + threadIdx.x; i < total; i += (long long)gridDim.x * blockDim.x)
        dst[i] = stage_pack_elem(p, which, D, H, Kb, i);
}

struct PackJob { void* dst; const float* src; long long total; int kind, which, kdim, pad; };
struct PackJobs { PackJob j[8]; };
static __global__ void rnde_pack_all_kernel(const float* __restrict__ p, const PackJobs J, int D, int H) {
    const PackJob job = J.j[blockIdx.y];
    for (long long i = blockIdx.x * (long long)blockDim.x + threadIdx.x; i < job.total; i += (long long)gridDim.x * blockDim.x) {
        if (job.kind == 0) ((f32x4*)job.dst)[i] = stage_pack_elem(p, job.which, D, H, job.kdim, i);
        else if (job.kind == 2) ((float*)job.dst)[i] = (job.src ? job.src : p)[i];
        else ((f32x4*)job.dst)[i] = ((const f32x4*)(job.src ? job.src : p))[i];
    }
}

__device__ __forceinline__ void dense_points(const StepParams& P, const RecLayout& L, const float* Rp, float tp, float dtp_, float tnew,
                                             int lo, int hi, size_t co, int gcol, int r0, bool colok, bool vec) {
    const f32x4 up = ld_tile(Rp + L.upc() + co, r0, P.D, true, vec);
    f32x4 k[7];
    k[0] = ld_tile(Rp + L.k1c() + co, r0, P.D, true, vec);
#pragma unroll
    for (int j = 1; j < 7; ++j) k[j] = ld_tile(Rp + L.k(j + 1) + co, r0, P.D, true, vec);
    const f32x4 un = ld_tile(Rp + L.unew() + co, r0, P.D, true, vec);
    for (int idx = lo; idx < hi; ++idx) {
        const float ts = P.sv_t[idx];
        f32x4 o = un;
        if (ts != tnew) {
            float b[7];
            dense_weights((ts - tp) / dtp_, b);
            f32x4 acc = b[0] * k[0];
#pragma unroll
            for (int j = 1; j < 7; ++j) acc += b[j] * k[j];
            o = up + dtp_ * acc;
        }
        st_tile(P.sv_out + ((size_t)gcol * P.nsave + idx) * P.D, r0, P.D, colok, vec && ((P.D & 3) == 0), o);
    }
}

enum { SM_START = 0, SM_STAGE = 1, SM_LAST = 2, SM_I1 = 3, SM_I2 = 4, SM_I3 = 5, SM_I4 = 6, SM_FEVAL1 = 7, SM_FEVAL2 = 8 };

__device__ __forceinline__ f32x4 ld4(const float* colbase, int r0, int D, bool ok, bool vec) { return ld_tile(colbase, r0, D, ok, vec); }
__device__ __forceinline__ void st4(float* colbase, int r0, int D, bool ok, bool vec, f32x4 v) { st_tile(colbase, r0, D, ok, vec, v); }

__device__ __forceinline__ void init_norm_parts_u0_f0(const StepParams& P, const f32x4& xv, const f32x4& kv, int r0, bool colok, float& part0, float& part1) {
    if (colok) {
#pragma unroll
        for (int i = 0; i < 4; ++i) {
            if (r0 + i < P.D) {
                const float sk = P.abstol + fabsf(xv[i]) * P.reltol;
                const float a = xv[i] / sk, b = kv[i] / sk;
                part0 += a * a; part1 += b * b;
            }
        }
    }
}
__device__ __forceinline__ float init_dt0_rule(const StepParams& P, double s0, double s1, bool writer, float* d1_out = nullptr) {
    const double N = (double)P.D * (double)P.Bn;
    const float d0 = (float)sqrt(s0 / N), d1 = (float)sqrt(s1 / N), dtmax = P.t1 - P.t0;
    float dt0;
    int c0 = 0, cl = 0;
    if (d0 < 1e-5f || d1 < 1e-5f) { dt0 = 1e-6f; c0 = 1; } else dt0 = (d0 / d1) / 100.f;
    if (dtmax < dt0) { dt0 = dtmax; cl = 1; }
    if (writer) { P.initrec->d0 = d0; P.initrec->d1 = d1; P.initrec->dt0 = dt0; P.initrec->dt0_const = c0; P.initrec->dt0_clamped = cl; }
    if (d1_out) *d1_out = d1;
    return dt0;
}
__device__ __forceinline__ f32x4 init_euler_step(const f32x4& xv, float dt0, const f32x4& f0) { return xv + dt0 * f0; }
__device__ __forceinline__ void init_norm_part_df(const StepParams& P, const f32x4& xv, const f32x4& f0, const f32x4& kv, int r0, bool colok, float& part0) {
    if (colok) {
#pragma unroll
        for (int i = 0; i < 4; ++i) {
            if (r0 + i < P.D) {
                const float sk = P.abstol + fabsf(xv[i]) * P.reltol;
                const float a = (kv[i] - f0[i]) / sk;
                part0 += a * a;
            }
        }
    }
}

template <int ACT2, int MODE>
__global__ __launch_bounds__(64 * kSMaxW) void rnde_stage_kernel(const StageParams Q, const int n, const int s) {
    const StepParams& P = Q.F;
    extern __shared__ __attribute__((aligned(16))) float smem[];
    const int KH = 16 * Q.K2b + 4, KG = 16 * Q.WT + 4;
    float* HL = smem;
    float* GL = HL + kSCB * KH;
    float* RED = GL + kSCB * KG;
    const int tid = threadIdx.x, lane = tid & 63;
    const int w = __builtin_amdgcn_readfirstlane(tid >> 6);
    const int rb = blockIdx.x / Q.C, ct = blockIdx.x - rb * Q.C;
    const int col = lane & 15, gcol = ct * kSCB + col;
    const bool colok = gcol < P.B;
    const bool vec = (P.D & 3) == 0;
    const bool writer = (blockIdx.x == 0 && tid == 0);
    const int T = rb * Q.WT + w;
    const int r0 = 16 * T + 4 * (lane >> 4);
    const bool tile_ok = T < Q.MT;
    const RecLayout L{(long long)P.D * P.Bpad, (long long)P.H * P.Bpad};
    constexpr bool kHasA = (MODE == SM_STAGE || MODE == SM_LAST || MODE == SM_I2 || MODE == SM_I4 || MODE == SM_FEVAL2);
    constexpr bool kHasD = (MODE == SM_START || MODE == SM_STAGE || MODE == SM_I1 || MODE == SM_I3 || MODE == SM_FEVAL1);

#ifdef RNDE_DIAG
#define SSTAMP(i) do { if (MODE == SM_STAGE && s == 3 && P.dbg_out && blockIdx.x == 0 && lane == 0) ((unsigned long long*)P.dbg_out)[(w * 8 + (i))] = clock64(); } while (0)
#else
#define SSTAMP(i) do { } while (0)
#endif
    SSTAMP(0);
    StepState S0;
    if constexpr (MODE == SM_STAGE || MODE == SM_LAST) S0 = P.ctl[n & 1];
    f32x4 c_up = {0.f, 0.f, 0.f, 0.f}, c_un = {0.f, 0.f, 0.f, 0.f}, c_k[6];
    bool c_early = false;
    if constexpr (MODE == SM_STAGE || MODE == SM_LAST) {
        if (P.tape && tile_ok) {
            const float* Rn = P.arena + (long long)n * P.rec_stride;
            const size_t co = (size_t)gcol * P.D;
            c_up = ld4(Rn + L.upc() + co, r0, P.D, true, vec);
            c_k[0] = ld4(Rn + L.k1c() + co, r0, P.D, true, vec);
#pragma unroll
            for (int j = 1; j < 6; ++j) if (j < s) c_k[j] = ld4(Rn + L.k(j + 1) + co, r0, P.D, true, vec);
            if constexpr (MODE == SM_LAST) c_un = ld4(Rn + L.unew() + co, r0, P.D, true, vec);
            c_early = true;
        }
    }
    f32x4 wB[kSMaxHT];
    f32x4 wD[kSMaxW];
    if constexpr (kHasA) {
#pragma unroll
        for (int kb = 0; kb < kSMaxHT; ++kb)
            if (kb < Q.K2b && tile_ok) wB[kb] = Q.pwB[((size_t)T * Q.K2b + kb) * 64 + lane];
    }
    if constexpr (kHasD) {
#pragma unroll
        for (int kb = 0; kb < kSMaxW; ++kb)
            if (kb < Q.WT && w < Q.HT && rb * Q.WT + kb < Q.MT) wD[kb] = Q.pwD[((size_t)w * Q.MT + rb * Q.WT + kb) * 64 + lane];
    }

    f32x4 zs = {0.f, 0.f, 0.f, 0.f};
    f32x4 zr[kSMaxW];
    float w1t_own[4] = {0.f, 0.f, 0.f, 0.f}, b1_own[4] = {0.f, 0.f, 0.f, 0.f};
    if constexpr (kHasA) {
#pragma unroll
        for (int i = 0; i < 4; ++i) {
            const int hr = 16 * w + 4 * (lane >> 4) + i;
            if (hr < P.H) { w1t_own[i] = Q.p[(size_t)P.H * P.D + hr]; b1_own[i] = Q.p[(size_t)P.H * (P.D + 1) + hr]; }
        }
        const int par0 = (MODE == SM_STAGE || MODE == SM_LAST) ? (s & 1) : 0;
        const f32x4* sl0 = (const f32x4*)Q.slab + (((size_t)par0 * Q.C + ct) * Q.R) * Q.HT * 64;
        if (w < Q.HT) {
#pragma unroll
            for (int r = 0; r < kSMaxW; ++r) if (r < Q.R) zr[r] = sl0[((size_t)r * Q.HT + w) * 64 + lane];
        }
    }

    float t = P.t0, dt = 0.f;
    int live = -1, rec = 0;
    if constexpr (MODE == SM_START) {
        const StepState S = advance_state(P, n, lane, writer, &P.ctl[n & 1]);
        if (P.nsave > 0) {
            const int lo = (n == 0) ? 0 : P.ctl[(n - 1) & 1].next_save, hi = S.next_save;
            if (hi > lo && tile_ok) {
                if (n == 0) {
                    st_tile(P.sv_out + (size_t)gcol * P.nsave * P.D, r0, P.D, colok, vec,
// ... 286 lines not shown
```

### regneuralde.jl_amd/csrc/rnde_x3.h

```cpp
#pragma once
#include <hip/hip_runtime.h>

namespace rnde {

typedef unsigned x3u4 __attribute__((ext_vector_type(4)));
typedef unsigned x3u2 __attribute__((ext_vector_type(2)));
typedef __bf16 x3bf8 __attribute__((ext_vector_type(8)));
typedef float x3f4 __attribute__((ext_vector_type(4)));

constexpr int kX3K = 136;
constexpr int kX3PlaneShorts = 16 * kX3K;
constexpr int kX3ImageFloats = 3 * kX3PlaneShorts / 2;

__device__ __forceinline__ unsigned x3_cvt2(float a, float b) {
    unsigned r;
    asm("v_cvt_pk_bf16_f32 %0, %1, %2" : "=v"(r) : "v"(a), "v"(b));
    return r;
}
#ifndef RNDE_X3_DOT2
#define RNDE_X3_DOT2 0
#endif
typedef __bf16 x3bf2 __attribute__((ext_vector_type(2)));
typedef float x3f2 __attribute__((ext_vector_type(2)));
__device__ __forceinline__ void x3_split2(float x0, float x1, unsigned& hi, unsigned& mid, unsigned& lo) {
#pragma clang fp contract(off)
#if RNDE_X3_DOT2
    unsigned kl = 0x0000BF80u, kh = 0xBF800000u;
    asm("" : "+s"(kl));
    asm("" : "+s"(kh));
    const x3bf2 bl = __builtin_bit_cast(x3bf2, kl), bh = __builtin_bit_cast(x3bf2, kh);
    const x3bf2 h = __builtin_convertvector((x3f2){x0, x1}, x3bf2);
    const float r0 = __builtin_amdgcn_fdot2_f32_bf16(h, bl, x0, false), r1 = __builtin_amdgcn_fdot2_f32_bf16(h, bh, x1, false);
    const x3bf2 m = __builtin_convertvector((x3f2){r0, r1}, x3bf2);
    const float s0 = __builtin_amdgcn_fdot2_f32_bf16(m, bl, r0, false), s1 = __builtin_amdgcn_fdot2_f32_bf16(m, bh, r1, false);
    hi = __builtin_bit_cast(unsigned, h);
    mid = __builtin_bit_cast(unsigned, m);
    lo = __builtin_bit_cast(unsigned, __builtin_convertvector((x3f2){s0, s1}, x3bf2));
#else
    hi = x3_cvt2(x0, x1);
    const float r0 = x0 - __uint_as_float(hi << 16), r1 = x1 - __uint_as_float(hi & 0xFFFF0000u);
    mid = x3_cvt2(r0, r1);
    const float s0 = r0 - __uint_as_float(mid << 16), s1 = r1 - __uint_as_float(mid & 0xFFFF0000u);
    lo = x3_cvt2(s0, s1);
#endif
}
__device__ __forceinline__ void x3_store4(unsigned short* img, int col, int k0, const x3f4& v) {
    unsigned h01, m01, l01, h23, m23, l23;
    x3_split2(v[0], v[1], h01, m01, l01);
    x3_split2(v[2], v[3], h23, m23, l23);
    unsigned short* p = img + col * kX3K + k0;
    *(x3u2*)p = (x3u2){h01, h23};
    *(x3u2*)(p + kX3PlaneShorts) = (x3u2){m01, m23};
    *(x3u2*)(p + 2 * kX3PlaneShorts) = (x3u2){l01, l23};
}
__device__ __forceinline__ x3u4 x3_frag(const unsigned short* img, int pl, int s, int lane) {
    return *(const x3u4*)(img + pl * kX3PlaneShorts + (lane & 15) * kX3K + 32 * s + 8 * (lane >> 4));
}
__device__ __forceinline__ x3f4 x3_mfma(const x3u4& a, const x3u4& b, const x3f4& c) {
    return __builtin_amdgcn_mfma_f32_16x16x32_bf16(__builtin_bit_cast(x3bf8, a), __builtin_bit_cast(x3bf8, b), c, 0, 0, 0);
}
template <int NS>
__device__ __forceinline__ x3f4 x3_tile(const x3u4 (&wa)[NS][3], const unsigned short* img, int lane) {
    x3f4 aL = {0.f, 0.f, 0.f, 0.f}, aN = {0.f, 0.f, 0.f, 0.f}, aM = {0.f, 0.f, 0.f, 0.f}, aH = {0.f, 0.f, 0.f, 0.f};
    x3u4 bh = x3_frag(img, 0, 0, lane), bm = x3_frag(img, 1, 0, lane), bl = x3_frag(img, 2, 0, lane);
#pragma unroll
    for (int s = 0; s < NS; ++s) {
        x3u4 nh = bh, nm = bm, nl = bl;
        if (s + 1 < NS) { nh = x3_frag(img, 0, s + 1, lane); nm = x3_frag(img, 1, s + 1, lane); nl = x3_frag(img, 2, s + 1, lane); }
        __builtin_amdgcn_sched_barrier(0);
        aL = x3_mfma(wa[s][2], bh, aL);
        aM = x3_mfma(wa[s][1], bh, aM);
        aH = x3_mfma(wa[s][0], bh, aH);
        aN = x3_mfma(wa[s][1], bm, aN);
        aL = x3_mfma(wa[s][0], bl, aL);
        aM = x3_mfma(wa[s][0], bm, aM);
        __builtin_amdgcn_sched_barrier(0);
        bh = nh; bm = nm; bl = nl;
    }
    return ((aL + aN) + aM) + aH;
}

struct X3PackDst { x3u4* d[4]; };
static __global__ void rnde_x3_pack_kernel(const float* __restrict__ p, const X3PackDst dst, int D, int H, int MT, int WT, int R, int HT) {
    const float* W1 = p;
    const float* b1 = W1 + (size_t)H * (D + 1);
    const float* W2 = b1 + H;
    const float* b2 = W2 + (size_t)D * (H + 1);
    const long long nB = (long long)MT * 4 * 64, nD = (long long)HT * R * 4 * 64, per = nB + nD;
    const int nimg = dst.d[2] ? 2 : 1;
    for (long long i = blockIdx.x * (long long)blockDim.x + threadIdx.x; i < nimg * per; i += (long long)gridDim.x * blockDim.x) {
        const int rev = (int)(i / per);
        const long long ii = i - rev * per;
        const bool isD = ii >= nB;
        const long long q = isD ? ii - nB : ii;
        const int l = (int)(q & 63), s = (int)((q >> 6) & 3), tile = (int)(q >> 8);
        float wv[8];
#pragma unroll
        for (int j = 0; j < 8; ++j) {
            const int k = 32 * s + 8 * (l >> 4) + j;
            float w = 0.f;
            if (!isD) {
                const int m = 16 * tile + (l & 15);
                if (m < D) {
                    if (!rev) w = k <= H ? W2[(size_t)k * D + m] : (k == H + 1 ? b2[m] : 0.f);
                    else if (k < H) w = W1[(size_t)m * H + k];
                }
            } else {
                const int wt = tile / R, rb = tile % R;
                const int m = 16 * wt + (l & 15), row = 16 * WT * rb + k;
                if (k < 16 * WT && row < D) {
                    if (!rev) { if (m < H) w = W1[(size_t)row * H + m]; }
                    else if (m <= H) w = W2[(size_t)m * D + row];
                }
            }
            wv[j] = w;
        }
        unsigned hi[4], mid[4], lo[4];
#pragma unroll
        for (int j = 0; j < 4; ++j) x3_split2(wv[2 * j], wv[2 * j + 1], hi[j], mid[j], lo[j]);
        x3u4* o = dst.d[2 * rev + (isD ? 1 : 0)] + ((size_t)(tile * 4 + s) * 3) * 64 + l;
        o[0] = (x3u4){hi[0], hi[1], hi[2], hi[3]};
        o[64] = (x3u4){mid[0], mid[1], mid[2], mid[3]};
        o[128] = (x3u4){lo[0], lo[1], lo[2], lo[3]};
    }
}

}
```

Measured before the change: 315,800 samples/s.

## Fold reverse init-stage kernels into one persistent launch; merge x3 pack into pack-all

Replaces the multi-launch backward init stage (separate phase kernels with host-side reductions between them) with a single persistent kernel. The workgroups exchange partial sums through a device-side meet barrier and slab polling, and the kernel only runs on the 784x100 MNIST shape when not coupled. It also folds the bf16x3 weight split/pack into the existing pack-all kernel as an extra job, which removes one more launch per step. The aim is to cut launch and inter-kernel sync overhead in the reverse pass. The cost is that the new kernel depends on all workgroups being co-resident and relies on spin-waits that can abort.

```diff
diff --git a/include/rnde.h b/include/rnde.h
--- a/include/rnde.h
+++ b/include/rnde.h
@@ -114,6 +114,7 @@
 int32_t     rnde_node_fallback_count(const rnde_node* h);
 int32_t     rnde_node_launches_per_attempt(const rnde_node* h);
 int32_t     rnde_node_one_launch_solves(const rnde_node* h);
+int32_t     rnde_node_one_launch_binits(const rnde_node* h);
 #define RNDE_MATRIX_F32 0
 #define RNDE_MATRIX_BF16X3 1
 rnde_status rnde_node_set_matrix_mode(rnde_node* h, int32_t mode);
diff --git a/regneuralde.jl_amd/_lib.py b/regneuralde.jl_amd/_lib.py
--- a/regneuralde.jl_amd/_lib.py
+++ b/regneuralde.jl_amd/_lib.py
@@ -102,6 +102,9 @@
     L.rnde_node_launches_per_attempt.argtypes = [vp]
     L.rnde_node_one_launch_solves.restype = C.c_int32
     L.rnde_node_one_launch_solves.argtypes = [vp]
+    if hasattr(L, "rnde_node_one_launch_binits"):
+        L.rnde_node_one_launch_binits.restype = C.c_int32
+        L.rnde_node_one_launch_binits.argtypes = [vp]
     L.rnde_node_set_matrix_mode.restype = C.c_int32
     L.rnde_node_set_matrix_mode.argtypes = [vp, i32]
     L.rnde_node_matrix_mode.restype = C.c_int32
@@ -215,7 +218,7 @@
            "rnde_node_forward", "rnde_node_forward_saveat", "rnde_node_forward_everystep", "rnde_node_forward_replay", "rnde_node_backward", "rnde_node_backward_async", "rnde_node_release_tape", "rnde_node_forward_host",
            "rnde_node_backward_host", "rnde_node_steps", "rnde_debug_feval", "rnde_debug_attempt",
            "rnde_bench_attempt", "rnde_bench_attempt_taped", "rnde_bench_attempt_cold_tape", "rnde_node_set_timing", "rnde_node_timing", "rnde_node_last_attempts", "rnde_node_fallback_count",
-           "rnde_node_launches_per_attempt", "rnde_node_one_launch_solves", "rnde_node_set_matrix_mode", "rnde_node_matrix_mode", "rnde_classifier_head", "rnde_node_classifier_grad", "rnde_momentum_step", "rnde_momentum_step_scaled", "rnde_adam_step",
+           "rnde_node_launches_per_attempt", "rnde_node_one_launch_solves", "rnde_node_one_launch_binits", "rnde_node_set_matrix_mode", "rnde_node_matrix_mode", "rnde_classifier_head", "rnde_node_classifier_grad", "rnde_momentum_step", "rnde_momentum_step_scaled", "rnde_adam_step",
            "rnde_comm_unique_id", "rnde_comm_create", "rnde_comm_destroy", "rnde_comm_world", "rnde_comm_last_error", "rnde_comm_library", "rnde_comm_allreduce", "rnde_comm_create_local_group", "rnde_comm_health", "rnde_comm_window_create", "rnde_comm_window_destroy", "rnde_comm_create_peers", "rnde_comm_path", "rnde_node_set_coupling", "rnde_tapes_create", "rnde_tapes_destroy", "rnde_tapes_last_error", "rnde_tapes_in_use", "rnde_tapes_node", "rnde_tapes_forward", "rnde_tapes_backward", "rnde_tapes_release",
            "rnde_nsde_param_count", "rnde_nsde_create", "rnde_nsde_destroy", "rnde_nsde_last_error", "rnde_nsde_forward",
            "rnde_nsde_forward_saveat", "rnde_nsde_forward_everystep", "rnde_nsde_forward_replay", "rnde_nsde_backward", "rnde_nsde_backward_async", "rnde_nsde_classifier_head", "rnde_nsde_classifier_grad", "rnde_nsde_steps", "rnde_nsde_debug_attempt", "rnde_nsde_set_pre_act", "rnde_nsde_moment_grad", "rnde_moment_loss", "rnde_adabelief_step", "rnde_nsde_timing", "rnde_normal_fill", "rnde_latent_create", "rnde_latent_destroy", "rnde_latent_last_error", "rnde_latent_param_counts", "rnde_latent_encode",
diff --git a/regneuralde.jl_amd/csrc/rnde.hip b/regneuralde.jl_amd/csrc/rnde.hip
--- a/regneuralde.jl_amd/csrc/rnde.hip
+++ b/regneuralde.jl_amd/csrc/rnde.hip
@@ -409,6 +409,9 @@
         if (h->s_meet.create_granules((size_t)c->max_attempts + kSolveInitRows, 3, 256) != hipSuccess) { g_create_err = "device allocation failed"; rnde_node_destroy(h); return RNDE_ERR_HIP; }
     }
     if (h->persist == 1) {
+        if (h->bi_meet.create_granules(kBinitMeetSeqs, 3, 256) != hipSuccess) { g_create_err = "device allocation failed"; rnde_node_destroy(h); return RNDE_ERR_HIP; }
+    }
+    if (h->persist == 1) {
         h->x3 = 1;
         if (const char* e7 = getenv("RNDE_X3")) h->x3 = atoi(e7) != 0;
         if (h->sMT == 49 && h->sHT == 7 && h->sR == 7 && h->sWT == 7 && h->D == 784 && h->H == 100 && !h->stage_generic) {
@@ -448,6 +451,7 @@
     if (h->mw_slab) hipFree(h->mw_slab);
     if (h->tslab) hipFree(h->tslab);
     h->s_meet.destroy();
+    h->bi_meet.destroy();
     if (h->x3B) hipFree(h->x3B);
     if (h->x3D) hipFree(h->x3D);
     if (h->x3Bt) hipFree(h->x3Bt);
@@ -542,12 +546,19 @@
     };
     add_copy(h->pcopy, nullptr, (long long)h->P);
     if (x_src) add_copy(h->xcopy, x_src, x_floats);
+    const bool x3_job = h->x3 && h->x3B && h->x3D && h->x3Bt && h->x3Dt && h->persist == 1 && !h->stage_generic;
+    if (x3_job) {
+        J.x3 = X3PackDst{{(x3u4*)h->x3B, (x3u4*)h->x3D, (x3u4*)h->x3Bt, (x3u4*)h->x3Dt}};
+        J.x3MT = h->sMT; J.x3WT = h->sWT; J.x3R = h->sR; J.x3HT = h->sHT;
+        add(nullptr, 2LL * ((long long)h->sMT + (long long)h->sHT * h->sR) * 4 * 64, 4, 0, 0);
+    }
     long long most = 0;
     for (int i = 0; i < n; ++i) most = std::max(most, J.j[i].total);
     const int grid = (int)std::min<long long>((most + 255) / 256, 256);
     hipLaunchKernelGGL(rnde_pack_all_kernel, dim3(grid, n), dim3(256), 0, s, p_dev, J, h->D, h->H);
     HIPCHK(h, hipGetLastError());
     h->rev_packed = true;
+    if (x3_job) { h->x3_fwd = true; h->x3_packed = true; return RNDE_OK; }
     return x3_pack(h, p_dev, true, s);
 }
 hipError_t slab_prepare(rnde_node* h, int Bpad, hipStream_t s) {
@@ -1065,6 +1076,7 @@
 extern "C" int32_t rnde_node_fallback_count(const rnde_node* h) { return h ? h->persist_fallbacks : 0; }
 
 extern "C" int32_t rnde_node_one_launch_solves(const rnde_node* h) { return h ? h->one_launch_solves : 0; }
+extern "C" int32_t rnde_node_one_launch_binits(const rnde_node* h) { return h ? h->one_launch_binits : 0; }
 extern "C" rnde_status rnde_node_set_matrix_mode(rnde_node* h, int32_t mode) {
     if (!h) return RNDE_ERR_BAD_ARG;
     if (mode != RNDE_MATRIX_F32 && mode != RNDE_MATRIX_BF16X3) { h->err = "matrix mode: 0 (fp32-input MFMA) or 1 (bf16x3 on the matrix cores)"; return RNDE_ERR_BAD_ARG; }
diff --git a/regneuralde.jl_amd/csrc/rnde_binit_persist.h b/regneuralde.jl_amd/csrc/rnde_binit_persist.h
--- /dev/null
+++ b/regneuralde.jl_amd/csrc/rnde_binit_persist.h
@@ -0,0 +1,148 @@
+#pragma once
+#include "rnde_binit_stage.h"
+#include "rnde_stage_persist.h"
+#include "rnde_solve_sync.h"
+#include "rnde_meet.h"
+
+namespace rnde {
+
+constexpr int kBinitMeetSeqs = 2;
+
+template <int ACT2>
+__global__ __launch_bounds__(64 * kSMaxW) void rnde_binit_persist_kernel(const BStageParams Q, const PersistSync Y, const Meet M) {
+#pragma clang fp contract(off)
+    const BwdParams& Bq = Q.B;
+    const StepParams& P = Bq.F;
+    extern __shared__ __attribute__((aligned(16))) float smem[];
+    const int KZ = 16 * Q.KHb + 4, KG = 16 * Q.WT + 4;
+    float* ZL = smem;
+    float* GL = ZL + kSCB * KZ;
+    float* RED = GL + kSCB * KG;
+    double* SUMS = (double*)(RED + 32);
+    const int tid = threadIdx.x, lane = tid & 63;
+    const int w = __builtin_amdgcn_readfirstlane(tid >> 6);
+    const int rb = (blockIdx.x >> 3) % Q.R, ct = 8 * ((blockIdx.x >> 3) / Q.R) + (blockIdx.x & 7);
+    if (ct >= Q.C) return;
+    const int wg = rb * Q.C + ct;
+    const int col = lane & 15, gcol = ct * kSCB + col;
+    const bool colok = gcol < P.B;
+    const bool vec = (P.D & 3) == 0;
+    const bool writer = (wg == 0 && tid == 0);
+    const int T = rb * Q.WT + w;
+    const int r0 = 16 * T + 4 * (lane >> 4);
+    const bool tile_ok = T < Q.MT;
+    const long long A = (long long)P.D * P.Bpad, HB = (long long)P.H * P.Bpad;
+    const size_t co = (size_t)gcol * P.D;
+    const double N = (double)P.D * (double)P.Bn;
+    if (tid == 0) { Y.xcc[wg] = __builtin_amdgcn_s_getreg((3 << 11) | (0 << 6) | 20) & 15; RED[24] = 0.f; RED[25] = 0.f; }
+
+    f32x4 pe[4];
+    bpart_request(Bq, 0, lane, pe);
+    const InitRec ir = *P.initrec;
+    const float dt0 = ir.dt0;
+    f32x4 wD[kSMaxW], wB[kSMaxHT];
+    binit_load_wD(Q, rb, w, lane, wD);
+    f32x4 xv = {0.f, 0.f, 0.f, 0.f}, f0v = xv, f1v = xv, Uv = xv, K1v = xv;
+    if (tile_ok) {
+        xv = ld4(P.x + co, r0, P.D, colok, P.xvec != 0);
+        f0v = ld4(P.f0 + co, r0, P.D, true, vec);
+        f1v = ld4(P.f1 + co, r0, P.D, true, vec);
+        Uv = ld4(Bq.U + co, r0, P.D, true, vec);
+        K1v = ld4(Bq.K1 + co, r0, P.D, true, vec);
+    }
+    binit_load_wB(Q, T, tile_ok, lane, wB);
+    float h1_own[4] = {0.f, 0.f, 0.f, 0.f}, h0_own[4] = {0.f, 0.f, 0.f, 0.f}, w1t_own[4] = {0.f, 0.f, 0.f, 0.f};
+#pragma unroll
+    for (int i = 0; i < 4; ++i) {
+        const int hr = 16 * w + 4 * (lane >> 4) + i;
+        if (hr < P.H && w < Q.HT) { h1_own[i] = P.h1[(size_t)gcol * P.H + hr]; h0_own[i] = P.h0[(size_t)gcol * P.H + hr]; w1t_own[i] = Q.p[(size_t)P.H * P.D + hr]; }
+    }
+
+    const int bufA = kSlabBufs - 2, bufB = kSlabBufs - 1;
+    const size_t tileA = (((size_t)bufA * Q.C + ct) * Q.R + rb) * Q.HT, tileB = (((size_t)bufB * Q.C + ct) * Q.R + rb) * Q.HT;
+    auto meet = [&](auto nvc, int seq, float dot, float tau, float* ipart_row) -> bool {
+        constexpr int NV = decltype(nvc)::value;
+        float sa, ta;
+        binit_block_sums(RED, dot, tau, colok, w, lane, Q.WT, sa, ta);
+        if (w == 0) {
+            float mine[NV];
+            if constexpr (NV == 2) { mine[0] = sa; mine[1] = ta; } else mine[0] = ta;
+            if (lane == 0) { float* o = ipart_row + (size_t)wg * 4; o[0] = mine[0]; o[1] = NV == 2 ? ta : 0.f; o[2] = 0.f; o[3] = 0.f; }
+            const float mine3[3] = {mine[0], NV == 2 ? ta : 0.f, 0.f};
+            double out[3];
+            const bool ok = meet_exchange_256(M.xch, M.epoch, M.abort_word, Y.max_spins, seq, M.n, wg, NV, mine3, out, lane);
+            if (lane == 0) {
+                if (!ok) RED[25] = 1.f;
+#pragma unroll
+                for (int v = 0; v < NV; ++v) SUMS[v] = ok ? out[v] : 0.0;
+            }
+        }
+        __syncthreads();
+        return RED[25] == 0.f;
+    };
+
+    IBState ib;
+    {
+        double tb, dtpb, qoldb, t1b, t0b;
+        finish_attempt_scalars_from(Bq, 0, lane, &pe, tb, dtpb, qoldb, t1b, t0b);
+        ib = binit_scalars1(Bq, ir, N, tb, dtpb, t1b, t0b);
+        if (writer) Bq.ibstate[0] = ib;
+        f32x4 v = {0.f, 0.f, 0.f, 0.f};
+        if (tile_ok) {
+            v = binit_elem1<ACT2>(P, xv, f0v, f1v, (float)ib.coef_w, colok, r0);
+            st4(Bq.zi2 + A + co, r0, P.D, true, vec, v);
+        }
+        binit_phase_d(Q, wD, v, GL, KG, rb, w, lane, tile_ok, [&](int ht, const f32x4& t) { slab_put(Y.tslab, tileA + ht, lane, t); });
+    }
+    f32x4 ub1 = {0.f, 0.f, 0.f, 0.f};
+    {
+        float dot = 0.f, tau = 0.f;
+        const bool got = binit_phase_a(Q, ZL, KZ, P.h1, Bq.zi1 + HB, rb, w, lane, gcol, tau,
+                                       [&](int ht, f32x4& z) { return slab_poll_sum(Y, bufA, Q.C, Q.R, Q.HT, ct, ht, lane, z); }, &h1_own, &w1t_own);
+        if (!got && lane == 0) RED[24] = 1.f;
+        __syncthreads();
+        if (RED[24] != 0.f) return;
+        if (tile_ok) {
+            ub1 = binit_phase_b(Q, wB, ZL, KZ, lane, r0);
+#pragma unroll
+            for (int i = 0; i < 4; ++i) dot += ub1[i] * f0v[i];
+        }
+        if (!meet(std::integral_constant<int, 2>{}, 0, dot, tau, Bq.ipart)) return;
+    }
+    f32x4 u0b = {0.f, 0.f, 0.f, 0.f};
+    {
+        float cv, cz;
+        const float cw = (float)ib.coef_w;
+        ib = binit_scalars2(ib, ir, N, SUMS[0], SUMS[1], cv, cz);
+        if (writer) Bq.ibstate[1] = ib;
+        f32x4 v = {0.f, 0.f, 0.f, 0.f};
+        if (tile_ok) {
+            v = binit_elem2<ACT2>(Bq, xv, f0v, f1v, ub1, Uv, K1v, cw, cv, cz, dt0, colok, gcol, r0, u0b);
+            st4(Bq.zi2 + co, r0, P.D, true, vec, v);
+        }
+        binit_phase_d(Q, wD, v, GL, KG, rb, w, lane, tile_ok, [&](int ht, const f32x4& t) { slab_put(Y.tslab, tileB + ht, lane, t); });
+    }
+    {
+        float tau = 0.f;
+        const bool got = binit_phase_a(Q, ZL, KZ, P.h0, Bq.zi1, rb, w, lane, gcol, tau,
+                                       [&](int ht, f32x4& z) { return slab_poll_sum(Y, bufB, Q.C, Q.R, Q.HT, ct, ht, lane, z); }, &h0_own, &w1t_own);
+        if (!got && lane == 0) RED[24] = 1.f;
+        __syncthreads();
+        if (RED[24] != 0.f) return;
+        for (int ht = w; ht < Q.HT; ht += Q.WT) slab_clear(Y.tslab, tileA + ht, lane);
+        if (tile_ok) {
+            const f32x4 gb = binit_phase_b(Q, wB, ZL, KZ, lane, r0);
+            st_tile(Bq.xbar + co, r0, P.D, colok, false, u0b + gb);
+        }
+        if (!meet(std::integral_constant<int, 1>{}, 1, 0.f, tau, Bq.ipart + (size_t)P.nwg * 4)) return;
+        for (int ht = w; ht < Q.HT; ht += Q.WT) slab_clear(Y.tslab, tileB + ht, lane);
+        if (writer) {
+            const double tau0 = SUMS[0];
+            const double sc = Bq.tspan_scale != 0.f ? (double)Bq.tspan_scale : 1.0;
+            Bq.tspan_out[0] = (float)(sc * (ib.t0b + tau0 + ib.tb));
+            Bq.tspan_out[1] = (float)(sc * ib.t1b);
+        }
+    }
+}
+
+}
diff --git a/regneuralde.jl_amd/csrc/rnde_binit_stage.h b/regneuralde.jl_amd/csrc/rnde_binit_stage.h
--- a/regneuralde.jl_amd/csrc/rnde_binit_stage.h
+++ b/regneuralde.jl_amd/csrc/rnde_binit_stage.h
@@ -2,6 +2,185 @@
 #include "rnde_bstage.h"
 
 namespace rnde {
+
+__device__ __forceinline__ IBState binit_scalars1(const BwdParams& Bq, const InitRec& ir, double N, double tb, double dtpb, double t1b, double t0b) {
+#pragma clang fp contract(off)
+    const float dt0 = ir.dt0;
+    const double dtb = Bq.track_initdt ? dtpb : 0.0;
+    double dt0b = 0, d1b = 0, d2b = 0;
+    if (ir.sel == 2) { t1b += dtb; t0b -= dtb; }
+    else if (ir.sel == 0) dt0b += 100.0 * dtb;
+    else if (!ir.dt1_const) {
+        const double mm = ir.max_is_d2 ? (double)ir.d2 : (double)ir.d1;
+        const double mb = dtb * (-0.2) * (double)ir.dt1 / mm;
+        if (ir.max_is_d2) d2b += mb; else d1b += mb;
+    } else if (dt0 * 1e-3f > 1e-6f) dt0b += 1e-3 * dtb;
+    const double n2 = (double)ir.d2 * (double)dt0, n2b = d2b / (double)dt0;
+    dt0b += -d2b * (double)ir.d2 / (double)dt0;
+    const double coef_w = n2 > 0 ? n2b / (N * n2) : 0.0;
+    IBState b; b.tb = tb; b.t1b = t1b; b.t0b = t0b; b.dt0b = dt0b; b.d1b = d1b; b.d2b = d2b; b.coef_w = coef_w; b.pad = 0;
+    return b;
+}
+template <int ACT2>
+__device__ __forceinline__ f32x4 binit_elem1(const StepParams& P, const f32x4& xv, const f32x4& f0v, const f32x4& f1v, float cw, bool colok, int r0) {
+#pragma clang fp contract(off)
+    f32x4 v = {0.f, 0.f, 0.f, 0.f};
+#pragma unroll
+    for (int i = 0; i < 4; ++i) {
+        const float sk = P.abstol + fabsf(xv[i]) * P.reltol;
+        const float wv = (f1v[i] - f0v[i]) / sk;
+        const float f1b = (colok && r0 + i < P.D ? cw * wv : 0.f) / sk;
+        v[i] = ACT2 ? f1b * (1.f - f1v[i] * f1v[i]) : f1b;
+    }
+    return v;
+}
+__device__ __forceinline__ IBState binit_scalars2(const IBState& ib, const InitRec& ir, double N, double dot1, double tau1, float& cv, float& cz) {
+#pragma clang fp contract(off)
+    const float dt0 = ir.dt0;
+    double dt0b = ib.dt0b + tau1 + dot1, t0b = ib.t0b + tau1, t1b = ib.t1b, d1b = ib.d1b, d0b = 0;
+    if (ir.dt0_clamped) { t1b += dt0b; t0b -= dt0b; }
+    else if (!ir.dt0_const) { d0b = dt0b / (100.0 * (double)ir.d1); d1b += -dt0b * (double)dt0 / (double)ir.d1; }
+    cv = ir.d1 > 0.f ? (float)(d1b / (N * (double)ir.d1)) : 0.f;
+    cz = ir.d0 > 0.f ? (float)(d0b / (N * (double)ir.d0)) : 0.f;
+    IBState b = ib; b.t1b = t1b; b.t0b = t0b;
+    return b;
+}
+template <int ACT2>
+__device__ __forceinline__ f32x4 binit_elem2(const BwdParams& Bq, const f32x4& xv, const f32x4& f0v, const f32x4& f1v, const f32x4& ub1, const f32x4& Uv,
+                                             const f32x4& K1v, float cw, float cv, float cz, float dt0, bool colok, int gcol, int r0, f32x4& u0b) {
+#pragma clang fp contract(off)
+    const StepParams& P = Bq.F;
+    f32x4 v = {0.f, 0.f, 0.f, 0.f};
+    u0b = (f32x4){0.f, 0.f, 0.f, 0.f};
+#pragma unroll
+    for (int i = 0; i < 4; ++i) {
+        const bool ok = colok && r0 + i < P.D;
+        const float sk = P.abstol + fabsf(xv[i]) * P.reltol;
+        const float wv = (f1v[i] - f0v[i]) / sk, vv = f0v[i] / sk, z = xv[i] / sk;
+        const float wb = ok ? cw * wv : 0.f, vb = ok ? cv * vv : 0.f, zb = ok ? cz * z : 0.f;
+        const float skb = -(wb * wv + vb * vv + zb * z) / sk;
+        const float f0b = K1v[i] + dt0 * ub1[i] + (vb - wb) / sk;
+        u0b[i] = Uv[i] + ub1[i] + zb / sk + skb * P.reltol * sgnf(xv[i]);
+        if (Bq.sv_ubar0 && ok) u0b[i] += Bq.sv_ubar0[((size_t)gcol * Bq.sv_T) * P.D + r0 + i];
+        v[i] = ACT2 ? f0b * (1.f - f0v[i] * f0v[i]) : f0b;
+    }
+    return v;
+}
+__device__ __forceinline__ void binit_load_wD(const BStageParams& Q, int rb, int w, int lane, f32x4 (&wD)[kSMaxW]) {
+#pragma unroll
+    for (int kb = 0; kb < kSMaxW; ++kb)
+        if (kb < Q.WT && w < Q.HT && rb * Q.WT + kb < Q.MT) wD[kb] = Q.pwDt[((size_t)w * Q.MT + rb * Q.WT + kb) * 64 + lane];
+}
+__device__ __forceinline__ void binit_load_wB(const BStageParams& Q, int T, bool tile_ok, int lane, f32x4 (&wB)[kSMaxHT]) {
+#pragma unroll
+    for (int kb = 0; kb < kSMaxHT; ++kb)
+        if (kb < Q.KHb && tile_ok) wB[kb] = Q.pwBt[((size_t)T * Q.KHb + kb) * 64 + lane];
+}
+template <class Put>
+__device__ __forceinline__ void binit_phase_d(const BStageParams& Q, const f32x4 (&wD)[kSMaxW], const f32x4& v, float* GL, int KG, int rb, int w, int lane,
+                                              bool tile_ok, Put put) {
+#pragma clang fp contract(off)
+    const int col = lane & 15;
+#pragma unroll
+    for (int i = 0; i < 4; ++i) GL[col * KG + kperm(16 * w + 4 * (lane >> 4) + i)] = tile_ok ? v[i] : 0.f;
+    __syncthreads();
+    const float* gbp = GL + col * KG + 4 * (lane >> 4);
+    f32x4 bg[kSMaxW];
+#pragma unroll
+    for (int kb = 0; kb < kSMaxW; ++kb) if (kb < Q.WT) bg[kb] = *(const f32x4*)(gbp + 16 * kb);
+    if (w < Q.HT) {
+        f32x4 acc0 = {0.f, 0.f, 0.f, 0.f}, acc1 = {0.f, 0.f, 0.f, 0.f};
+#pragma unroll
+        for (int kb = 0; kb < kSMaxW; ++kb) {
+            if (kb < Q.WT && rb * Q.WT + kb < Q.MT) {
+                acc0 = mfma16(wD[kb][0], bg[kb][0], acc0);
+                acc1 = mfma16(wD[kb][1], bg[kb][1], acc1);
+                acc0 = mfma16(wD[kb][2], bg[kb][2], acc0);
+                acc1 = mfma16(wD[kb][3], bg[kb][3], acc1);
+            }
+        }
+        put(w, acc0 + acc1);
+    }
+    for (int ht = w + Q.WT; ht < Q.HT; ht += Q.WT) {
+        f32x4 acc0 = {0.f, 0.f, 0.f, 0.f}, acc1 = {0.f, 0.f, 0.f, 0.f};
+#pragma unroll
+        for (int kb = 0; kb < kSMaxW; ++kb) {
+            if (kb < Q.WT && rb * Q.WT + kb < Q.MT) {
+                const f32x4 a = Q.pwDt[((size_t)ht * Q.MT + rb * Q.WT + kb) * 64 + lane];
+                acc0 = mfma16(a[0], bg[kb][0], acc0);
+                acc1 = mfma16(a[1], bg[kb][1], acc1);
+                acc0 = mfma16(a[2], bg[kb][2], acc0);
+                acc1 = mfma16(a[3], bg[kb][3], acc1);
+            }
+        }
+        put(ht, acc0 + acc1);
+    }
+}
+template <class Sum>
+__device__ __forceinline__ bool binit_phase_a(const BStageParams& Q, float* ZL, int KZ, const float* hsrc, float* z1dst, int rb, int w, int lane, int gcol,
+                                              float& tau, Sum sum, const float (*hpre)[4] = nullptr, const float (*w1pre)[4] = nullptr) {
+#pragma clang fp contract(off)
+    const StepParams& P = Q.B.F;
+    const int col = lane & 15, tid = threadIdx.x;
+    const float* W1t = Q.p + (size_t)P.H * P.D;
+    bool all_ok = true;
+    for (int ht = w; ht < Q.HT; ht += Q.WT) {
+        f32x4 z = {0.f, 0.f, 0.f, 0.f};
+        if (all_ok) all_ok = sum(ht, z);
+        const int h0 = 16 * ht + 4 * (lane >> 4);
+#pragma unroll
+        for (int i = 0; i < 4; ++i) {
+            const int hr = h0 + i;
+            float zv = 0.f;
+            if (hr < P.H) {
+                const float hv = (hpre && ht == w) ? (*hpre)[i] : hsrc[(size_t)gcol * P.H + hr];
+                zv = z[i] * (1.f - hv * hv);
+                if (rb == 0) { z1dst[(size_t)gcol * P.H + hr] = zv; tau += ((w1pre && ht == w) ? (*w1pre)[i] : W1t[hr]) * zv; }
+            } else if (hr == P.H) {
+                if (rb == 0) tau += z[i];
+            }
+            if (hr < 16 * Q.KHb) ZL[col * KZ + kperm(hr)] = zv;
+        }
+    }
+    if (Q.KHb > Q.HT) {
+        for (int i = tid; i < kSCB * 16 * Q.KHb; i += blockDim.x) {
+            const int c = i / (16 * Q.KHb), k = i - c * 16 * Q.KHb;
+            if (k >= 16 * Q.HT) ZL[c * KZ + kperm(k)] = 0.f;
+        }
+    }
+    return all_ok;
+}
+__device__ __forceinline__ f32x4 binit_phase_b(const BStageParams& Q, const f32x4 (&wB)[kSMaxHT], const float* ZL, int KZ, int lane, int r0) {
+#pragma clang fp contract(off)
+    f32x4 acc0 = {0.f, 0.f, 0.f, 0.f}, acc1 = {0.f, 0.f, 0.f, 0.f};
+    const float* zb = ZL + (lane & 15) * KZ + 4 * (lane >> 4);
+    f32x4 bf[kSMaxHT];
+#pragma unroll
+    for (int kb = 0; kb < kSMaxHT; ++kb) if (kb < Q.KHb) bf[kb] = *(const f32x4*)(zb + 16 * kb);
+#pragma unroll
+    for (int kb = 0; kb < kSMaxHT; ++kb) {
+        if (kb < Q.KHb) {
+            acc0 = mfma16(wB[kb][0], bf[kb][0], acc0);
+            acc1 = mfma16(wB[kb][1], bf[kb][1], acc1);
+            acc0 = mfma16(wB[kb][2], bf[kb][2], acc0);
+            acc1 = mfma16(wB[kb][3], bf[kb][3], acc1);
+        }
+    }
+    f32x4 gb = acc0 + acc1;
+#pragma unroll
+    for (int i = 0; i < 4; ++i) if (r0 + i >= Q.B.F.D) gb[i] = 0.f;
+    return gb;
+}
+__device__ __forceinline__ void binit_block_sums(float* RED, float dot, float tau, bool colok, int w, int lane, int WT, float& sa, float& ta) {
+#pragma clang fp contract(off)
+    if (!colok) tau = 0.f;
+    dot = wave_sum_f(dot); tau = wave_sum_f(tau);
+    __syncthreads();
+    if (lane == 0) { RED[w] = dot; RED[8 + w] = tau; }
+    __syncthreads();
+    sa = 0.f; ta = 0.f;
+    if (w == 0) for (int i = 0; i < WT; ++i) { sa += RED[i]; ta += RED[8 + i]; }
+}
 
 template <int ACT2, int STEP>
 __global__ __launch_bounds__(64 * kSMaxW) void rnde_binit_stage_kernel(const BStageParams Q) {
@@ -33,12 +212,9 @@
     constexpr int kPhase = STEP < 2 ? 1 : 2;
     constexpr int par = STEP < 2 ? 0 : 1;
 
-    float dot = 0.f, tau = 0.f;
     if constexpr (kD) {
         f32x4 wD[kSMaxW];
-#pragma unroll
-        for (int kb = 0; kb < kSMaxW; ++kb)
-            if (kb < Q.WT && w < Q.HT && rb * Q.WT + kb < Q.MT) wD[kb] = Q.pwDt[((size_t)w * Q.MT + rb * Q.WT + kb) * 64 + lane];
+        binit_load_wD(Q, rb, w, lane, wD);
         f32x4 xv = {0.f, 0.f, 0.f, 0.f}, f0v = xv, f1v = xv, ub1 = xv, Uv = xv, K1v = xv;
         if (tile_ok) {
             xv = ld4(P.x + co, r0, P.D, colok, P.xvec != 0);
@@ -54,28 +230,10 @@
         if constexpr (kPhase == 1) {
             double tb, dtpb, qoldb, t1b, t0b;
             finish_attempt_scalars(Bq, 0, lane, tb, dtpb, qoldb, t1b, t0b);
-            const double dtb = Bq.track_initdt ? dtpb : 0.0;
-            double dt0b = 0, d1b = 0, d2b = 0;
-            if (ir.sel == 2) { t1b += dtb; t0b -= dtb; }
-            else if (ir.sel == 0) dt0b += 100.0 * dtb;
-            else if (!ir.dt1_const) {
-                const double mm = ir.max_is_d2 ? (double)ir.d2 : (double)ir.d1;
-                const double mb = dtb * (-0.2) * (double)ir.dt1 / mm;
-                if (ir.max_is_d2) d2b += mb; else d1b += mb;
-            } else if (dt0 * 1e-3f > 1e-6f) dt0b += 1e-3 * dtb;
-            const double n2 = (double)ir.d2 * (double)dt0, n2b = d2b / (double)dt0;
-            dt0b += -d2b * (double)ir.d2 / (double)dt0;
-            const double coef_w = n2 > 0 ? n2b / (N * n2) : 0.0;
-            if (writer) { IBState b; b.tb = tb; b.t1b = t1b; b.t0b = t0b; b.dt0b = dt0b; b.d1b = d1b; b.d2b = d2b; b.coef_w = coef_w; b.pad = 0; Bq.ibstate[0] = b; }
-            const float cw = (float)coef_w;
+            const IBState b = binit_scalars1(Bq, ir, N, tb, dtpb, t1b, t0b);
+            if (writer) Bq.ibstate[0] = b;
             if (tile_ok) {
-#pragma unroll
-                for (int i = 0; i < 4; ++i) {
-                    const float sk = P.abstol + fabsf(xv[i]) * P.reltol;
-                    const float wv = (f1v[i] - f0v[i]) / sk;
-                    const float f1b = (colok && r0 + i < P.D ? cw * wv : 0.f) / sk;
-                    v[i] = ACT2 ? f1b * (1.f - f1v[i] * f1v[i]) : f1b;
-                }
+                v = binit_elem1<ACT2>(P, xv, f0v, f1v, (float)b.coef_w, colok, r0);
                 st4(Bq.zi2 + A + co, r0, P.D, true, vec, v);
             }
         } else {
@@ -83,122 +241,32 @@
             double dot1 = 0, tau1 = 0;
             for (int i = lane; i < P.nwg; i += 64) { dot1 += (double)Bq.ipart[4 * i]; tau1 += (double)Bq.ipart[4 * i + 1]; }
             dot1 = wave_sum_d(dot1); tau1 = wave_sum_d(tau1);
-            double dt0b = ib.dt0b + tau1 + dot1, t0b = ib.t0b + tau1, t1b = ib.t1b, d1b = ib.d1b, d0b = 0;
-            if (ir.dt0_clamped) { t1b += dt0b; t0b -= dt0b; }
-            else if (!ir.dt0_const) { d0b = dt0b / (100.0 * (double)ir.d1); d1b += -dt0b * (double)dt0 / (double)ir.d1; }
-            const float cv = ir.d1 > 0.f ? (float)(d1b / (N * (double)ir.d1)) : 0.f;
-            const float cz = ir.d0 > 0.f ? (float)(d0b / (N * (double)ir.d0)) : 0.f;
-            const float cw = (float)ib.coef_w;
-            if (writer) { IBState b = ib; b.t1b = t1b; b.t0b = t0b; Bq.ibstate[1] = b; }
+            float cv, cz;
+            const IBState b = binit_scalars2(ib, ir, N, dot1, tau1, cv, cz);
+            if (writer) Bq.ibstate[1] = b;
             if (tile_ok) {
-                f32x4 u0b = {0.f, 0.f, 0.f, 0.f};
-#pragma unroll
-                for (int i = 0; i < 4; ++i) {
-                    const bool ok = colok && r0 + i < P.D;
-                    const float sk = P.abstol + fabsf(xv[i]) * P.reltol;
-                    const float wv = (f1v[i] - f0v[i]) / sk, vv = f0v[i] / sk, z = xv[i] / sk;
-                    const float wb = ok ? cw * wv : 0.f, vb = ok ? cv * vv : 0.f, zb = ok ? cz * z : 0.f;
-                    const float skb = -(wb * wv + vb * vv + zb * z) / sk;
-                    const float f0b = K1v[i] + dt0 * ub1[i] + (vb - wb) / sk;
-                    u0b[i] = Uv[i] + ub1[i] + zb / sk + skb * P.reltol * sgnf(xv[i]);
-                    if (Bq.sv_ubar0 && ok) u0b[i] += Bq.sv_ubar0[((size_t)gcol * Bq.sv_T) * P.D + r0 + i];
-                    v[i] = ACT2 ? f0b * (1.f - f0v[i] * f0v[i]) : f0b;
-                }
+                f32x4 u0b;
+                v = binit_elem2<ACT2>(Bq, xv, f0v, f1v, ub1, Uv, K1v, (float)ib.coef_w, cv, cz, dt0, colok, gcol, r0, u0b);
                 st4(Bq.zi2 + co, r0, P.D, true, vec, v);
                 st_tile(Bq.xbar + co, r0, P.D, colok, false, u0b);
             }
         }
-#pragma unroll
-        for (int i = 0; i < 4; ++i) GL[col * KG + kperm(16 * w + 4 * (lane >> 4) + i)] = tile_ok ? v[i] : 0.f;
-        __syncthreads();
         f32x4* sl = (f32x4*)Q.slab + ((((size_t)par * Q.C + ct) * Q.R + rb) * Q.HT) * 64;
-        const float* gbp = GL + col * KG + 4 * (lane >> 4);
-        f32x4 bg[kSMaxW];
-#pragma unroll
-        for (int kb = 0; kb < kSMaxW; ++kb) if (kb < Q.WT) bg[kb] = *(const f32x4*)(gbp + 16 * kb);
-        if (w < Q.HT) {
-            f32x4 acc0 = {0.f, 0.f, 0.f, 0.f}, acc1 = {0.f, 0.f, 0.f, 0.f};
-#pragma unroll
-            for (int kb = 0; kb < kSMaxW; ++kb) {
-                if (kb < Q.WT && rb * Q.WT + kb < Q.MT) {
-                    acc0 = mfma16(wD[kb][0], bg[kb][0], acc0);
-                    acc1 = mfma16(wD[kb][1], bg[kb][1], acc1);
-                    acc0 = mfma16(wD[kb][2], bg[kb][2], acc0);
-                    acc1 = mfma16(wD[kb][3], bg[kb][3], acc1);
-                }
-            }
-            sl[(size_t)w * 64 + lane] = acc0 + acc1;
-        }
-        for (int ht = w + Q.WT; ht < Q.HT; ht += Q.WT) {
-            f32x4 acc0 = {0.f, 0.f, 0.f, 0.f}, acc1 = {0.f, 0.f, 0.f, 0.f};
-#pragma unroll
-            for (int kb = 0; kb < kSMaxW; ++kb) {
-                if (kb < Q.WT && rb * Q.WT + kb < Q.MT) {
-                    const f32x4 a = Q.pwDt[((size_t)ht * Q.MT + rb * Q.WT + kb) * 64 + lane];
-                    acc0 = mfma16(a[0], bg[kb][0], acc0);
-                    acc1 = mfma16(a[1], bg[kb][1], acc1);
-                    acc0 = mfma16(a[2], bg[kb][2], acc0);
-                    acc1 = mfma16(a[3], bg[kb][3], acc1);
-                }
-            }
-            sl[(size_t)ht * 64 + lane] = acc0 + acc1;
-        }
-        return;
+        binit_phase_d(Q, wD, v, GL, KG, rb, w, lane, tile_ok, [&](int ht, const f32x4& t) { sl[(size_t)ht * 64 + lane] = t; });
     } else {
         f32x4 wB[kSMaxHT];
-#pragma unroll
-        for (int kb = 0; kb < kSMaxHT; ++kb)
-            if (kb < Q.KHb && tile_ok) wB[kb] = Q.pwBt[((size_t)T * Q.KHb + kb) * 64 + lane];
-        const float* hsrc = kPhase == 1 ? P.h1 : P.h0;
-        float* z1dst = kPhase == 1 ? Bq.zi1 + HB : Bq.zi1;
-        const float* W1t = Q.p + (size_t)P.H * P.D;
+        binit_load_wB(Q, T, tile_ok, lane, wB);
         const f32x4* sl = (const f32x4*)Q.slab + (((size_t)par * Q.C + ct) * Q.R) * Q.HT * 64;
         f32x4 f0v = {0.f, 0.f, 0.f, 0.f};
         if (kPhase == 1 && tile_ok) f0v = ld4(P.f0 + co, r0, P.D, true, vec);
-        for (int ht = w; ht < Q.HT; ht += Q.WT) {
-            f32x4 z = {0.f, 0.f, 0.f, 0.f};
+        float dot = 0.f, tau = 0.f;
+        binit_phase_a(Q, ZL, KZ, kPhase == 1 ? P.h1 : P.h0, kPhase == 1 ? Bq.zi1 + HB : Bq.zi1, rb, w, lane, gcol, tau, [&](int ht, f32x4& z) {
             for (int r = 0; r < Q.R; ++r) z += sl[((size_t)r * Q.HT + ht) * 64 + lane];
-            const int h0 = 16 * ht + 4 * (lane >> 4);
-#pragma unroll
-            for (int i = 0; i < 4; ++i) {
-                const int hr = h0 + i;
-                float zv = 0.f;
-                if (hr < P.H) {
-                    const float hv = hsrc[(size_t)gcol * P.H + hr];
-                    zv = z[i] * (1.f - hv * hv);
-                    if (rb == 0) { z1dst[(size_t)gcol * P.H + hr] = zv; tau += W1t[hr] * zv; }
-                } else if (hr == P.H) {
-                    if (rb == 0) tau += z[i];
-                }
-                if (hr < 16 * Q.KHb) ZL[col * KZ + kperm(hr)] = zv;
-            }
-        }
-        if (Q.KHb > Q.HT) {
-            for (int i = tid; i < kSCB * 16 * Q.KHb; i += blockDim.x) {
-                const int c = i / (16 * Q.KHb), k = i - c * 16 * Q.KHb;
-                if (k >= 16 * Q.HT) ZL[c * KZ + kperm(k)] = 0.f;
-            }
-        }
+            return true;
+        });
         __syncthreads();
-        f32x4 gb = {0.f, 0.f, 0.f, 0.f};
         if (tile_ok) {
-            f32x4 acc0 = {0.f, 0.f, 0.f, 0.f}, acc1 = {0.f, 0.f, 0.f, 0.f};
-            const float* zb = ZL + col * KZ + 4 * (lane >> 4);
-            f32x4 bf[kSMaxHT];
-#pragma unroll
-            for (int kb = 0; kb < kSMaxHT; ++kb) if (kb < Q.KHb) bf[kb] = *(const f32x4*)(zb + 16 * kb);
-#pragma unroll
-            for (int kb = 0; kb < kSMaxHT; ++kb) {
-                if (kb < Q.KHb) {
-                    acc0 = mfma16(wB[kb][0], bf[kb][0], acc0);
-                    acc1 = mfma16(wB[kb][1], bf[kb][1], acc1);
-                    acc0 = mfma16(wB[kb][2], bf[kb][2], acc0);
-                    acc1 = mfma16(wB[kb][3], bf[kb][3], acc1);
-                }
-            }
-            gb = acc0 + acc1;
-#pragma unroll
-            for (int i = 0; i < 4; ++i) if (r0 + i >= P.D) gb[i] = 0.f;
+            const f32x4 gb = binit_phase_b(Q, wB, ZL, KZ, lane, r0);
             if constexpr (kPhase == 1) {
                 st4(Bq.UB1 + co, r0, P.D, true, vec, gb);
 #pragma unroll
@@ -208,14 +276,9 @@
                 st_tile(Bq.xbar + co, r0, P.D, colok, false, u0b + gb);
             }
         }
-        if (!colok) tau = 0.f;
-        dot = wave_sum_f(dot); tau = wave_sum_f(tau);
-        __syncthreads();
-        if (lane == 0) { RED[w] = dot; RED[8 + w] = tau; }
-        __syncthreads();
+        float sa, ta;
+        binit_block_sums(RED, dot, tau, colok, w, lane, Q.WT, sa, ta);
         if (tid == 0) {
-            float sa = 0.f, ta = 0.f;
-            for (int i = 0; i < Q.WT; ++i) { sa += RED[i]; ta += RED[8 + i]; }
             if constexpr (kPhase == 1) { float* o = Bq.ipart + (size_t)wg * 4; o[0] = sa; o[1] = ta; o[2] = 0.f; o[3] = 0.f; }
             else { float* o = Bq.ipart + ((size_t)P.nwg + wg) * 4; o[0] = ta; o[1] = 0.f; o[2] = 0.f; o[3] = 0.f; }
         }
diff --git a/regneuralde.jl_amd/csrc/rnde_node.h b/regneuralde.jl_amd/csrc/rnde_node.h
--- a/regneuralde.jl_amd/csrc/rnde_node.h
+++ b/regneuralde.jl_amd/csrc/rnde_node.h
@@ -9,6 +9,7 @@
 #include "rnde_solve_sync.h"
 #include "rnde_meet.h"
 #include "rnde_binit_stage.h"
+#include "rnde_binit_persist.h"
 #include "rnde_head.h"
 #include "rnde_chain.h"
 #include "rk_tables.h"
@@ -71,6 +72,7 @@
     int persist2 = -1;
     int persist = 0, persist_spins = kPersistMaxSpins; int tslab_Bpad = -1; size_t tslab_bytes = 0; float* tslab = nullptr; unsigned *pabort = nullptr, *pxcc = nullptr; unsigned* h_pchk = nullptr;
     int stage_solve = 1; MeetRes s_meet; int one_launch_solves = 0;
+    MeetRes bi_meet; int one_launch_binits = 0;
     int x3 = 0; void *x3B = nullptr, *x3D = nullptr, *x3Bt = nullptr, *x3Dt = nullptr; bool x3_packed = false, x3_fwd = false;
     hipStream_t wstream = nullptr;
     std::vector<hipEvent_t> wevents;
diff --git a/regneuralde.jl_amd/csrc/rnde_reverse.hip b/regneuralde.jl_amd/csrc/rnde_reverse.hip
--- a/regneuralde.jl_amd/csrc/rnde_reverse.hip
+++ b/regneuralde.jl_amd/csrc/rnde_reverse.hip
@@ -359,7 +359,21 @@
             if ((st = couple_sum(h, b.bpart + (size_t)(n & 1) * Q.bpart_n * 4, 4LL * Q.bpart_n, s)) != RNDE_OK) return st;
         }
         HIPCHK(h, hipGetLastError());
-        {
+        bool binit_fold = h->persist == 1 && h->bi_meet.xch && BQ.C <= 32 && !h->couple && Q.F.nwg == BQ.R * BQ.C &&
+                          BQ.WT == 7 && BQ.HT == 7 && BQ.KHb == 7 && BQ.MT == 49 && BQ.R == 7 && h->D == 784 && h->H == 100 && !h->stage_generic;
+        if (binit_fold) { const char* e = getenv("RNDE_BINIT_FOLD"); binit_fold = !(e && e[0] == '0'); }
+        if (binit_fold) {
+            PersistSync Y{h->tslab, h->pabort, h->pxcc, h->persist_spins};
+            HIPCHK(h, slab_prepare(h, Q.F.Bpad, s));
+            Meet M = h->bi_meet.begin(Q.F.nwg, false, s);
+            HIPCHK(h, h->bi_meet.err);
+            M.abort_word = h->pabort;
+            const dim3 pgrid(8 * BQ.R * ((BQ.C + 7) / 8));
+            if (h->act2) hipLaunchKernelGGL((rnde_binit_persist_kernel<1>), pgrid, blk, h->stage_lds, s, BQ, Y, M);
+            else hipLaunchKernelGGL((rnde_binit_persist_kernel<0>), pgrid, blk, h->stage_lds, s, BQ, Y, M);
+            HIPCHK(h, hipGetLastError());
+            ++h->one_launch_binits;
+        } else {
             if (h->act2) {
                 hipLaunchKernelGGL((rnde_binit_stage_kernel<1, 0>), grid, blk, h->stage_lds, s, BQ);
                 hipLaunchKernelGGL((rnde_binit_stage_kernel<1, 1>), grid, blk, h->stage_lds, s, BQ);
diff --git a/regneuralde.jl_amd/csrc/rnde_stage.h b/regneuralde.jl_amd/csrc/rnde_stage.h
--- a/regneuralde.jl_amd/csrc/rnde_stage.h
+++ b/regneuralde.jl_amd/csrc/rnde_stage.h
@@ -1,5 +1,6 @@
 #pragma once
 #include "rnde_fwd.h"
+#include "rnde_x3.h"
 
 namespace rnde {
 
@@ -59,11 +60,12 @@
 }
 
 struct PackJob { void* dst; const float* src; long long total; int kind, which, kdim, pad; };
-struct PackJobs { PackJob j[8]; };
+struct PackJobs { PackJob j[8]; X3PackDst x3; int x3MT, x3WT, x3R, x3HT; };
 static __global__ void rnde_pack_all_kernel(const float* __restrict__ p, const PackJobs J, int D, int H) {
     const PackJob job = J.j[blockIdx.y];
     for (long long i = blockIdx.x * (long long)blockDim.x + threadIdx.x; i < job.total; i += (long long)gridDim.x * blockDim.x) {
         if (job.kind == 0) ((f32x4*)job.dst)[i] = stage_pack_elem(p, job.which, D, H, job.kdim, i);
+        else if (job.kind == 4) x3_pack_elem(p, J.x3, i, D, H, J.x3MT, J.x3WT, J.x3R, J.x3HT);
         else if (job.kind == 2) ((float*)job.dst)[i] = (job.src ? job.src : p)[i];
         else ((f32x4*)job.dst)[i] = ((const f32x4*)(job.src ? job.src : p))[i];
     }
diff --git a/regneuralde.jl_amd/csrc/rnde_x3.h b/regneuralde.jl_amd/csrc/rnde_x3.h
--- a/regneuralde.jl_amd/csrc/rnde_x3.h
+++ b/regneuralde.jl_amd/csrc/rnde_x3.h
@@ -81,48 +81,51 @@
 }
 
 struct X3PackDst { x3u4* d[4]; };
-static __global__ void rnde_x3_pack_kernel(const float* __restrict__ p, const X3PackDst dst, int D, int H, int MT, int WT, int R, int HT) {
+__device__ __forceinline__ void x3_pack_elem(const float* __restrict__ p, const X3PackDst& dst, long long i, int D, int H, int MT, int WT, int R, int HT) {
     const float* W1 = p;
     const float* b1 = W1 + (size_t)H * (D + 1);
     const float* W2 = b1 + H;
     const float* b2 = W2 + (size_t)D * (H + 1);
     const long long nB = (long long)MT * 4 * 64, nD = (long long)HT * R * 4 * 64, per = nB + nD;
+    const int rev = (int)(i / per);
+    const long long ii = i - rev * per;
+    const bool isD = ii >= nB;
+    const long long q = isD ? ii - nB : ii;
+    const int l = (int)(q & 63), s = (int)((q >> 6) & 3), tile = (int)(q >> 8);
+    float wv[8];
+#pragma unroll
+    for (int j = 0; j < 8; ++j) {
+        const int k = 32 * s + 8 * (l >> 4) + j;
+        float w = 0.f;
+        if (!isD) {
+            const int m = 16 * tile + (l & 15);
+            if (m < D) {
+                if (!rev) w = k <= H ? W2[(size_t)k * D + m] : (k == H + 1 ? b2[m] : 0.f);
+                else if (k < H) w = W1[(size_t)m * H + k];
+            }
+        } else {
+            const int wt = tile / R, rb = tile % R;
+            const int m = 16 * wt + (l & 15), row = 16 * WT * rb + k;
+            if (k < 16 * WT && row < D) {
+                if (!rev) { if (m < H) w = W1[(size_t)row * H + m]; }
+                else if (m <= H) w = W2[(size_t)m * D + row];
+            }
+        }
+        wv[j] = w;
+    }
+    unsigned hi[4], mid[4], lo[4];
+#pragma unroll
+    for (int j = 0; j < 4; ++j) x3_split2(wv[2 * j], wv[2 * j + 1], hi[j], mid[j], lo[j]);
+    x3u4* o = dst.d[2 * rev + (isD ? 1 : 0)] + ((size_t)(tile * 4 + s) * 3) * 64 + l;
+    o[0] = (x3u4){hi[0], hi[1], hi[2], hi[3]};
+    o[64] = (x3u4){mid[0], mid[1], mid[2], mid[3]};
+    o[128] = (x3u4){lo[0], lo[1], lo[2], lo[3]};
+}
+static __global__ void rnde_x3_pack_kernel(const float* __restrict__ p, const X3PackDst dst, int D, int H, int MT, int WT, int R, int HT) {
+    const long long per = ((long long)MT + (long long)HT * R) * 4 * 64;
     const int nimg = dst.d[2] ? 2 : 1;
-    for (long long i = blockIdx.x * (long long)blockDim.x + threadIdx.x; i < nimg * per; i += (long long)gridDim.x * blockDim.x) {
-        const int rev = (int)(i / per);
-        const long long ii = i - rev * per;
-        const bool isD = ii >= nB;
-        const long long q = isD ? ii - nB : ii;
-        const int l = (int)(q & 63), s = (int)((q >> 6) & 3), tile = (int)(q >> 8);
-        float wv[8];
-#pragma unroll
-        for (int j = 0; j < 8; ++j) {
-            const int k = 32 * s + 8 * (l >> 4) + j;
-            float w = 0.f;
-            if (!isD) {
-                const int m = 16 * tile + (l & 15);
-                if (m < D) {
-                    if (!rev) w = k <= H ? W2[(size_t)k * D + m] : (k == H + 1 ? b2[m] : 0.f);
-                    else if (k < H) w = W1[(size_t)m * H + k];
-                }
-            } else {
-                const int wt = tile / R, rb = tile % R;
-                const int m = 16 * wt + (l & 15), row = 16 * WT * rb + k;
-                if (k < 16 * WT && row < D) {
-                    if (!rev) { if (m < H) w = W1[(size_t)row * H + m]; }
-                    else if (m <= H) w = W2[(size_t)m * D + row];
-                }
-            }
-            wv[j] = w;
-        }
-        unsigned hi[4], mid[4], lo[4];
-#pragma unroll
-        for (int j = 0; j < 4; ++j) x3_split2(wv[2 * j], wv[2 * j + 1], hi[j], mid[j], lo[j]);
-        x3u4* o = dst.d[2 * rev + (isD ? 1 : 0)] + ((size_t)(tile * 4 + s) * 3) * 64 + l;
-        o[0] = (x3u4){hi[0], hi[1], hi[2], hi[3]};
-        o[64] = (x3u4){mid[0], mid[1], mid[2], mid[3]};
-        o[128] = (x3u4){lo[0], lo[1], lo[2], lo[3]};
-    }
+    for (long long i = blockIdx.x * (long long)blockDim.x + threadIdx.x; i < nimg * per; i += (long long)gridDim.x * blockDim.x)
+        x3_pack_elem(p, dst, i, D, H, MT, WT, R, HT);
 }
 
 }
```

New measurement: 318,800 samples/s (median of 6 runs). Within noise of the previous version (+0.9%).
